# zahmedy/PyTorch-Distributed-Data-Parallel-DDP-Trainer

Hardware: AMD Instinct MI355X
Metric: images/sec MNIST SimpleCNN DDP at 1/2/4/8 MI355X; DDP scaling efficiency (higher is better)
Workload: dtype bf16; 1 GPU; model=SimpleCNN (520,586 params), global_batch=32, per_rank_batch=32, image=1x28x28, parallelism=dp1, engine=fused hipGraph, graph_steps=7, graph_head=0, fuse_level=3, level3=True, params_finite=True, bucket_allreduce=none, params_identical_across_ranks=True, ranks_seen=1, force_allreduce=False, inlaunch_allreduce=False

## Files before the change

csrc/bindings.cpp:

```cpp
#include <torch/extension.h>
#include <c10/hip/HIPStream.h>

#include <optional>

#include "kernels/conv_infer.h"
#include "kernels/launchers.h"
#include "runtime/runtime.h"

namespace py = pybind11;
using at::Tensor;
using namespace ddp_amd;

extern "C" const char ddp_amd_source_hash_str[];

namespace {

hipStream_t cur_stream() { return c10::hip::getCurrentHIPStream().stream(); }

void check_cuda(const Tensor& t, const char* name) {
  TORCH_CHECK(t.is_cuda(), name, " must be a GPU tensor");
  TORCH_CHECK(t.is_contiguous(), name, " must be contiguous");
}
void check(const Tensor& t, const char* name, at::ScalarType st) {
  check_cuda(t, name);
// ... 1118 lines not shown
  m.def("seg_sqnorm", &op_seg_sqnorm, py::arg("p"), py::arg("g"), py::arg("plan"), py::arg("partials"),
        py::arg("ticket"), py::arg("sums"), py::arg("trust"), py::arg("trust_coef"), py::arg("eps"),
        py::arg("gscale") = py::none());
  m.def("lars", &op_lars, py::arg("p"), py::arg("g"), py::arg("mbuf"), py::arg("lr"), py::arg("momentum"),
        py::arg("dampening"), py::arg("nesterov"), py::arg("maximize"), py::arg("first_step"), py::arg("update"),
        py::arg("shadows"), py::arg("plan"), py::arg("trust"), py::arg("gscale") = py::none(),
        py::arg("sched") = py::none());
  m.def("seg_sqnorm_blocks", &seg_sqnorm_blocks);
  m.attr("LARS_ITEM") = LARS_ITEM;
  m.attr("LARS_CHUNK") = LARS_CHUNK;
  m.attr("LARS_MAX_BLOCKS") = LARS_MAX_BLOCKS;
  m.attr("LARS_MAX_SEGS") = LARS_MAX_SEGS;
  m.def("grad_norm_blocks", &grad_norm_blocks);
  m.attr("GRAD_NORM_THREADS") = GN_THREADS;
  m.attr("GRAD_NORM_QUADS") = GN_QUADS;
  m.attr("GRAD_NORM_MAX_BLOCKS") = GN_MAX_BLOCKS;
  m.def("grad_reduce", &op_grad_reduce);
  m.def("scale_copy", &op_scale_copy);
  m.def("_mark_exiting", &ddp_amd::mark_exiting);
  m.def("conv_gemm_fwd", &op_conv_gemm_fwd, py::arg("X"), py::arg("W"), py::arg("bias"), py::arg("Y"),
        py::arg("KH"), py::arg("KW"), py::arg("stride"), py::arg("pad"), py::arg("relu") = false,
        py::arg("stats") = py::none(), py::arg("part") = py::none(), py::arg("bp") = 0, py::arg("bc") = 0,
        py::arg("splits") = 0, py::arg("halo") = -1, py::arg("bn") = py::none());
  m.def("conv_gemm_infer", &op_conv_gemm_infer, py::arg("X"), py::arg("W"), py::arg("sc"), py::arg("sh"),
        py::arg("res"), py::arg("Y"), py::arg("KH"), py::arg("KW"), py::arg("stride"), py::arg("pad"),
        py::arg("relu") = true, py::arg("part") = py::none(), py::arg("bp") = 0, py::arg("bc") = 0,
        py::arg("splits") = 0, py::arg("halo") = -1);
  m.def("bn_fold", &op_bn_fold);
  m.def("resnet_eval_tail", &op_resnet_eval_tail);
  m.def("resnet_eval_totals", &op_resnet_eval_totals);
  m.def("conv_gemm_dgrad", &op_conv_gemm_dgrad, py::arg("dY"), py::arg("W"), py::arg("Xact"), py::arg("dX"),
        py::arg("KH"), py::arg("KW"), py::arg("stride"), py::arg("pad"), py::arg("part") = py::none(),
        py::arg("bp") = 0, py::arg("bc") = 0, py::arg("splits") = 0, py::arg("parity") = -1,
        py::arg("halo") = -1);
  m.def("conv_gemm_wgrad_chunks", &op_conv_gemm_wgrad_chunks);
  m.def("conv_gemm_wgrad_set_halo", &conv_gemm_wgrad_set_halo, py::arg("halo"), py::arg("target") = 256,
        py::arg("cit") = 0,
        "weight-gradient plan override: halo 0 = the per-tap GEMM kernel only, 1 (default) / 2 = "
        "tap-fused halo kernel for every eligible stride-1 3x3 layer; target = blocks per launch; cit = "
        "input channels per halo block (0 auto, 16, 32)");
  m.def("conv_gemm_wgrad_force_tile", &conv_gemm_wgrad_force_tile);
  m.def("conv_gemm_wgrad_tiles", [](const Tensor& X, const Tensor& dY, int KH, int KW, int st, int pd) {
    return conv_gemm_wgrad_tiles(geom_of(X, dY, KH, KW, st, pd));
  });
  m.def("conv_gemm_wgrad_ppc", [](const Tensor& X, const Tensor& dY, int KH, int KW, int st, int pd) {
    return conv_gemm_wgrad_ppc(geom_of(X, dY, KH, KW, st, pd));
  });
  m.def("conv_gemm_wgrad", &op_conv_gemm_wgrad, py::arg("dY"), py::arg("X"), py::arg("out"), py::arg("KH"),
        py::arg("KW"), py::arg("stride"), py::arg("pad"), py::arg("ppc"), py::arg("accum") = false,
        py::arg("ks") = 0, py::arg("bn") = py::none());
  m.def("conv_gemm_wgrad_uses_halo", [](const Tensor& X, const Tensor& dY, int KH, int KW, int stride, int pad,
                                        int ppc) { return conv_gemm_wgrad_uses_halo(geom_of(X, dY, KH, KW, stride, pad), ppc); });
  m.def("conv_gemm_plan", &op_conv_gemm_plan, py::arg("X"), py::arg("Y"), py::arg("KH"), py::arg("KW"),
        py::arg("stride"), py::arg("pad"), py::arg("dgrad") = false, py::arg("bp") = 0, py::arg("bc") = 0,
        py::arg("splits") = 0, py::arg("parity") = -1, py::arg("halo") = -1);
  m.def("bn_finalize", &op_bn_finalize);
  m.def("hip_set_device_flags", [](int dev, unsigned flags) {
    hipError_t e = hipSetDevice(dev);
    if (e == hipSuccess) e = hipSetDeviceFlags(flags);
    return (int)e;
  });
  m.def("bn_apply", &op_bn_apply);
  m.def("bn_finalize_groups", &bn_finalize_groups);
  m.def("bn_bwd_rows", [](long P, int C) { return bn_bwd_rows(P, C, nullptr); });
  m.def("bn_bwd", &op_bn_bwd, py::arg("dout"), py::arg("out"), py::arg("x"), py::arg("mean"),
        py::arg("invstd"), py::arg("gamma"), py::arg("count"), py::arg("ws"), py::arg("sums"),
        py::arg("dgamma"), py::arg("dbeta"), py::arg("accum"), py::arg("dx"), py::arg("dres"),
        py::arg("dout2") = py::none(), py::arg("mask_beta") = py::none());
  m.def("bn_bwd_set_px_per_block", &bn_bwd_set_px_per_block);
  m.def("maxpool_fwd", &op_maxpool_fwd, py::arg("x"), py::arg("y"), py::arg("amax"), py::arg("bn") = py::none());
  m.def("maxpool_bwd", &op_maxpool_bwd, py::arg("dy"), py::arg("amax"), py::arg("dx"),
        py::arg("dy2") = py::none());
  m.def("avgpool_fwd", &op_avgpool_fwd);
  m.def("image_gather_nhwc4", &op_image_gather_nhwc4);
  m.def("image_gather_aug_nhwc4", &op_image_gather_aug_nhwc4);
  m.def("image_gather_mix_nhwc4", &op_image_gather_mix_nhwc4);
  m.def("avgpool_bwd", &op_avgpool_bwd);
  m.def("sgemm", &op_sgemm, py::arg("M"), py::arg("N"), py::arg("K"), py::arg("A"), py::arg("sam"),
        py::arg("sak"), py::arg("B"), py::arg("sbk"), py::arg("sbn"), py::arg("C"), py::arg("bias"),
        py::arg("alpha"), py::arg("accum") = false);
  m.def("transpose_w", &op_transpose_w);
  m.def("rccl_version", []() { int v = 0; ncclGetVersion(&v); return v; });
  m.def("step_head_slots", &conv3x3_step_head_slots);
  m.def("source_hash", []() {
    const std::string s(ddp_amd_source_hash_str);
    const size_t eq = s.find('=');
    return eq == std::string::npos ? s : s.substr(eq + 1);
  });
  m.def("pci_bus_id", [](int dev) {
    char buf[64] = {0};
    if (hipDeviceGetPCIBusId(buf, sizeof(buf) - 1, dev) != hipSuccess)
      throw std::runtime_error("hipDeviceGetPCIBusId failed");
    return std::string(buf);
  });

  py::class_<Comm, std::shared_ptr<Comm>>(m, "Comm")
      .def_static("new_unique_id", []() { return py::bytes(Comm::new_unique_id()); })
      .def(py::init([](py::bytes uid, int rank, int world, int device) {
             return std::make_shared<Comm>(std::string(uid), rank, world, device);
           }))
      .def_property_readonly("rank", &Comm::rank)
      .def_property_readonly("world", &Comm::world)
      .def("all_reduce", [](Comm& c, Tensor& t, int op, uint64_t stream) {
             check_cuda(t, "tensor");
             c.all_reduce(t.data_ptr(), t.numel(), dtype_code(t), op, stream_or_current(stream));
           }, py::arg("tensor"), py::arg("op") = 0, py::arg("stream") = 0)
      .def("all_reduce_premul", [](Comm& c, Tensor& t, double scale, uint64_t stream) {
             check_cuda(t, "tensor");
             TORCH_CHECK(t.scalar_type() == at::kFloat && t.is_contiguous(), "all_reduce_premul: contiguous fp32");
             c.all_reduce_premul(t.data_ptr<float>(), t.numel(), (float)scale, stream_or_current(stream));
           }, py::arg("tensor"), py::arg("scale"), py::arg("stream") = 0)
      .def("broadcast", [](Comm& c, Tensor& t, int root, uint64_t stream) {
             check_cuda(t, "tensor");
             c.broadcast(t.data_ptr(), t.numel(), dtype_code(t), root, stream_or_current(stream));
           }, py::arg("tensor"), py::arg("root") = 0, py::arg("stream") = 0)
      .def("all_gather", [](Comm& c, const Tensor& send, Tensor& recv, uint64_t stream) {
             check_cuda(send, "send"); check_cuda(recv, "recv");
             TORCH_CHECK(recv.numel() == send.numel() * c.world(), "all_gather: recv size");
             c.all_gather(send.data_ptr(), recv.data_ptr(), send.numel(), dtype_code(send),
                          stream_or_current(stream));
           }, py::arg("send"), py::arg("recv"), py::arg("stream") = 0)
      .def("reduce_scatter", [](Comm& c, const Tensor& send, Tensor& recv, int op, uint64_t stream) {
             check_cuda(send, "send"); check_cuda(recv, "recv");
             TORCH_CHECK(send.numel() == recv.numel() * c.world(), "reduce_scatter: send size");
             c.reduce_scatter(send.data_ptr(), recv.data_ptr(), recv.numel(), dtype_code(recv), op,
                              stream_or_current(stream));
           }, py::arg("send"), py::arg("recv"), py::arg("op") = 0, py::arg("stream") = 0);

  py::class_<XgmiComm, std::shared_ptr<XgmiComm>>(m, "XgmiComm")
      .def(py::init<int, int, int>(), py::arg("rank"), py::arg("world"), py::arg("device"))
      .def("add_channel", &XgmiComm::add_channel, py::arg("off"), py::arg("n"), py::arg("oneshot") = false,
           py::arg("grid_cap") = 0)
      .def("blocks", &XgmiComm::blocks)
      .def("bus_id", &XgmiComm::bus_id)
      .def("oneshot", &XgmiComm::oneshot)
      .def_property_readonly("channels", &XgmiComm::channels)
      .def("set_data", [](XgmiComm& x, Tensor& t) {
        check(t, "data", at::kFloat);
        x.set_data(t.data_ptr<float>(), t.numel());
      })
      .def("export_handles", [](const XgmiComm& x) { return py::bytes(x.export_handles()); })
      .def("import_handles", [](XgmiComm& x, const std::vector<py::bytes>& all) {
        std::vector<std::string> v;
        for (const auto& b : all) v.emplace_back(b);
        x.import_handles(v);
      })
      .def("all_reduce", [](XgmiComm& x, int ch, double scale, bool publish, double prescale) {
        x.all_reduce(ch, cur_stream(), (float)scale, publish, (float)prescale);
      }, py::arg("channel"), py::arg("scale") = 1.0, py::arg("publish") = false, py::arg("prescale") = 1.0)
      .def("all_reduce_pair", [](XgmiComm& x, int ch0, int ch1, std::optional<Tensor> params,
                                 std::optional<Tensor> mbuf, double lr, double momentum, double dampening,
                                 double wd, bool nesterov, bool first_step, std::optional<Tensor> step_ctr) {
        SgdArgs sa{(float)lr, (float)momentum, (float)dampening, (float)wd, nesterov ? 1 : 0, 0,
                   first_step ? 1 : 0, params ? 1 : 0};
        float* p = nullptr;
        float* m = nullptr;
        if (params) {
          check(*params, "params", at::kFloat);
          TORCH_CHECK(params->numel() >= x.data_numel(), "all_reduce_pair: params smaller than the data buffer");
          p = params->data_ptr<float>();
          if (momentum != 0.0) {
            TORCH_CHECK(mbuf.has_value(), "all_reduce_pair: momentum buffer required");
            check(*mbuf, "momentum", at::kFloat);
            TORCH_CHECK(mbuf->numel() == params->numel(), "all_reduce_pair: momentum size");
            m = mbuf->data_ptr<float>();
          }
// ... 53 lines not shown
            check(p, "params", at::kFloat);
            TORCH_CHECK(p.numel() >= x.data_numel(r), "xgmi loopback: params smaller than the data buffer");
            TORCH_CHECK(((uintptr_t)p.data_ptr() & 15) == 0, "xgmi loopback: params must be 16-byte aligned");
            rb[r].params = p.data_ptr<float>();
            if (mom) {
              Tensor& mb = (*mbuf)[r];
              check(mb, "momentum", at::kFloat);
              TORCH_CHECK(mb.numel() == p.numel() && ((uintptr_t)mb.data_ptr() & 15) == 0,
                          "xgmi loopback: momentum buffer size / alignment");
              rb[r].mbuf = mb.data_ptr<float>();
            }
            if (shadows) {
              rb[r].sh = make_shadows((*shadows)[r]);
              for (int i = 0; i < rb[r].sh.count; ++i)
                TORCH_CHECK(rb[r].sh.r[i].off >= 0 && rb[r].sh.r[i].off + rb[r].sh.r[i].n <= p.numel(),
                            "shadow out of range");
            }
          }
        } else {
          TORCH_CHECK(!shadows, "xgmi loopback: shadows need params");
        }
        if (step_ctr) {
          TORCH_CHECK((int)step_ctr->size() == W, "xgmi loopback: one step counter per rank");
          for (int r = 0; r < W; ++r) {
            check((*step_ctr)[r], "step_ctr", at::kInt);
            rb[r].step_ctr = (*step_ctr)[r].data_ptr<int>();
          }
        }
        x.all_reduce(ch, cur_stream(), sa, rb, (float)scale, publish, (float)prescale, wt);
      }, py::arg("channel"), py::arg("scale") = 1.0, py::arg("publish") = false, py::arg("prescale") = 1.0,
         py::arg("wt") = false, py::arg("params") = py::none(), py::arg("momentum_buffer") = py::none(),
         py::arg("shadows") = py::none(), py::arg("step_ctr") = py::none(), py::arg("lr") = 0.0,
         py::arg("momentum") = 0.0, py::arg("dampening") = 0.0, py::arg("weight_decay") = 0.0,
         py::arg("nesterov") = false, py::arg("first_step") = false)
      .def("error_flags", &XgmiLoopback::error_flags)
      .def("seq", &XgmiLoopback::seq, py::arg("channel"), py::arg("rank"), py::arg("block"))
      .def("set_timeout", &XgmiLoopback::set_timeout);
  py::class_<Reducer,std::shared_ptr<Reducer>>(m, "Reducer")
      .def(py::init([](std::shared_ptr<Comm> comm, Tensor& flat, std::vector<long> poff,
                       std::vector<long> pnum, std::vector<int> pb, std::vector<long> boff,
                       std::vector<long> bnum, bool prescale) {
             check(flat, "flat_grad", at::kFloat);
             for (size_t i = 0; i < poff.size(); ++i)
               TORCH_CHECK(poff[i] >= 0 && poff[i] + pnum[i] <= flat.numel(), "param slot OOB");
             for (size_t i = 0; i < boff.size(); ++i)
               TORCH_CHECK(boff[i] >= 0 && boff[i] + bnum[i] <= flat.numel(), "bucket OOB");
             return std::make_shared<Reducer>(comm, flat.data_ptr<float>(), poff, pnum, pb, boff,
                                              bnum, prescale);
           }))
      .def("mark_ready", [](Reducer& r, int param, std::optional<Tensor> grad) {
             const float* src = nullptr;
             if (grad) { check(*grad, "grad", at::kFloat); src = grad->data_ptr<float>(); }
             r.mark_ready(param, src, cur_stream());
           })
      .def("finalize", [](Reducer& r) { r.finalize(cur_stream()); })
      .def("set_xgmi", &Reducer::set_xgmi, py::arg("xgmi"), py::arg("channels"))
      .def_property_readonly("world", &Reducer::world)
      .def("reset", &Reducer::reset)
      .def_property_readonly("num_buckets", &Reducer::num_buckets)
      .def_property_readonly("allreduce_calls", &Reducer::allreduce_calls);

  py::class_<SimpleCNNEngine, std::shared_ptr<SimpleCNNEngine>>(m, "SimpleCNNEngine")
      .def(py::init([](py::dict cfgd, py::dict t, py::dict offs, std::shared_ptr<Comm> comm) {
             EngineConfig c{};
             c.max_batch = cfgd["max_batch"].cast<int>();
             c.H = cfgd["H"].cast<int>(); c.W = cfgd["W"].cast<int>();
             c.C1 = cfgd["C1"].cast<int>(); c.C2 = cfgd["C2"].cast<int>(); c.NO = cfgd["NO"].cast<int>();
             c.pxt_fwd = cfgd["pxt_fwd"].cast<int>(); c.pxt_dgrad = cfgd["pxt_dgrad"].cast<int>();
             c.wgrad_rows = cfgd["wgrad_rows"].cast<int>();
             c.world = cfgd["world"].cast<int>(); c.rank = cfgd["rank"].cast<int>();
             c.lr = cfgd["lr"].cast<float>(); c.momentum = cfgd["momentum"].cast<float>();
             c.dampening = cfgd["dampening"].cast<float>();
             c.weight_decay = cfgd["weight_decay"].cast<float>();
             c.nesterov = cfgd["nesterov"].cast<bool>(); c.maximize = cfgd["maximize"].cast<bool>();
             c.force_allreduce = cfgd.contains("force_allreduce") ? cfgd["force_allreduce"].cast<bool>() : false;
             c.fuse_level = cfgd.contains("fuse_level") ? cfgd["fuse_level"].cast<int>() : 0;
             c.fuse_opt = cfgd.contains("fuse_opt") ? (int)cfgd["fuse_opt"].cast<bool>() : 1;
             c.store_a1 = cfgd.contains("store_a1") ? cfgd["store_a1"].cast<int>() : 0;
             c.f32 = cfgd.contains("f32") ? (int)cfgd["f32"].cast<bool>() : 0;
             c.fuse_reduce = cfgd.contains("fuse_reduce") ? cfgd["fuse_reduce"].cast<int>() : 1;
             c.wgrad_split = cfgd.contains("wgrad_split") ? cfgd["wgrad_split"].cast<int>() : 1;
             c.l3_fc_role = cfgd.contains("l3_fc_role") ? cfgd["l3_fc_role"].cast<int>() : 1;
             c.dist_mode = cfgd.contains("dist_mode") ? cfgd["dist_mode"].cast<int>() : 3;
             TORCH_CHECK(c.dist_mode >= 0 && c.dist_mode <= 4, "engine: dist_mode must be 0..4");
             TORCH_CHECK(c.l3_fc_role == 0 || c.l3_fc_role == 1, "engine: l3_fc_role must be 0 or 1");
             TORCH_CHECK(c.wgrad_split == 1 || c.wgrad_split == 2, "engine: wgrad_split must be 1 or 2");
             const int es = c.f32 ? 4 : 2;
             TORCH_CHECK(c.store_a1 >= 0 && c.store_a1 <= 2, "engine: store_a1 must be 0, 1 or 2");
             TORCH_CHECK(c.fuse_level == 0 || c.fuse_level == 1 || c.fuse_level == 3,
                         "engine: fuse_level must be 0, 1 or 3 (level 2 was removed in round 4)");
             TORCH_CHECK(conv3x3_fwd_lds(c.W, c.C1, c.pxt_fwd, c.fuse_level > 0, es) <= 160 * 1024 &&
                             conv3x3_wgrad_lds(c.W, c.C1, c.C2, c.wgrad_rows, c.fuse_level > 0, es) <= 160 * 1024 &&
                             conv3x3_dgrad_lds(c.W, c.C2, c.pxt_dgrad, true, es) <= 160 * 1024,
                         "engine: LDS budget exceeded for this tiling");
             auto T = [&](const char* k) { return t[k].cast<Tensor>(); };
             auto need = [&](const char* k, at::ScalarType st, long n) {
               Tensor x = T(k);
               check(x, k, st);
               TORCH_CHECK(x.numel() >= n, "engine buffer ", k, " too small: ", x.numel(), " < ", n);
               return x;
             };
             const long B = c.max_batch, HW = (long)c.H * c.W;
             EngineBuffers b{};
             Tensor params = need("params", at::kFloat, 1);
             b.params = params.data_ptr<float>();
             b.n_params = params.numel();
             b.grads = need("grads", at::kFloat, b.n_params).data_ptr<float>();
             b.momentum = (c.momentum != 0.f) ? need("momentum", at::kFloat, b.n_params).data_ptr<float>() : nullptr;
             auto O = [&](const char* k) { return offs[k].cast<long>(); };
             b.off_w1 = O("w1"); b.off_b1 = O("b1"); b.off_w2 = O("w2"); b.off_b2 = O("b2");
             b.off_wfc = O("wfc"); b.off_bfc = O("bfc");
             std::vector<EngineBucket> buckets;
             for (auto item : offs["buckets"].cast<py::list>()) {
               auto pr = item.cast<std::pair<long, long>>();
               buckets.push_back(EngineBucket{pr.first, pr.second});
             }
             TORCH_CHECK(b.off_wfc + (long)c.NO * HW * c.C2 <= b.n_params && b.off_w1 + 9L * c.C1 <= b.n_params &&
                         b.off_b2 + c.C2 <= b.n_params && b.off_w2 + 9L * c.C1 * c.C2 <= b.n_params,
                         "engine: parameter offsets out of range");
             TORCH_CHECK(fc_bwd_lds(c.max_batch, c.NO, true, ((long)c.max_batch * HW + 64L * c.pxt_fwd - 1) / (64L * c.pxt_fwd) * 2 * c.NO) <= 160 * 1024,
                         "engine: batch too large for fc_bwd LDS");
             if (c.f32) {
               TORCH_CHECK(c.fuse_level >= 1 && c.store_a1 == 0, "engine: fp32 needs fuse_level 1 or 3 and store_a1 0");
               b.a2_f32 = need("a2", at::kFloat, B * HW * c.C2).data_ptr<float>();
               b.dz2_f32 = need("dz2", at::kFloat, B * HW * c.C2).data_ptr<float>();
               b.w2t_f32 = need("w2t_f32", at::kFloat, 9L * c.C1 * c.C2).data_ptr<float>();
               b.wfc_frag32 = need("wfc_frag32", at::kFloat, (long)c.NO * HW * c.C2).data_ptr<float>();
             } else {
               b.w2_bf16 = bf(need("w2_bf16", at::kBFloat16, 9L * c.C1 * c.C2));
               b.w2t_bf16 = bf(need("w2t_bf16", at::kBFloat16, 9L * c.C1 * c.C2));
               b.wfc_bf16 = bf(need("wfc_bf16", at::kBFloat16, (long)c.NO * HW * c.C2));
               b.wfc_frag = bf(need("wfc_frag", at::kBFloat16, (long)c.NO * HW * c.C2));
               b.a1 = bf(need("a1", at::kBFloat16, B * HW * c.C1));
               b.a2 = bf(need("a2", at::kBFloat16, B * HW * c.C2));
               b.dz2 = bf(need("dz2", at::kBFloat16, B * HW * c.C2));
               b.dz1 = bf(need("dz1", at::kBFloat16, B * HW * c.C1));
             }
             b.fc_part = need("fc_part", at::kFloat, 2L * conv3x3_dgrad_blocks(B, c.H, c.W, c.pxt_fwd) * c.NO).data_ptr<float>();
             b.dlogits = need("dlogits", at::kFloat, B * c.NO).data_ptr<float>();
             b.loss_rows = need("loss_rows", at::kFloat, B).data_ptr<float>();
             b.loss_hist = need("loss_hist", at::kFloat, 1).data_ptr<float>();
             b.w2slab = need("w2slab", at::kFloat, (long)conv3x3_wgrad_blocks(B, c.H, c.wgrad_rows) * (9L * c.C1 * c.C2 + c.C2)).data_ptr<float>();
             b.w1slab = need("w1slab", at::kFloat, (long)conv3x3_dgrad_blocks(B, c.H, c.W, c.pxt_dgrad) * 320).data_ptr<float>();
             b.step_ctr = need("step_ctr", at::kInt, 1).data_ptr<int>();
             b.xb = need("xb", at::kByte, B * HW).data_ptr<unsigned char>();
             b.yb = need("yb", at::kInt, B).data_ptr<int>();
             if (t.contains("sync_flags")) {
               long nfl = L3_HEAD_OFF;
               if (c.fuse_level >= 3) nfl = std::max(nfl, (long)L3_HEAD_OFF + (long)FWD_DZ_CNT_STRIDE * 2);
               b.sync_flags = need("sync_flags", at::kInt, nfl).data_ptr<int>();
               b.sync_err = need("sync_err", at::kInt, 1).data_ptr<int>();
             }
             Tensor images = need("images", at::kByte, HW);
             b.images = images.data_ptr<unsigned char>();
             Tensor labels = need("labels", at::kInt, 1);
             b.labels = labels.data_ptr<int>();
             Tensor idx = need("idx", at::kInt, 1);
             b.idx = idx.data_ptr<int>();
             b.n_idx = (int)idx.numel();
             b.n_rows = (int)std::min<long>(images.numel() / HW, labels.numel());
             if (cfgd.contains("epoch_order") && cfgd["epoch_order"].cast<bool>()) b.idx = nullptr;
             TORCH_CHECK(conv3x3_wgrad_lds(c.W, c.C1, c.C2, c.wgrad_rows, true, es) <= 160 * 1024, "wgrad rows too large");
             return std::make_shared<SimpleCNNEngine>(c, b, comm, buckets);
           }),
           py::arg("config"), py::arg("tensors"), py::arg("offsets"), py::arg("comm") = nullptr)
      .def("step", &SimpleCNNEngine::step, py::arg("batch"), py::arg("batch_stride"))
      .def("refresh_shadows", &SimpleCNNEngine::refresh_shadows)
      .def("set_lr", &SimpleCNNEngine::set_lr)
      .def("capture", &SimpleCNNEngine::capture)
      .def("replay", &SimpleCNNEngine::replay)
      .def("destroy_graph", &SimpleCNNEngine::destroy_graph)
      .def("synchronize", &SimpleCNNEngine::synchronize, py::call_guard<py::gil_scoped_release>())
      .def_property_readonly("last_fused_reduce", &SimpleCNNEngine::last_fused_reduce)
      .def_property_readonly("last_level3", &SimpleCNNEngine::last_level3)
      .def_property_readonly("last_fc_role", &SimpleCNNEngine::last_fc_role)
      .def_property_readonly("last_xar", &SimpleCNNEngine::last_xar)
      .def_property_readonly("last_pair", &SimpleCNNEngine::last_pair)
      .def_property_readonly("last_head", &SimpleCNNEngine::last_head)
      .def_property_readonly("graph_heads", &SimpleCNNEngine::graph_heads)
      .def("overlap_active", &SimpleCNNEngine::overlap_active)
      .def("level3_active", &SimpleCNNEngine::level3_active, py::arg("batch"))
      .def_property_readonly("sync_error", &SimpleCNNEngine::sync_error)
      .def("set_momentum_started", &SimpleCNNEngine::set_momentum_started)
      .def("set_xgmi", &SimpleCNNEngine::set_xgmi, py::arg("xgmi"), py::arg("channels"))
      .def_property_readonly("num_buckets", &SimpleCNNEngine::num_buckets)
      .def("bucket_stage", &SimpleCNNEngine::bucket_stage)
      .def_property_readonly("graph_steps", &SimpleCNNEngine::graph_steps)
      .def_property_readonly("stream", [](SimpleCNNEngine& e) { return (uint64_t)e.stream(); });
}
```

csrc/kernels/common.h:

```cpp
#pragma once
#include <hip/hip_runtime.h>
#include <stdint.h>

#include "kernels/types.h"

namespace ddp_amd {

typedef __attribute__((ext_vector_type(8))) short bf16x8;
typedef __attribute__((ext_vector_type(4))) short bf16x4;
typedef __attribute__((ext_vector_type(4))) float f32x4;
typedef __attribute__((address_space(3))) bf16x4 lds_bf16x4;
typedef __attribute__((address_space(3))) char lds_char;
__device__ __forceinline__ lds_bf16x4* lds_ptr4(lds_char* base, int elem_off) {
  return (lds_bf16x4*)(base + 2 * elem_off);
}
typedef __attribute__((ext_vector_type(2))) __bf16 bf16x2v;

constexpr int WAVE = 64;

__device__ __forceinline__ void lds_barrier() {
  asm volatile("s_waitcnt lgkmcnt(0)\n\ts_barrier" ::: "memory");
}

namespace {
__constant__ unsigned long long* g_stamp_buf = nullptr;
}
#define DDP_STAMP(kid, slot)                                                                 \
  do {                                                                                       \
    unsigned long long* _sb = g_stamp_buf;                                                   \
    if (_sb && threadIdx.x == 0 && blockIdx.y == 0 && blockIdx.x < 4096)                    \
      _sb[(kid) * STAMP_KSTRIDE + blockIdx.x * STAMP_SLOTS + (slot)] = __builtin_amdgcn_s_memrealtime(); \
  } while (0)
#define DDP_STAMPS_SETTER(name)                                                              \
  void name(void* p) { (void)hipMemcpyToSymbol(HIP_SYMBOL(g_stamp_buf), &p, sizeof(p)); }

__device__ __forceinline__ float bf2f(bf16_t b) {
  return __builtin_bit_cast(float, ((unsigned)b) << 16);
}
__device__ __forceinline__ bf16_t f2bf(float f) {
  return __builtin_bit_cast(bf16_t, (__bf16)f);
}
__device__ __forceinline__ float bf16_round(float f) { return bf2f(f2bf(f)); }

__device__ __forceinline__ bf16x8 zero8() {
  bf16x8 z = {0, 0, 0, 0, 0, 0, 0, 0};
  return z;
}
__device__ __forceinline__ bf16x8 ld8(const bf16_t* p) {
  return *reinterpret_cast<const bf16x8*>(p);
}
__device__ __forceinline__ f32x4 mfma16(bf16x8 a, bf16x8 b, f32x4 c) {
  return __builtin_amdgcn_mfma_f32_16x16x32_bf16(a, b, c, 0, 0, 0);
}

__device__ __forceinline__ bf16x8 ld16(const void* p) { return *reinterpret_cast<const bf16x8*>(p); }
__device__ __forceinline__ void st16(void* p, bf16x8 v) { *reinterpret_cast<bf16x8*>(p) = v; }

struct F32Frag {
  f32x4 lo, hi;
};
template <typename T>
struct Prec;
template <>
struct Prec<bf16_t> {
  using Frag = bf16x8;
  static constexpr int CE = 8;
  static constexpr int PAD = 16;
  static __device__ __forceinline__ int kofs(int lane) { return 8 * (lane >> 4); }
  static __device__ __forceinline__ Frag frag(const bf16_t* p) { return *reinterpret_cast<const bf16x8*>(p); }
  static __device__ __forceinline__ Frag zero() { return zero8(); }
  static __device__ __forceinline__ f32x4 mma(const Frag& a, const Frag& b, f32x4 c) { return mfma16(a, b, c); }
};
template <>
struct Prec<float> {
  using Frag = F32Frag;
  static constexpr int CE = 4;
  static constexpr int PAD = 8;
  static __device__ __forceinline__ int kofs(int lane) { return 4 * (lane >> 4); }
  static __device__ __forceinline__ Frag frag(const float* p) {
    return Frag{*reinterpret_cast<const f32x4*>(p), *reinterpret_cast<const f32x4*>(p + 16)};
  }
  static __device__ __forceinline__ Frag zero() { return Frag{{0.f, 0.f, 0.f, 0.f}, {0.f, 0.f, 0.f, 0.f}}; }
  static __device__ __forceinline__ f32x4 mma(const Frag& a, const Frag& b, f32x4 c) {
#pragma unroll
    for (int j = 0; j < 4; ++j) c = __builtin_amdgcn_mfma_f32_16x16x4f32(a.lo[j], b.lo[j], c, 0, 0, 0);
#pragma unroll
    for (int j = 0; j < 4; ++j) c = __builtin_amdgcn_mfma_f32_16x16x4f32(a.hi[j], b.hi[j], c, 0, 0, 0);
    return c;
  }
};
template <typename F>
__device__ __forceinline__ F fsel(bool ok, const F& v, const F& z) {
  return ok ? v : z;
}

__device__ __forceinline__ int xcd_remap(int b, int nb) {
  const int per = nb >> 3, rem = nb & 7, x = b & 7, i = b >> 3;
  return x < rem ? x * (per + 1) + i : rem * (per + 1) + (x - rem) * per + i;
}
__device__ __forceinline__ int3 xcd_block3() {
  const int gx = gridDim.x, gy = gridDim.y;
  const int b = blockIdx.x + gx * (blockIdx.y + gy * blockIdx.z);
  const int l = xcd_remap(b, gx * gy * gridDim.z);
  return make_int3(l % gx, (l / gx) % gy, l / (gx * gy));
}

__device__ __forceinline__ uint2 pack4(float a, float b, float c, float d) {
  uint2 r;
  r.x = (unsigned)f2bf(a) | ((unsigned)f2bf(b) << 16);
  r.y = (unsigned)f2bf(c) | ((unsigned)f2bf(d) << 16);
  return r;
}
__device__ __forceinline__ void unpack4(uint2 v, float* o) {
  o[0] = __builtin_bit_cast(float, v.x << 16);
  o[1] = __builtin_bit_cast(float, v.x & 0xffff0000u);
  o[2] = __builtin_bit_cast(float, v.y << 16);
  o[3] = __builtin_bit_cast(float, v.y & 0xffff0000u);
}

__device__ __forceinline__ bf16x8 mask8(bf16x8 g, bf16x8 y) {
  bf16x8 r;
#pragma unroll
  for (int j = 0; j < 8; ++j) {
    const unsigned short u = (unsigned short)y[j];
    const bool pos = (u & 0x8000u) == 0 && u != 0;
    r[j] = pos ? g[j] : (short)0;
  }
  return r;
}

template <typename T>
__device__ __forceinline__ bf16x8 mask16(bf16x8 g, bf16x8 y);
template <>
__device__ __forceinline__ bf16x8 mask16<bf16_t>(bf16x8 g, bf16x8 y) {
  return mask8(g, y);
}
template <>
__device__ __forceinline__ bf16x8 mask16<float>(bf16x8 g, bf16x8 y) {
  const f32x4 gf = __builtin_bit_cast(f32x4, g), yf = __builtin_bit_cast(f32x4, y);
// ... 142 lines not shown
```

csrc/kernels/conv3x3_body.h:

```cpp
#pragma once
#include <algorithm>
#include <stdexcept>

#include <cstdio>
#include <cstdlib>

#include "kernels/common.h"
#include "kernels/fc_bwd_body.h"
#include "kernels/launchers.h"
#include "kernels/slab_reduce.h"
#include "kernels/xgmi_body.h"

namespace ddp_amd {

template <int INF, int NT = 256, typename S1, typename D1, typename S2, typename D2>
__device__ __forceinline__ void stage2(int n1, S1 src1, D1 dst1, int n2, S2 src2, D2 dst2) {
  const int n = n1 + n2;
  for (int base = threadIdx.x; base < n; base += NT * INF) {
    bf16x8 v[INF];
#pragma unroll
    for (int u = 0; u < INF; ++u) {
      const int i = base + u * NT;
      v[u] = (i < n1) ? src1(i) : ((i < n) ? src2(i - n1) : zero8());
    }
#pragma unroll
    for (int u = 0; u < INF; ++u) {
      const int i = base + u * NT;
      if (i < n1) dst1(i, v[u]);
      else if (i < n) dst2(i - n1, v[u]);
    }
  }
}
template <typename SrcFn, typename DstFn>
__device__ __forceinline__ void stage16(int n, SrcFn src, DstFn dst) {
  stage2<8>(n, src, dst, 0, src, dst);
}

constexpr unsigned long long DZ_WAIT_TICKS = 2000000;

struct BwdReduce {
  SlabSet ss{};
  long nchunks = 0;
  int first_reducer = 0;
  int nconv = 0;
  int* done = nullptr;
  int* err = nullptr;
  int interleave = 0;
  int deep = 0;
};

#define DDP_GEOM_OVERRIDE()                                    \
  if (GH) {                                                    \
    H = GH; W = GW; Cin = GCI; Cout = GCO;                     \
  }


__host__ __device__ inline size_t fwd_stage_lds(int W, int Cin, int pxt, bool a1x, int es = 2) {
  const size_t XR = 64 * pxt + 2 * W + 2;
  const int pad = es == 2 ? 16 : 8;
  const size_t b = (size_t)es * ((size_t)64 * (9 * Cin + pad) + XR * (Cin + pad)) +
                   (a1x ? sizeof(float) * ((XR + 2 * W + 2) + Cin * 10) : 0);
  return (b + 15) & ~(size_t)15;
}
constexpr int FC_MAX_NOF = 16;
__host__ __device__ inline size_t fc_epi_lds(int pxt, int nof) { return sizeof(float) * 4 * pxt * 4 * nof; }

template <typename T, int PXT, bool MASK_DY, bool MASK_X, bool FUSE_W1, bool A1X, int GH, int GW, int GCI,
          int GCO, int WGS = 0>
__device__ __forceinline__ void dgrad_body(
    const T* __restrict__ dY, const T* __restrict__ Yact, const T* __restrict__ WT,
    const T* __restrict__ Xact, T* __restrict__ dX, int B, int H, int W, int Cin, int Cout,
    const void* __restrict__ x0, int x0_u8, BatchIdx bi, float* __restrict__ w1slab, C1Src c1, char* smem, int bx, int by) {
  using P = Prec<T>;
  constexpr bool F32 = sizeof(T) == 4;
  constexpr bool WG = WGS > 0, HALF = WGS == 1;
  static_assert(!WG || (F32 && GCI == 32 && GCO == 64 && FUSE_W1), "weights-from-global dgrad: fp32 SimpleCNN conv2");
  constexpr int CE = P::CE;
  constexpr int NCT = HALF ? 1 : 2;
  DDP_STAMP(STAMP_K_DGRAD, 0);
  DDP_GEOM_OVERRIDE();
  constexpr int CH = 64 * PXT;
  const int lane = threadIdx.x & 63, wave = threadIdx.x >> 6;
  const int HW = H * W;
  const long Ptot = (long)B * HW;
  const int ci_blk = HALF ? by * 16 : by * 32;
  const int KW = 9 * Cout, WS = KW + P::PAD, DS = Cout + P::PAD;
  const int XR = CH + 2 * W + 2;
  T* sWT = reinterpret_cast<T*>(smem);
  T* sDY = sWT + (WG ? 0 : 32 * WS);
  float* sx0 = reinterpret_cast<float*>(sDY + XR * DS);
  float* s_w1 = sx0 + XR;
  unsigned char* s_m1 = reinterpret_cast<unsigned char*>(s_w1 + 4 * 320);
  const long P0 = (long)bx * CH;
  const long Pbase = P0 - W - 1;
  const int mg = HALF ? 2 * by + (wave & 1) : wave;

  auto x0_at = [&](int r) {
    const long P = Pbase + r;
    float v = 0.f;
    if (P >= 0 && P < Ptot) {
      const int n = (int)(P / HW), rm = (int)(P - (long)n * HW);
      if (x0_u8) v = (float)((const unsigned char*)x0)[(long)bi.row(n, bi.base()) * HW + rm] / 255.0f;
      else v = ((const float*)x0)[P];
    }
    return v;
  };
  const float x0_pre = (FUSE_W1 && (int)threadIdx.x < XR) ? x0_at(threadIdx.x) : 0.f;
  Conv1Group cg;
  if (A1X) cg = conv1_group_load(c1.w, c1.b, mg);
  const T* wg = WT + (long)(ci_blk + (lane & 15)) * Cout + P::kofs(lane);
  const long tstr = (long)Cin * Cout;
  typename P::Frag an[WG ? 2 : 1][WG ? NCT : 1];
  if constexpr (WG) {
#pragma unroll
    for (int k = 0; k < 2; ++k)
#pragma unroll
      for (int t = 0; t < NCT; ++t) an[k][t] = P::frag(wg + 16 * t * Cout + 32 * k);
  }
  const int wc = KW / CE, cpc = Cout / CE;
  stage2<F32 ? 32 : 16>(WG ? 0 : 32 * wc,
          [&](int i) {
            const int r = i / wc, rest = (i - r * wc) * CE;
            const int tap = rest / Cout, co = rest - tap * Cout;
            return ld16(WT + ((long)tap * Cin + ci_blk + r) * Cout + co);
          },
          [&](int i, bf16x8 v) { const int r = i / wc, c = (i - r * wc) * CE; st16(sWT + r * WS + c, v); },
          XR * cpc,
          [&](int i) {
            const int r = i / cpc, c = (i - r * cpc) * CE;
            const long Pq = Pbase + r;
            bf16x8 v = zero8();
            if (Pq >= 0 && Pq < Ptot) {
              v = ld16(dY + Pq * Cout + c);
              if (MASK_DY) v = mask16<T>(v, ld16(Yact + Pq * Cout + c));
            }
            return v;
          },
          [&](int i, bf16x8 v) { const int r = i / cpc, c = (i - r * cpc) * CE; st16(sDY + r * DS + c, v); });
  DDP_STAMP(STAMP_K_CONV1, 0);
  if (FUSE_W1) {
    if ((int)threadIdx.x < XR) sx0[threadIdx.x] = x0_pre;
    for (int r = threadIdx.x + 256; r < XR; r += 256) sx0[r] = x0_at(r);
  }
  DDP_STAMP(STAMP_K_CONV1, 1);
  if (A1X) {
    __syncthreads();
    const int g = mg;
    for (int lp = lane + (HALF ? 64 * (wave >> 1) : 0); lp < CH; lp += HALF ? 128 : 64) {
      const long P = P0 + lp;
      unsigned m = 0;
      if (P < Ptot) {
        const int rm = (int)(P % HW);
        const int hh = rm / W, ww = rm - (rm / W) * W;
        float v[9];
#pragma unroll
        for (int k = 0; k < 9; ++k) {
          const int dh = k / 3 - 1, dw = k % 3 - 1;
          const bool ok = (unsigned)(hh + dh) < (unsigned)H && (unsigned)(ww + dw) < (unsigned)W;
          v[k] = ok ? sx0[lp + W + 1 + dh * W + dw] : 0.f;
        }
#pragma unroll
        for (int j = 0; j < 8; ++j) {
          const float a1v = conv1_eval_g(cg, v, j);
          m |= ((F32 ? a1v : bf2f(f2bf(a1v))) > 0.f ? 1u : 0u) << j;
        }
      }
      s_m1[lp * 4 + g] = (unsigned char)m;
    }
    DDP_STAMP(STAMP_K_CONV1, 2);
  }
  const int kofs = P::kofs(lane);
  const int col = lane & 15;
  int h[PXT], w[PXT], rowc[PXT];
  bool valid[PXT];
  long Pp[PXT];
  float xa[PXT][2][4] = {};
#pragma unroll
  for (int pt = 0; pt < PXT; ++pt) {
    const int lp = (wave * PXT + pt) * 16 + col;
    Pp[pt] = P0 + lp;
    valid[pt] = Pp[pt] < Ptot;
    const long Pc = valid[pt] ? Pp[pt] : 0;
    const int n = (int)(Pc / HW);
    const int rm = (int)(Pc - (long)n * HW);
    h[pt] = rm / W;
    w[pt] = rm - h[pt] * W;
    rowc[pt] = lp + W + 1;
    if (MASK_X && !A1X) {
#pragma unroll
      for (int t = 0; t < NCT; ++t) {
        const T* xp = Xact + Pc * Cin + ci_blk + 16 * t + 4 * (lane >> 4);
        if constexpr (F32) {
          const float4 x4 = *reinterpret_cast<const float4*>(xp);
          xa[pt][t][0] = x4.x; xa[pt][t][1] = x4.y; xa[pt][t][2] = x4.z; xa[pt][t][3] = x4.w;
        } else {
          unpack4(*reinterpret_cast<const uint2*>(xp), xa[pt][t]);
        }
      }
    }
  }
  lds_barrier();
  DDP_STAMP(STAMP_K_DGRAD, 1);

  f32x4 acc[PXT][NCT];
#pragma unroll
  for (int pt = 0; pt < PXT; ++pt)
#pragma unroll
    for (int t = 0; t < NCT; ++t) acc[pt][t] = (f32x4){0.f, 0.f, 0.f, 0.f};
  auto kstep = [&](int tap, int co0, const typename P::Frag* a) {
    const int dh = 1 - tap / 3, dw = 1 - tap % 3;
    typename P::Frag b[PXT];
#pragma unroll
    for (int pt = 0; pt < PXT; ++pt) {
      const int hh = h[pt] + dh, ww = w[pt] + dw;
      const bool ok = valid[pt] && (unsigned)hh < (unsigned)H && (unsigned)ww < (unsigned)W;
      const typename P::Frag v = P::frag(sDY + (rowc[pt] + dh * W + dw) * DS + co0 + kofs);
      b[pt] = fsel(ok, v, P::zero());
    }
#pragma unroll
    for (int pt = 0; pt < PXT; ++pt)
#pragma unroll
      for (int t = 0; t < NCT; ++t) acc[pt][t] = P::mma(a[t], b[pt], acc[pt][t]);
  };
  if constexpr (WG) {
#pragma unroll
    for (int tap = 0; tap < 9; ++tap) {
      typename P::Frag ac[2][NCT];
#pragma unroll
      for (int k = 0; k < 2; ++k)
#pragma unroll
        for (int t = 0; t < NCT; ++t) ac[k][t] = an[k][t];
      if (tap + 1 < 9) {
#pragma unroll
        for (int k = 0; k < 2; ++k)
#pragma unroll
          for (int t = 0; t < NCT; ++t) an[k][t] = P::frag(wg + (tap + 1) * tstr + 16 * t * Cout + 32 * k);
      }
      kstep(tap, 0, ac[0]);
      kstep(tap, 32, ac[1]);
    }
  } else {
    const T* wrow = sWT + col * WS + kofs;
#pragma unroll
    for (int tap = 0; tap < 9; ++tap) {
      for (int co0 = 0; co0 < Cout; co0 += 32) {
        const typename P::Frag a[2] = {P::frag(wrow + tap * Cout + co0), P::frag(wrow + 16 * WS + tap * Cout + co0)};
        kstep(tap, co0, a);
      }
    }
  }

  DDP_STAMP(STAMP_K_DGRAD, 2);
  float w1a[FUSE_W1 ? NCT : 1][4][10];
  if (FUSE_W1) {
#pragma unroll
    for (int t = 0; t < NCT; ++t)
#pragma unroll
      for (int j = 0; j < 4; ++j)
#pragma unroll
        for (int k = 0; k < 10; ++k) w1a[t][j][k] = 0.f;
  }
#pragma unroll
  for (int pt = 0; pt < PXT; ++pt) {
    float xv[9];
    if (FUSE_W1) {
#pragma unroll
      for (int k = 0; k < 9; ++k) {
        const int dh = k / 3 - 1, dw = k % 3 - 1;
        const int hh = h[pt] + dh, ww = w[pt] + dw;
        const bool ok = valid[pt] && (unsigned)hh < (unsigned)H && (unsigned)ww < (unsigned)W;
        xv[k] = ok ? sx0[rowc[pt] + dh * W + dw] : 0.f;
      }
    }
#pragma unroll
    for (int t = 0; t < NCT; ++t) {
      const int ci = ci_blk + 16 * t + 4 * (lane >> 4);
      float v[4] = {acc[pt][t][0], acc[pt][t][1], acc[pt][t][2], acc[pt][t][3]};
      if (MASK_X && A1X) {
        const int lp = (wave * PXT + pt) * 16 + col;
        const unsigned m = s_m1[lp * 4 + (ci >> 3)] >> (ci & 7);
#pragma unroll
        for (int j = 0; j < 4; ++j) v[j] = ((m >> j) & 1u) ? v[j] : 0.f;
      } else if (MASK_X) {
#pragma unroll
        for (int j = 0; j < 4; ++j) v[j] = xa[pt][t][j] > 0.f ? v[j] : 0.f;
      }
      float q[4] = {v[0], v[1], v[2], v[3]};
      if constexpr (F32) {
        if (dX && valid[pt]) *reinterpret_cast<float4*>(dX + Pp[pt] * Cin + ci) = make_float4(v[0], v[1], v[2], v[3]);
      } else {
        const uint2 pk = pack4(v[0], v[1], v[2], v[3]);
        if (dX && valid[pt]) *reinterpret_cast<uint2*>(dX + Pp[pt] * Cin + ci) = pk;
        unpack4(pk, q);
      }
      if (FUSE_W1) {
#pragma unroll
        for (int j = 0; j < 4; ++j) {
          const float d = valid[pt] ? q[j] : 0.f;
#pragma unroll
          for (int k = 0; k < 9; ++k) w1a[t][j][k] = fmaf(d, xv[k], w1a[t][j][k]);
          w1a[t][j][9] += d;
        }
      }
    }
  }
  DDP_STAMP(STAMP_K_DGRAD, 3);
  if (FUSE_W1) {
#pragma unroll
    for (int t = 0; t < NCT; ++t)
#pragma unroll
      for (int j = 0; j < 4; ++j)
#pragma unroll
        for (int k = 0; k < 10; ++k) w1a[t][j][k] = sum16(w1a[t][j][k]);
    if (col == 0) {
#pragma unroll
      for (int t = 0; t < NCT; ++t)
#pragma unroll
        for (int j = 0; j < 4; ++j) {
          const int ci = ci_blk + 16 * t + 4 * (lane >> 4) + j;
#pragma unroll
          for (int k = 0; k < 9; ++k) s_w1[wave * 320 + ci * 9 + k] = w1a[t][j][k];
          s_w1[wave * 320 + 288 + ci] = w1a[t][j][9];
        }
    }
    __syncthreads();
    for (int i = threadIdx.x; i < 320; i += 256) {
      if (HALF && ((i < 288 ? i / 9 : i - 288) >> 4) != by) continue;
      st_wt(w1slab + (long)bx * 320 + i, ((s_w1[i] + s_w1[320 + i]) + s_w1[640 + i]) + s_w1[960 + i]);
    }
  }
  DDP_STAMP(STAMP_K_DGRAD, 4);
}

template <typename T, int PXT, bool MASK_DY, bool MASK_X, bool FUSE_W1, bool A1X, int GH, int GW, int GCI,
          int GCO>
__global__ __launch_bounds__(256) void conv3x3_dgrad_kernel(
    const T* __restrict__ dY, const T* __restrict__ Yact, const T* __restrict__ WT,
    const T* __restrict__ Xact, T* __restrict__ dX, int B, int H, int W, int Cin, int Cout,
    const void* __restrict__ x0, int x0_u8, BatchIdx bi, float* __restrict__ w1slab, C1Src c1) {
  extern __shared__ __attribute__((aligned(16))) char smem[];
  dgrad_body<T, PXT, MASK_DY, MASK_X, FUSE_W1, A1X, GH, GW, GCI, GCO>(
      dY, Yact, WT, Xact, dX, B, H, W, Cin, Cout, x0, x0_u8, bi, w1slab, c1, smem, blockIdx.x, blockIdx.y);
}

template <typename T, bool MASK_DY, bool A1X, int GH, int GW, int GCI, int GCO, bool STAGE = false, int CS = 1>
__device__ __forceinline__ void wgrad_body(
    const T* __restrict__ dY, const T* __restrict__ Yact, const T* __restrict__ X,
    float* __restrict__ slab, int B, int H, int W, int Cin, int Cout, int R, C1Src c1, char* smem, int bx, int by) {
  constexpr bool F32 = sizeof(T) == 4;
  constexpr int CE = Prec<T>::CE;
  static_assert(CS == 1 || (CS == 2 && (STAGE || F32) && !(STAGE && F32) && GCI == 32 && GCO == 64),
                "the channel-split wgrad role: bf16 with a staged slab row, or fp32 with direct stores");
  constexpr bool XC = F32 && CS == 2;
  DDP_STAMP(STAMP_K_WGRAD, 0);
  DDP_GEOM_OVERRIDE();
  const int lane = threadIdx.x & 63, wave = threadIdx.x >> 6;
  const int nRC = (H + R - 1) / R;
  int rb = bx, half = 0;
  if constexpr (CS == 2) {
    if (((B * nRC) & 7) == 0) {
      half = (bx >> 3) & 1;
      rb = ((bx >> 4) << 3) | (bx & 7);
    } else {
      half = bx & 1;
      rb = bx >> 1;
    }
  }
  const int n = rb / nRC;
  const int r0 = (rb - n * nRC) * R;
  const int Wp = (W + 7) & ~7;
  const int DS = Cout + 16, XS = XC ? 16 : Cin + 16;
  const int nslot = ((R * Wp + 31) / 32) * 32;
  T* sdY = reinterpret_cast<T*>(smem);
  T* sX = sdY + (long)nslot * DS;
  const int XW = Wp + 2;

  const int c1g = CS == 2 ? 2 * half + (wave & 1) : wave;
  Conv1Group cg;
  if (A1X) cg = conv1_group_load(c1.w, c1.b, c1g);
  const int cxn = CS == 2 ? Cin / 2 : Cin, cx0 = half * cxn;
  const int cpy_dy = Cout / CE, cpy_x = cxn / CE;
  auto dy_src = [&](int i) {
    const int slot = i / cpy_dy, ch = (i - slot * cpy_dy) * CE;
    const int r = slot / Wp, c = slot - (slot / Wp) * Wp;
    const int hh = r0 + r;
    bf16x8 v = zero8();
    if (r < R && hh < H && c < W) {
      const long off = (((long)n * H + hh) * W + c) * Cout + ch;
      v = ld16(dY + off);
      if (MASK_DY) v = mask16<T>(v, ld16(Yact + off));
    }
    return v;
  };
  auto dy_dst = [&](int i, bf16x8 v) {
    const int slot = i / cpy_dy, ch = (i - slot * cpy_dy) * CE;
    st16(sdY + (long)slot * DS + ch, v);
  };
  const int XW2 = Wp + 4, XR2 = R + 4, NXX = XR2 * XW2;
  float* sxx = reinterpret_cast<float*>(sX + (long)(R + 2) * XW * XS);
  const long img = A1X ? (long)c1.bi.row(n, c1.bi.base()) * H * W : 0;
  auto x_inside = [&](int i, int& off) {
    const int rr = i / XW2, cc = i - (i / XW2) * XW2;
    const int hh = r0 - 2 + rr, ww = cc - 2;
    off = hh * W + ww;
    return (unsigned)hh < (unsigned)H && (unsigned)ww < (unsigned)W;
  };
  auto recompute = [&]() {
    conv1_recompute_tile<T>(
        (R + 2) * XW, cg, c1g, CS == 2 ? 64 * (wave >> 1) : 0, CS == 2 ? 128 : 64,
        [&](int pos) {
          const int rr = pos / XW, cc = pos - (pos / XW) * XW;
          return (unsigned)(r0 - 1 + rr) < (unsigned)H && (unsigned)(cc - 1) < (unsigned)W;
        },
        [&](int pos, int k) {
          const int rr = pos / XW, cc = pos - (pos / XW) * XW;
          return sxx[(rr + k / 3) * XW2 + cc + k % 3];
        },
        [&](int pos, int g) { return sX + (long)pos * XS + 8 * (XC ? g - 2 * half : g); });
  };
  const int ndy = nslot * cpy_dy;
  stage2<F32 ? 32 : 16>(ndy, dy_src, dy_dst,
          A1X ? 0 : (R + 2) * XW * cpy_x,
          [&](int i) {
            const int pos = i / cpy_x, ch = cx0 + (i - pos * cpy_x) * CE;
            const int rr = pos / XW, cc = pos - (pos / XW) * XW;
            const int hh = r0 - 1 + rr, ww = cc - 1;
            return ((unsigned)hh < (unsigned)H && (unsigned)ww < (unsigned)W)
                       ? ld16(X + (((long)n * H + hh) * W + ww) * Cin + ch) : zero8();
          },
          [&](int i, bf16x8 v) {
            const int pos = i / cpy_x, ch = cx0 + (i - pos * cpy_x) * CE;
            st16(sX + (long)pos * XS + (XC ? ch - cx0 : ch), v);
          });
  if (A1X) {
    for (int i = threadIdx.x; i < NXX; i += 256) {
      int off = 0;
      sxx[i] = x_inside(i, off) ? (float)c1.x[img + off] / 255.0f : 0.f;
    }
    __syncthreads();
    DDP_STAMP(STAMP_K_WGRAD, 1);
    recompute();
  }
  __syncthreads();
  DDP_STAMP(STAMP_K_WGRAD, 2);

  constexpr int NCT = CS == 2 ? 1 : 2;
  const int nct = Cin / 16;
  const int asg = by * 4 + wave;
  const int coT = CS == 2 ? 16 * wave : (asg / nct) * 32;
  const int ciT = CS == 2 ? 16 * half : (asg - (asg / nct) * nct) * 16;
  const int g = lane >> 4, i16 = lane & 15, q = i16 >> 2, p = i16 & 3;

  f32x4 acc[NCT][9], accb[NCT];
#pragma unroll
  for (int c = 0; c < NCT; ++c) {
    accb[c] = (f32x4){0.f, 0.f, 0.f, 0.f};
#pragma unroll
    for (int k = 0; k < 9; ++k) acc[c][k] = (f32x4){0.f, 0.f, 0.f, 0.f};
  }
  if constexpr (F32) {
    const int ciL = XC ? 0 : ciT;
    const bool bias = CS == 1 || ciT == 0;
#pragma unroll 1
    for (int s0 = 0; s0 < nslot; s0 += 32) {
#pragma unroll
      for (int j = 0; j < 8; ++j) {
        const int sl = s0 + 4 * j + g;
        float a[NCT];
#pragma unroll
        for (int c = 0; c < NCT; ++c) a[c] = sdY[(long)sl * DS + coT + 16 * c + i16];
        const int rs0 = sl / Wp, cs = sl - rs0 * Wp, rs = min(rs0, R - 1);
#pragma unroll
// ... 28 lines not shown
      }
      const int rA0 = sA / Wp, cA = sA - rA0 * Wp, rB0 = sB / Wp, cB = sB - rB0 * Wp;
      const int rA = min(rA0, R - 1), rB = min(rB0, R - 1);
      const int xA = ldsX + (rA * XW + cA) * XS + ciT + 4 * p, xB = ldsX + (rB * XW + cB) * XS + ciT + 4 * p;
#pragma unroll
      for (int tap = 0; tap < 9; ++tap) {
        const int kh = tap / 3, kw = tap % 3;
        const int to = (kh * XW + kw) * XS;
        const bf16x4 lo = __builtin_amdgcn_ds_read_tr16_b64_v4i16(lds_ptr4(lsm, xA + to));
        const bf16x4 hi = __builtin_amdgcn_ds_read_tr16_b64_v4i16(lds_ptr4(lsm, xB + to));
        const bf16x8 b = (bf16x8){lo[0], lo[1], lo[2], lo[3], hi[0], hi[1], hi[2], hi[3]};
#pragma unroll
        for (int c = 0; c < NCT; ++c) acc[c][tap] = mfma16(a[c], b, acc[c][tap]);
      }
      if (CS == 1 || ciT == 0) {
#pragma unroll
        for (int c = 0; c < NCT; ++c) accb[c] = mfma16(a[c], ones, accb[c]);
      }
    }
  }

  DDP_STAMP(STAMP_K_WGRAD, 3);
  const long row = (long)Cout * 9 * Cin + Cout;
  float* out = slab + (long)rb * row;
  if constexpr (STAGE) {
    __syncthreads();
    float* srow = reinterpret_cast<float*>(smem);
    const int wrow = 9 * Cin;
#pragma unroll
    for (int c = 0; c < NCT; ++c)
#pragma unroll
      for (int r = 0; r < 4; ++r) {
        const int co = coT + 16 * c + 4 * g + r;
        const int sk = 16 * (co >> 2);
#pragma unroll
        for (int tap = 0; tap < 9; ++tap) srow[co * wrow + tap * Cin + ciT + i16 + sk] = acc[c][tap][r];
        if (ciT == 0 && i16 == 0) srow[Cout * wrow + 4 * Cout + co] = accb[c][r];
      }
    __syncthreads();
    const __amdgpu_buffer_rsrc_t rs = __builtin_amdgcn_make_buffer_rsrc(out, (short)0, (int)(row * 4), 0x00020000);
    typedef __attribute__((ext_vector_type(4))) int i32x4_t;
    if constexpr (CS == 2) {
      const int nq = Cout * 9 * 4;
      const int nst = nq + (half == 0 ? Cout / 4 : 0);
      for (int i = threadIdx.x; i < nst; i += 256) {
        const int e = i < nq ? (i >> 2) * Cin + 16 * half + 4 * (i & 3) : Cout * wrow + 4 * (i - nq);
        const int pos = e < Cout * wrow ? e + 16 * ((e / wrow) >> 2) : e + 4 * Cout;
        __builtin_amdgcn_raw_buffer_store_b128(__builtin_bit_cast(i32x4_t, *reinterpret_cast<const float4*>(srow + pos)),
                                               rs, e * 4, 0, 16 );
      }
    } else {
      for (int i = threadIdx.x; i < row / 4; i += 256) {
        const int e = 4 * i;
        const int pos = e < Cout * wrow ? e + 16 * ((e / wrow) >> 2) : e + 4 * Cout;
        __builtin_amdgcn_raw_buffer_store_b128(__builtin_bit_cast(i32x4_t, *reinterpret_cast<const float4*>(srow + pos)),
                                               rs, i * 16, 0, 16 );
      }
    }
  } else {
#pragma unroll
    for (int c = 0; c < NCT; ++c)
#pragma unroll
      for (int r = 0; r < 4; ++r) {
        const int co = coT + 16 * c + 4 * g + r;
#pragma unroll
        for (int tap = 0; tap < 9; ++tap) st_wt(out + ((long)co * 9 + tap) * Cin + ciT + i16, acc[c][tap][r]);
        if (ciT == 0 && i16 == 0) st_wt(out + (long)Cout * 9 * Cin + co, accb[c][r]);
      }
  }
  DDP_STAMP(STAMP_K_WGRAD, 4);
}

template <typename T, bool MASK_DY, bool A1X, int GH, int GW, int GCI, int GCO>
__global__ __launch_bounds__(256) void conv3x3_wgrad_kernel(
    const T* __restrict__ dY, const T* __restrict__ Yact, const T* __restrict__ X,
    float* __restrict__ slab, int B, int H, int W, int Cin, int Cout, int R, C1Src c1) {
  extern __shared__ __attribute__((aligned(16))) char smem[];
  wgrad_body<T, MASK_DY, A1X, GH, GW, GCI, GCO>(dY, Yact, X, slab, B, H, W, Cin, Cout, R, c1, smem,
                                              blockIdx.x, blockIdx.y);
}

constexpr int BFC_MAXB = 64;

__device__ __forceinline__ float* fc_role_prologue(const BwdFc& fcr, int B, char* smem, bool first0) {
  float* s_dl = reinterpret_cast<float*>(smem);
  for (int i = threadIdx.x; i < B * 10; i += 256) s_dl[(i / 10) * FCDW_LD + i % 10] = fcr.dl[i];
  __syncthreads();
  if (first0 && threadIdx.x < 64) {
    float* s_dd = s_dl + B * FCDW_LD;
    for (int i = threadIdx.x; i < B * 10; i += 64) s_dd[i] = s_dl[(i / 10) * FCDW_LD + i % 10];
    asm volatile("s_waitcnt lgkmcnt(0)" ::: "memory");
    fc_bwd_bias_loss<false>(fcr.ex, s_dd, nullptr, B, 10, true);
  }
  return s_dl;
}
template <typename T>
__device__ __forceinline__ void fc_role_chunk(const BwdFc& fcr, const float* s_dl, int B, long q) {
  const T* a2 = static_cast<const T*>(fcr.a2);
  if (B <= 32) fc_dw_wave_chunk<32>(s_dl, a2, fcr.dW, fcr.scale, B, fcr.K, fcr.ex, q * 128);
  else fc_dw_wave_chunk<BFC_MAXB>(s_dl, a2, fcr.dW, fcr.scale, B, fcr.K, fcr.ex, q * 128);
}

template <int SLEEP = 2>
__device__ __forceinline__ bool wait_count(const int* cnt, int want, int* err, int code) {
  __shared__ int s_ok;
  if (threadIdx.x < 64) {
    const unsigned long long t0 = __builtin_amdgcn_s_memrealtime();
    bool ok = true;
    while (__hip_atomic_load(cnt, __ATOMIC_RELAXED, __HIP_MEMORY_SCOPE_AGENT) < want) {
      if (__builtin_amdgcn_s_memrealtime() - t0 > DZ_WAIT_TICKS) {
        if (threadIdx.x == 0 && err) __hip_atomic_store(err, code, __ATOMIC_RELAXED, __HIP_MEMORY_SCOPE_AGENT);
        ok = false;
        break;
      }
      __builtin_amdgcn_s_sleep(SLEEP);
    }
    if (threadIdx.x == 0) s_ok = ok ? 1 : 0;
  }
  __syncthreads();
  return s_ok != 0;
}

__device__ __forceinline__ void count_done(int* cnt) {
  asm volatile("s_waitcnt vmcnt(0)" ::: "memory");
  __syncthreads();
  if (threadIdx.x == 0) __hip_atomic_fetch_add(cnt, 1, __ATOMIC_RELAXED, __HIP_MEMORY_SCOPE_AGENT);
}

template <typename T, int PXT, bool DA1X, bool WA1X, int GH, int GW, int GCI, int GCO, bool FRED, int CS = 1,
          bool FCR = false, int DG = 1, bool XAR = false>
__global__ __launch_bounds__(256, (sizeof(T) == 2 || CS == 2) ? 2 : 1) void conv3x3_bwd_kernel(
    const T* __restrict__ dY, const T* __restrict__ WT, T* __restrict__ dX,
    float* __restrict__ w1slab, float* __restrict__ slab, int B, int H, int W, int Cin, int Cout,
    int R, int nd, C1Src c1, const T* __restrict__ Xact, BwdReduce red, BwdFc fcr, BwdXar xar) {
  extern __shared__ __attribute__((aligned(16))) char smem[];
  int cb = (int)blockIdx.x;
  if constexpr (XAR) {
    static_assert(FCR && FRED, "the in-launch all-reduce waits for the fc role and the fused reduction");
    const int nx = xar.nblk0 + xar.nblk1;
    if (cb < nx) {
      unsigned* s_sh = reinterpret_cast<unsigned*>(smem);
      DDP_STAMP(STAMP_K_XGMI, 0);
      const int k = cb < xar.nblk0 ? 0 : 1;
      XgmiArgs* s_xa = reinterpret_cast<XgmiArgs*>(smem + 64);
      {
        const int* src = reinterpret_cast<const int*>(xar.args + k);
        int* dst = reinterpret_cast<int*>(s_xa);
        for (int i = threadIdx.x; i < (int)(sizeof(XgmiArgs) / 4); i += 256) dst[i] = src[i];
      }
      if (k == 0) {
        const bool ok = wait_count(xar.fc_done, xar.fc_expect, xar.err, XAR_ERR);
        DDP_STAMP(STAMP_K_XGMI, 5);
        if (ok) xgmi_allreduce_body(*s_xa, cb, xar.nblk0, s_sh);
      } else {
        const bool ok = wait_count(xar.fc_done, xar.fc_expect, xar.err, XAR_ERR) &&
                        wait_count(xar.red_done, xar.red_expect, xar.err, XAR_ERR);
        DDP_STAMP(STAMP_K_XGMI, 5);
        if (ok) xgmi_allreduce_body(*s_xa, cb - xar.nblk0, xar.nblk1, s_sh);
      }
      asm volatile("s_waitcnt vmcnt(0)" ::: "memory");
      __syncthreads();
      DDP_STAMP(STAMP_K_XGMI, 7);
      if (threadIdx.x == 0) {
        const int old = __hip_atomic_fetch_add(xar.xar_done, 1, __ATOMIC_RELAXED, __HIP_MEMORY_SCOPE_AGENT);
        if (old == nx - 1 && xar.step_ctr) xar.step_ctr[0] += 1;
      }
      return;
    }
    cb -= nx;
  }
  if constexpr (FCR) {
    const int f = cb - fcr.fc0;
    if (f >= 0 && f < fcr.nfc) {
      DDP_STAMP(STAMP_K_FC_BWD, 0);
      __builtin_amdgcn_s_setprio(2);
      const float* s_dl = fc_role_prologue(fcr, B, smem, f == 0);
      DDP_STAMP(STAMP_K_FC_BWD, 1);
      const int nch = (int)((fcr.K + 127) / 128);
      const int q = f * 4 + (threadIdx.x >> 6);
      if (q < nch) fc_role_chunk<T>(fcr, s_dl, B, q);
      DDP_STAMP(STAMP_K_FC_BWD, 4);
      if constexpr (XAR) count_done(xar.fc_done);
      return;
// ... 108 lines not shown
```

csrc/kernels/conv3x3_fwd.h:

```cpp
#pragma once

#include <type_traits>

#include "kernels/conv3x3_body.h"
#include "kernels/xent_body.h"

namespace ddp_amd {

constexpr unsigned long long FWD_DZ_WAIT_TICKS = 2000000;
#ifndef DDP_AMD_F32_FC_PREFETCH
#define DDP_AMD_F32_FC_PREFETCH 0
#endif
constexpr bool F32_FC_PREFETCH = DDP_AMD_F32_FC_PREFETCH;
#ifndef DDP_AMD_FWD_PF_SPLIT
#define DDP_AMD_FWD_PF_SPLIT 1
#endif

struct FwdMerge {
  const XgmiArgs* args = nullptr;
  int nblk0 = 0, nblk1 = 0;
  int* fc_done = nullptr;
  int* conv_done = nullptr;
  int* err = nullptr;
  ShadowSet late{};
};
constexpr int MRG_ERR = 5;

__device__ __forceinline__ bf16x8 ld16_sc1(__amdgpu_buffer_rsrc_t r, int byte_off) {
  typedef __attribute__((ext_vector_type(4))) int i32x4_t;
  return __builtin_bit_cast(bf16x8, __builtin_amdgcn_raw_buffer_load_b128(r, byte_off, 0, 16 ));
}
__device__ __forceinline__ Conv1Group conv1_group_load_sc1(const float* w1, const float* b1, int g) {
  Conv1Group r;
#pragma unroll
  for (int j = 0; j < 8; ++j) {
#pragma unroll
    for (int k = 0; k < 9; ++k)
      r.w[j][k] = __hip_atomic_load(w1 + (8 * g + j) * 9 + k, __ATOMIC_RELAXED, __HIP_MEMORY_SCOPE_AGENT);
    r.b[j] = __hip_atomic_load(b1 + 8 * g + j, __ATOMIC_RELAXED, __HIP_MEMORY_SCOPE_AGENT);
  }
  return r;
}
constexpr int MRG_SLEEP = 16;

__device__ __forceinline__ void merge_allreduce_role(FwdMerge mg, char* smem) {
  const int k = (int)blockIdx.x < mg.nblk1 ? 1 : 0;
  const int rb = k == 1 ? (int)blockIdx.x : (int)blockIdx.x - mg.nblk1;
  __builtin_amdgcn_s_setprio(2);
  unsigned* s_sh = reinterpret_cast<unsigned*>(smem);
  XgmiArgs* s_xa = reinterpret_cast<XgmiArgs*>(smem + 64);
  {
    const int* src = reinterpret_cast<const int*>(mg.args + k);
    int* dst = reinterpret_cast<int*>(s_xa);
    for (int i = threadIdx.x; i < (int)(sizeof(XgmiArgs) / 4); i += (int)blockDim.x) dst[i] = src[i];
  }
  __syncthreads();
  DDP_STAMP(STAMP_K_HEAD, 0);
  xgmi_allreduce_body<true>(*s_xa, rb, k == 0 ? mg.nblk0 : mg.nblk1, s_sh, STAMP_K_HEAD);
  DDP_STAMP(STAMP_K_HEAD, 7);
  count_done(k == 0 ? mg.fc_done : mg.conv_done);
  DDP_STAMP(STAMP_K_HEAD, 6);
  if (k == 1 && mg.late.count) {
    const XgmiArgs& a = *s_xa;
    const ShadowSet late = mg.late;
    const long n = a.n, G = (long)mg.nblk1 * XGMI_THREADS;
    const float* pb = a.params + a.off;
    const __amdgpu_buffer_rsrc_t rp = sys_rsrc(pb);
    for (long q = (long)rb * XGMI_THREADS + threadIdx.x; 4 * q < n; q += G) {
      if (4 * q + 3 < n) {
        shadow_quad<false>(late, a.off + 4 * q, ld4_sys(rp, q));
      } else {
        for (long e = 4 * q; e < n; ++e) shadow_one<false>(late, a.off + e, ld_sys(pb + e));
      }
    }
  }
}

template <typename T, int PXT, int NW, bool RELU, int NOF, bool A1X, int GH, int GW, int GCI, int GCO,
          bool DZ = false, int OCC = 1>
__global__ __launch_bounds__(NW * 64, OCC * NW / 4) void conv3x3_fwd_kernel(
    const T* __restrict__ X, const T* __restrict__ Wt, const float* __restrict__ bias,
    T* __restrict__ Y, int B, int H, int W, int Cin, int Cout,
    const T* __restrict__ wfc, float* __restrict__ fc_part, C1Src c1, FwdDz dzo) {
  constexpr bool MRG = false;
  constexpr bool NOA2 = false;
  const FwdMerge mg{};
  extern __shared__ __attribute__((aligned(16))) char smem[];
  const int bx = (int)blockIdx.x, by = (int)blockIdx.y;
#include "kernels/conv3x3_fwd_body.inc.h"
}

template <typename T, int PXT, int NW, bool RELU, int NOF, bool A1X, int GH, int GW, int GCI, int GCO, bool DZ,
          int OCC, bool MRG>
__device__ __forceinline__ void fwd_body(
    const int bx, const int by, const T* __restrict__ X, const T* __restrict__ Wt, const float* __restrict__ bias,
    T* __restrict__ Y, int B, int H, int W, int Cin, int Cout, const T* __restrict__ wfc,
    float* __restrict__ fc_part, const C1Src& c1, const FwdDz& dzo, const FwdMerge& mg) {
  constexpr bool NOA2 = false;
  extern __shared__ __attribute__((aligned(16))) char smem[];
#include "kernels/conv3x3_fwd_body.inc.h"
}

template <typename T, int PX, int OCC = 1>
static auto fwd_dz_kernel() {
  return conv3x3_fwd_kernel<T, 1, 4 * PX, true, 10, true, 28, 28, 32, 64, true, OCC>;
}

static bool fwd_dz_occ2(unsigned grid) {
  static const int env = [] { const char* e = getenv("DDP_AMD_FWD_OCC2"); return e ? atoi(e) : -1; }();
  if (env >= 0) return env == 1;
  int dev = 0, cus = 0;
  if (hipGetDevice(&dev) != hipSuccess) return false;
  if (hipDeviceGetAttribute(&cus, hipDeviceAttributeMultiprocessorCount, dev) != hipSuccess) return false;
  return cus > 0 && grid > (unsigned)cus;
}

template <typename T>
static bool fwd_dz_fits(int B, int H, int W, int pxt) {
  if (H != 28 || W != 28 || (pxt != 1 && pxt != 2) || B <= 0) return false;
  const long P = (long)B * H * W;
  const int per_blk = 64 * pxt;
  if (per_blk > H * W || P >= (1L << 31)) return false;
  const long grid = (P + per_blk - 1) / per_blk;
  const size_t lds = conv3x3_fwd_lds(W, 32, pxt, true, (int)sizeof(T));
  bool occ2 = false;
  const void* k = pxt == 2 ? reinterpret_cast<const void*>(fwd_dz_kernel<T, 2>())
                           : reinterpret_cast<const void*>(fwd_dz_kernel<T, 1>());
  if constexpr (sizeof(T) == 2) {
    occ2 = pxt == 2 && fwd_dz_occ2((unsigned)grid);
    if (occ2) {
      k = reinterpret_cast<const void*>(fwd_dz_kernel<T, 2, 2>());
      lds_optin(fwd_dz_kernel<T, 2, 2>(), lds);
    }
  }
  if (!occ2) lds_optin(pxt == 2 ? fwd_dz_kernel<T, 2>() : fwd_dz_kernel<T, 1>(), lds);
  int dev = 0, cus = 0, occ = 0;
  if (hipGetDevice(&dev) != hipSuccess) return false;
  if (hipDeviceGetAttribute(&cus, hipDeviceAttributeMultiprocessorCount, dev) != hipSuccess) return false;
  if (hipOccupancyMaxActiveBlocksPerMultiprocessor(&occ, k, occ2 ? 512 : 256 * pxt, lds) != hipSuccess) return false;
  if ((long)occ * cus >= grid) return true;
  return inorder_optin() && (long)occ * cus >= 64;
}
}
```

csrc/kernels/conv3x3_fwd_body.inc.h:

```cpp
  using P = Prec<T>;
  constexpr bool F32 = sizeof(T) == 4;
  static_assert(!DZ || (NOF == 10 && A1X), "level-3 dZ2 needs the fc epilogue and the conv1 recompute");
  static_assert(!MRG || (DZ && !F32), "the merged forward is the bf16 level-3 forward");
  constexpr int CE = P::CE;
  DDP_STAMP(STAMP_K_CONV_FWD, 0);
  DDP_GEOM_OVERRIDE();
  typedef __attribute__((address_space(1))) unsigned long long gran_t;
  constexpr int DZ_SW = (OCC == 2 || F32) ? XENT_MAX_BLK / 2 : XENT_MAX_BLK;
  unsigned dz_epoch = 1u;
  if constexpr (DZ) {
    const unsigned g = *dzo.gen + 1u;
    dz_epoch = g ? g : 1u;
  }
  constexpr int CH = 16 * NW * PXT, NT = NW * 64;
  const int lane = threadIdx.x & 63, wave = threadIdx.x >> 6;
  const int HW = H * W;
  const long Ptot = (long)B * HW;
  const int co0 = by * 64;
  const int KW = 9 * Cin, WS = KW + P::PAD, XS = Cin + P::PAD;
  const int XR = CH + 2 * W + 2;
  T* sW = reinterpret_cast<T*>(smem);
  T* sX = sW + 64 * WS;
  const long P0 = (long)bx * CH;
  const long Pbase = P0 - W - 1;
// ... 280 lines not shown
        if constexpr (NOA2) st_wt(dst, acc_o);
        else *dst = acc_o;
      }
    }
  }
  DDP_STAMP(STAMP_K_CONV_FWD, 4);
  if constexpr (DZ) {
    const int HWi = H * W;
    const int img0 = (int)(P0 / HWi);
    const long plast = (P0 + CH < Ptot ? P0 + CH : Ptot) - 1;
    const int nimg = (int)(plast / HWi) - img0 + 1;
    float* s_lg = s_fc + NW * PXT * 4 * NOF;
    float* s_dl = s_lg + 2 * NOF;
    auto store_a2 = [&]() {
#pragma unroll
      for (int pt = 0; pt < PXT; ++pt)
#pragma unroll
        for (int t = 0; t < 4; ++t) {
          const int co = co0 + 16 * t + 4 * (lane >> 4);
          if (!valid[pt]) continue;
          if constexpr (F32) st_wt(reinterpret_cast<float4*>(Y + Pp[pt] * Cout + co), a2q[pt][t]);
          else st_wt(reinterpret_cast<uint2*>(Y + Pp[pt] * Cout + co), a2pk[pt][t]);
        }
    };
    DDP_STAMP(STAMP_K_FWD_DZ, 0);
    store_a2();
    if (wave == 0) {
      const int slot = lane >= NOF ? 1 : 0, o = lane - slot * NOF;
      const bool act = lane < 2 * NOF && slot < nimg;
      int label = 0;
      float fcb = 0.f;
      if (lane < 2 * NOF) {
        const int im = img0 + slot;
        if (im < B) label = c1.labels[c1.bi.row(im, bi_base)];
        fcb = MRG ? __hip_atomic_load(dzo.fc_bias + o, __ATOMIC_RELAXED, __HIP_MEMORY_SCOPE_AGENT) : dzo.fc_bias[o];
      }
      const int im = img0 + (act ? slot : 0);
      const int nblk = (im * HWi + HWi - 1) / CH - im * HWi / CH + 1;
      const gran_t* gr = (const gran_t*)dzo.gran;
      const unsigned long long t0 = __builtin_amdgcn_s_memrealtime();
      bool dead = false;
      float a = 0.f;
      DDP_STAMP(STAMP_K_FWD_DZ, 1);
      auto sweep = [&](auto j0c) {
        constexpr int J0 = decltype(j0c)::value;
        unsigned long long g[DZ_SW];
#pragma unroll
        for (int k = 0; k < DZ_SW; ++k) g[k] = 0;
        const bool none = J0 > 0 && !__any(act && nblk > J0);
        while (!none) {
          bool ok = true;
          if (act) {
#pragma unroll
            for (int k = 0; k < DZ_SW; ++k)
              g[k] = __hip_atomic_load(gr + xent_logit_idx(im, o, HWi, CH, NOF, J0 + k), __ATOMIC_RELAXED,
                                       __HIP_MEMORY_SCOPE_AGENT);
#pragma unroll
            for (int k = 0; k < DZ_SW; ++k) ok &= (unsigned)(g[k] >> 32) == dz_epoch;
          }
          if (__all(ok) || dead) break;
          if (__builtin_amdgcn_s_memrealtime() - t0 > FWD_DZ_WAIT_TICKS) {
            if (lane == 0 && dzo.err) __hip_atomic_store(dzo.err, 3, __ATOMIC_RELAXED, __HIP_MEMORY_SCOPE_AGENT);
            dead = true;
            break;
          }
          __builtin_amdgcn_s_sleep(1);
        }
        a = xent_logit_acc_range<J0, J0 + DZ_SW>(a, im, o, HWi, CH, NOF, [&](int j, int) {
          return __builtin_bit_cast(float, (unsigned)g[j - J0]);
        });
      };
      sweep(std::integral_constant<int, 0>{});
      if constexpr (DZ_SW < XENT_MAX_BLK) sweep(std::integral_constant<int, DZ_SW>{});
      DDP_STAMP(STAMP_K_FWD_DZ, 2);
      asm volatile("" : "+v"(label));
      if (act) s_lg[lane] = fcb + a;
      DDP_STAMP(STAMP_K_FWD_DZ, 4);
      asm volatile("s_waitcnt lgkmcnt(0)" ::: "memory");
      if (act) {
        float lossv = 0.f;
        const float d = xent_row_dl(s_lg + slot * NOF, NOF, o, label, dzo.gscale, &lossv);
        s_dl[lane] = d;
        if (dzo.dl_out && (slot == 1 || P0 == (long)img0 * HWi)) {
          dzo.dl_out[im * NOF + o] = d;
          if (o == 0) dzo.loss_rows[im] = lossv;
        }
      }
    }
    lds_barrier();
    DDP_STAMP(STAMP_K_FWD_DZ, 3);
#pragma unroll
    for (int pt = 0; pt < PXT; ++pt) {
      const long tp = P0 + (wave * PXT + pt) * 16;
      const float* dl = s_dl + (tp / HWi != img0 ? NOF : 0);
      float d[NOF];
#pragma unroll
      for (int o = 0; o < NOF; ++o) d[o] = dl[o];
#pragma unroll
      for (int t = 0; t < 4; ++t) {
        if constexpr (!PFW && !F32) __builtin_amdgcn_sched_barrier(0);
        float dz[4] = {0.f, 0.f, 0.f, 0.f};
#pragma unroll
        for (int o = 0; o < NOF; ++o) {
          float w4[4];
          if constexpr (F32) {
            const float4 wf = wq[pt][t][o];
            w4[0] = wf.x; w4[1] = wf.y; w4[2] = wf.z; w4[3] = wf.w;
          } else if constexpr (PFW) {
            unpack4(wv[pt][t][o], w4);
          } else {
            unpack4(fcw(pt, t, o), w4);
          }
#pragma unroll
          for (int j = 0; j < 4; ++j) dz[j] = fmaf(d[o], w4[j], dz[j]);
        }
        float q[4];
        if constexpr (F32) {
          q[0] = a2q[pt][t].x; q[1] = a2q[pt][t].y; q[2] = a2q[pt][t].z; q[3] = a2q[pt][t].w;
        } else {
          unpack4(a2pk[pt][t], q);
        }
#pragma unroll
        for (int j = 0; j < 4; ++j) dz[j] = q[j] > 0.f ? dz[j] : 0.f;
        const int co = co0 + 16 * t + 4 * (lane >> 4);
        if constexpr (F32) {
          if (valid[pt]) st_wt(reinterpret_cast<float4*>(dzo.dz2_f32 + Pp[pt] * Cout + co), make_float4(dz[0], dz[1], dz[2], dz[3]));
        } else {
          if (valid[pt]) st_wt(reinterpret_cast<uint2*>(dzo.dz2 + Pp[pt] * Cout + co), pack4(dz[0], dz[1], dz[2], dz[3]));
        }
      }
    }
    DDP_STAMP(STAMP_K_CONV_FWD, 7);
    DDP_STAMP(STAMP_K_FWD_DZ, 5);
  }
```

csrc/kernels/fc_bwd_body.h:

```cpp
#pragma once
#include "kernels/common.h"
#include "kernels/launchers.h"
#include "kernels/xent_body.h"

namespace ddp_amd {

constexpr int FCB_RB = 8;

template <int CPL>
struct ColF {
  float v[CPL];
};
template <int CPL>
__device__ __forceinline__ ColF<CPL> ldc(const bf16_t* p) {
  ColF<CPL> r;
  if constexpr (CPL == 2) {
    const unsigned u = *reinterpret_cast<const unsigned*>(p);
    r.v[0] = __builtin_bit_cast(float, u << 16);
    r.v[1] = __builtin_bit_cast(float, u & 0xffff0000u);
  } else {
    const uint2 u = *reinterpret_cast<const uint2*>(p);
    r.v[0] = __builtin_bit_cast(float, u.x << 16);
    r.v[1] = __builtin_bit_cast(float, u.x & 0xffff0000u);
    r.v[2] = __builtin_bit_cast(float, u.y << 16);
    r.v[3] = __builtin_bit_cast(float, u.y & 0xffff0000u);
  }
  return r;
}
template <int CPL>
__device__ __forceinline__ ColF<CPL> ldc(const float* p) {
  ColF<CPL> r;
  if constexpr (CPL == 2) {
    const float2 a = *reinterpret_cast<const float2*>(p);
    r.v[0] = a.x; r.v[1] = a.y;
  } else {
    const float4 a = *reinterpret_cast<const float4*>(p);
    r.v[0] = a.x; r.v[1] = a.y; r.v[2] = a.z; r.v[3] = a.w;
  }
  return r;
}
template <int CPL>
__device__ __forceinline__ void stc_wt(bf16_t* p, const float* v) {
  const unsigned a = (unsigned)f2bf(v[0]) | ((unsigned)f2bf(v[1]) << 16);
  if constexpr (CPL == 2) {
    st_wt(reinterpret_cast<unsigned*>(p), a);
  } else {
    const unsigned b = (unsigned)f2bf(v[2]) | ((unsigned)f2bf(v[3]) << 16);
    st_wt(reinterpret_cast<uint2*>(p), make_uint2(a, b));
  }
}
template <int CPL>
__device__ __forceinline__ void stc_wt(float* p, const float* v) {
  if constexpr (CPL == 2) st_wt(reinterpret_cast<float2*>(p), make_float2(v[0], v[1]));
  else st_wt(reinterpret_cast<float4*>(p), make_float4(v[0], v[1], v[2], v[3]));
}

template <int WPB, int NOT, int CPL>
__host__ __device__ constexpr int fcb_red_floats() { return WPB * NOT * 64 * CPL; }

__host__ __device__ inline long fcb_lds_floats(int B, int NO, bool xent, long npart, int red) {
  const long head = ((long)(xent ? 2 * B * NO + B : B * NO) + B + 3) & ~3L;
  return head + (red > npart ? red : npart);
}

template <bool XENT>
__device__ __forceinline__ void fc_bwd_bias_loss(const FcBwdExtras& ex, const float* s_dl, const float* s_loss,
                                                 int B, int NO, bool last) {
  const int lane = threadIdx.x & 63;
  if (ex.dbias && lane < NO) {
    float acc = 0.f;
#pragma unroll 16
    for (int b = 0; b < B; ++b) acc += s_dl[b * NO + lane];
    const float g = acc * ex.dbias_scale;
    if (ex.sys_store) st_sys(ex.dbias + lane, g);
    else ex.dbias[lane] = g;
    if (last && ex.p_b && ex.sgd.update) {
      float m = ex.m_b ? ex.m_b[lane] : 0.f;
      const float pn = sgd_one(ex.p_b[lane], 0.f + g, &m, ex.sgd);
      ex.p_b[lane] = pn;
      if (ex.m_b) ex.m_b[lane] = m;
    }
  }
  if ((XENT || ex.loss_rows) && ex.loss_out) {
    const float* lr = XENT ? s_loss : ex.loss_rows;
    const int at = ex.step_ctr ? *ex.step_ctr : 0;
    float acc = 0.f;
    for (int b0 = 0; b0 < B; b0 += 64) {
      const float v = b0 + lane < B ? lr[b0 + lane] : 0.f;
      const int nb = B - b0 < 64 ? B - b0 : 64;
      for (int k = 0; k < nb; ++k)
        acc += __builtin_bit_cast(float, __builtin_amdgcn_readlane(__builtin_bit_cast(int, v), k));
    }
    if (lane == 63) {
      ex.loss_out[at] = acc / (float)B;
      if (last && ex.step_inc) *ex.step_inc = at + 1;
    }
  }
  if (last || !ex.last_ctr) {
    if (ex.zero_i32)
      for (int i = lane; i < ex.n_zero; i += 64) ex.zero_i32[(long)i * ex.zero_stride] = 0;
    if (ex.gen_inc && lane == 0) {
      const unsigned g = *ex.gen_inc + 1u;
      *ex.gen_inc = g == 0xffffffffu ? 0u : g;
    }
  }
}

constexpr int FCDW_LD = 12;
template <int MAXB, typename T>
__device__ __forceinline__ void fc_dw_wave_chunk(const float* s_dl, const T* __restrict__ X,
                                                 float* __restrict__ dW, float scale, int B, long K,
                                                 const FcBwdExtras& ex, long col0) {
  constexpr bool F32 = sizeof(T) == 4;
  constexpr int NO = 10, VW = 8, RPV = (MAXB + VW - 1) / VW;
  const int lane = threadIdx.x & 63;
  const long col = col0 + 2 * lane;
  const bool active = col < K;
  const long cc = active ? col : 0;
  typedef __attribute__((ext_vector_type(2))) int i32x2_t;
  const int vo4 = (int)cc * 4, vo2 = (int)cc * 2;
  float2 pp[NO], mm[NO];
  if (ex.sgd.update) {
    const __amdgpu_buffer_rsrc_t rp = __builtin_amdgcn_make_buffer_rsrc(ex.p_w, (short)0, 0x7fffffff, 0x00020000);
    const __amdgpu_buffer_rsrc_t rm =
        __builtin_amdgcn_make_buffer_rsrc(ex.m_w ? ex.m_w : ex.p_w, (short)0, 0x7fffffff, 0x00020000);
#pragma unroll
    for (int o = 0; o < NO; ++o) {
      pp[o] = __builtin_bit_cast(float2, __builtin_amdgcn_raw_buffer_load_b64(rp, vo4, (int)(o * K * 4), 0));
      mm[o] = ex.m_w ? __builtin_bit_cast(float2, __builtin_amdgcn_raw_buffer_load_b64(rm, vo4, (int)(o * K * 4), 0))
                     : make_float2(0.f, 0.f);
    }
  }
  const __amdgpu_buffer_rsrc_t rx = __builtin_amdgcn_make_buffer_rsrc(const_cast<T*>(X), (short)0, 0x7fffffff,
                                                                      0x00020000);
  unsigned xw[F32 ? 1 : MAXB];
  float2 xf[F32 ? MAXB : 1];
#pragma unroll
  for (int b = 0; b < MAXB; ++b) {
    if constexpr (F32)
      xf[b] = __builtin_bit_cast(float2, __builtin_amdgcn_raw_buffer_load_b64(rx, vo4, (int)((long)min(b, B - 1) * K * 4), 0));
    else
      xw[b] = (unsigned)__builtin_amdgcn_raw_buffer_load_b32(rx, vo2, (int)((long)min(b, B - 1) * K * 2), 0);
  }
  float acc[NO][2];
#pragma unroll
  for (int v = 0; v < VW; ++v) {
    __builtin_amdgcn_sched_barrier(0);
    float p[NO][2];
#pragma unroll
    for (int o = 0; o < NO; ++o) p[o][0] = p[o][1] = 0.f;
#pragma unroll
    for (int u = 0; u < RPV; ++u) {
      const int b = v + VW * u;
      if (b < MAXB && b < B) {
        const float x0 = F32 ? xf[F32 ? b : 0].x : __builtin_bit_cast(float, xw[F32 ? 0 : b] << 16);
        const float x1 = F32 ? xf[F32 ? b : 0].y : __builtin_bit_cast(float, xw[F32 ? 0 : b] & 0xffff0000u);
        const float4 d0 = *reinterpret_cast<const float4*>(s_dl + b * FCDW_LD);
        const float4 d1 = *reinterpret_cast<const float4*>(s_dl + b * FCDW_LD + 4);
        const float2 d2 = *reinterpret_cast<const float2*>(s_dl + b * FCDW_LD + 8);
        const float d[NO] = {d0.x, d0.y, d0.z, d0.w, d1.x, d1.y, d1.z, d1.w, d2.x, d2.y};
#pragma unroll
        for (int o = 0; o < NO; ++o) {
          p[o][0] = fmaf(d[o], x0, p[o][0]);
          p[o][1] = fmaf(d[o], x1, p[o][1]);
        }
      }
    }
#pragma unroll
    for (int o = 0; o < NO; ++o) {
      acc[o][0] = v == 0 ? p[o][0] : acc[o][0] + p[o][0];
      acc[o][1] = v == 0 ? p[o][1] : acc[o][1] + p[o][1];
    }
  }
  __builtin_amdgcn_sched_barrier(0);
  if (!active) return;
  const long frag0 = (ex.sh_frag || ex.sh_frag32) ? fcfrag_index((int)col, ex.frag_HW, ex.frag_C) : 0;
#pragma unroll
  for (int o = 0; o < NO; ++o) {
    const float g0 = acc[o][0] * scale, g1 = acc[o][1] * scale;
    const long idx = (long)o * K + col;
    if (dW) {
      if (ex.sys_store) {
        st_sys(dW + idx, g0);
        st_sys(dW + idx + 1, g1);
      } else {
        *reinterpret_cast<float2*>(dW + idx) = make_float2(g0, g1);
      }
    }
    if (ex.sgd.update) {
      float m0 = mm[o].x, m1 = mm[o].y;
      const float p0 = sgd_one(pp[o].x, g0, &m0, ex.sgd), p1 = sgd_one(pp[o].y, g1, &m1, ex.sgd);
      st_wt(reinterpret_cast<float2*>(ex.p_w + idx), make_float2(p0, p1));
      if (ex.m_w) *reinterpret_cast<float2*>(ex.m_w + idx) = make_float2(m0, m1);
      const unsigned pb = (unsigned)f2bf(p0) | ((unsigned)f2bf(p1) << 16);
      if (ex.sh_plain) st_wt(reinterpret_cast<unsigned*>(ex.sh_plain + idx), pb);
      if (ex.sh_frag) st_wt(reinterpret_cast<unsigned*>(ex.sh_frag + frag0 + (long)o * K), pb);
      if (ex.sh_frag32) st_wt(reinterpret_cast<float2*>(ex.sh_frag32 + frag0 + (long)o * K), make_float2(p0, p1));
    }
  }
}

template <typename T, bool MASK, bool XENT, int NOT, int WPB, int VW, int CPL, bool DXO = true>
__device__ __forceinline__ void fc_bwd_body(const float* __restrict__ dL, const T* __restrict__ X,
                                            const T* __restrict__ Wf, T* __restrict__ dX,
                                            float* __restrict__ dW, float scale, int B, long K, int NO_rt,
                                            const FcBwdExtras& ex, float* smem, int bx, int* ready) {
  static_assert(VW % WPB == 0, "virtual waves must be a multiple of the physical waves");
  constexpr int COLS = 64 * CPL, NT = WPB * 64, KV = VW / WPB;
  DDP_STAMP(STAMP_K_FC_BWD, 0);
  const int NO = NOT == 10 ? 10 : NO_rt;
  const int lane = threadIdx.x & 63, wave = threadIdx.x >> 6;
  float* s_dl = smem;
  float* s_loss = s_dl + B * NO;
  float* s_lg = s_loss + B;
  int* s_lab = reinterpret_cast<int*>(s_lg + B * NO);
  float* s_red = smem + (((XENT ? 2 * B * NO + B : B * NO) + B + 3) & ~3);

  const long col = (long)bx * COLS + CPL * lane;
  const bool active = col < K;
  const long cc = active ? col : 0;
  ColF<CPL> wr[DXO ? NOT : 1];
  if constexpr (DXO) {
#pragma unroll
    for (int o = 0; o < NOT; ++o) {
      if (o < NO) wr[o] = ldc<CPL>(Wf + (long)o * K + cc);
// ... 158 lines not shown
```

csrc/kernels/infer.hip:

```cpp
#include <stdexcept>

#include "kernels/conv3x3_fwd.h"
#include "kernels/xent_body.h"

namespace ddp_amd {

template <typename T, int NW>
__global__ __launch_bounds__(NW * 64, NW / 4) void simplecnn_infer_kernel(
    const T* __restrict__ Wt, const float* __restrict__ bias, const T* __restrict__ wfc,
    const float* __restrict__ fc_bias, int B, float* __restrict__ fc_part, int* __restrict__ img_cnt, C1Src c1,
    InferOut out) {
  constexpr int PXT = 1, NOF = 10, OCC = 1, GH = 28, GW = 28, GCI = 32, GCO = 64;
  constexpr bool RELU = true, A1X = true, DZ = false, MRG = false, NOA2 = true;
  const T* X = nullptr;
  T* Y = nullptr;
  int H = GH, W = GW, Cin = GCI, Cout = GCO;
  const FwdDz dzo{};
  const FwdMerge mg{};
  extern __shared__ __attribute__((aligned(16))) char smem[];
  const int bx = (int)blockIdx.x, by = 0;
#include "kernels/conv3x3_fwd_body.inc.h"
  if (wave != 0) return;
  const int img0 = (int)(P0 / HW);
  const long plast = (P0 + CH < Ptot ? P0 + CH : Ptot) - 1;
  const int nimg = (int)(plast / HW) - img0 + 1;
  float* s_lg = s_fc + NW * PXT * 4 * NOF;
  asm volatile("s_waitcnt vmcnt(0)" ::: "memory");
  bool last = false;
  if (lane < nimg) {
    const int im = img0 + lane;
    const int kb0 = im * HW / CH, kb1 = (im * HW + HW - 1) / CH;
    int* cnt = img_cnt + (long)im * FWD_DZ_CNT_STRIDE;
    const int prev = __hip_atomic_fetch_add(cnt, 1, __ATOMIC_RELAXED, __HIP_MEMORY_SCOPE_AGENT);
    last = prev == kb1 - kb0;
    if (last) __hip_atomic_store(cnt, 0, __ATOMIC_RELAXED, __HIP_MEMORY_SCOPE_AGENT);
  }
  const unsigned long long fin = __ballot(last);
  if (!fin) return;
  const int slot = lane >= NOF ? 1 : 0, o = lane - slot * NOF;
  const bool mine = lane < 2 * NOF && ((fin >> slot) & 1);
  const int im = img0 + slot;
  if (mine) {
    const float a = xent_logit_acc(im, o, HW, CH, NOF, [&](int i) {
      return __hip_atomic_load(fc_part + i, __ATOMIC_RELAXED, __HIP_MEMORY_SCOPE_AGENT);
    });
    const float lg = fc_bias[o] + a;
    s_lg[lane] = lg;
    if (out.logits) out.logits[(long)im * NOF + o] = lg;
  }
  asm volatile("s_waitcnt lgkmcnt(0)" ::: "memory");
  if (mine && o == 0) {
    const float* x = s_lg + slot * NOF;
    const int label = c1.labels[c1.bi.row(im, c1.bi.base())];
    float lossv = 0.f;
    (void)xent_row_dl(x, NOF, 0, label, 1.f, &lossv);
    int best = 0;
    float mx = x[0];
    for (int k = 1; k < NOF; ++k)
      if (x[k] > mx) { mx = x[k]; best = k; }
    out.pred[im] = best;
    out.correct[im] = best == label ? 1 : 0;
    out.loss_rows[im] = lossv;
  }
}

int infer_blocks(int B, int pxt) { return (int)(((long)B * 28 * 28 + 64 * pxt - 1) / (64 * pxt)); }

static size_t infer_lds(int pxt, int es) {
  return std::max(conv3x3_fwd_lds(28, 32, pxt, true, es), (size_t)(80 * 1024 + 16));
}

template <typename T>
static void infer_launch(const T* Wt, const float* bias, const T* wfc, const float* fc_bias, int B, int pxt,
                         const C1Src& c1, float* fc_part, int* img_cnt, const InferOut& out, hipStream_t s) {
  const char* bad = !Wt || !bias ? "the conv2 weight / bias" : !wfc || !fc_bias ? "the fc weight (FCFRAG order) / bias"
                    : !c1.x || !c1.labels || !c1.w || !c1.b ? "the images / labels / conv1 parameters"
                    : !fc_part || !img_cnt ? "its scratch" : !out.pred || !out.correct || !out.loss_rows ? "its outputs"
                    : nullptr;
  if (bad) throw std::runtime_error(std::string("simplecnn_infer: missing ") + bad);
  if (pxt != 1 && pxt != 2) throw std::runtime_error("simplecnn_infer: pxt must be 1 or 2");
  if (B <= 0 || (long)B * 28 * 28 >= (1L << 31)) throw std::runtime_error("simplecnn_infer: need 0 < B * 784 < 2^31");
  const size_t lds = infer_lds(pxt, (int)sizeof(T));
  const dim3 grid((unsigned)infer_blocks(B, pxt));
  if (pxt == 2) {
    auto k = simplecnn_infer_kernel<T, 8>;
    lds_optin(k, lds);
    hipLaunchKernelGGL(k, grid, dim3(512), lds, s, Wt, bias, wfc, fc_bias, B, fc_part, img_cnt, c1, out);
  } else {
    auto k = simplecnn_infer_kernel<T, 4>;
    lds_optin(k, lds);
    hipLaunchKernelGGL(k, grid, dim3(256), lds, s, Wt, bias, wfc, fc_bias, B, fc_part, img_cnt, c1, out);
  }
}

void simplecnn_infer(const bf16_t* Wt, const float* bias, const bf16_t* wfc, const float* fc_bias, int B, int pxt,
                     const C1Src& c1, float* fc_part, int* img_cnt, const InferOut& out, hipStream_t s) {
// ... 46 lines not shown
```

csrc/kernels/launchers.h:

```cpp
#pragma once
#include <hip/hip_runtime.h>
#include <stdint.h>

#include "kernels/types.h"

namespace ddp_amd {

void stamps_set(void* buf);

void conv1_fwd(const void* x, bool x_is_u8, BatchIdx bi, const float* w, const float* b, bf16_t* y,
               int B, int H, int W, int Cout, hipStream_t s);
void conv1_fwd(const void* x, bool x_is_u8, BatchIdx bi, const float* w, const float* b, float* y,
               int B, int H, int W, int Cout, hipStream_t s);
int conv1_wgrad_blocks(int B, int H, int W, int chunk);
void conv1_wgrad(const void* x, bool x_is_u8, BatchIdx bi, const bf16_t* dy, const bf16_t* yact,
                 float* slab, int B, int H, int W, int Cout, int chunk, hipStream_t s);
void conv1_wgrad(const void* x, bool x_is_u8, BatchIdx bi, const float* dy, const float* yact,
                 float* slab, int B, int H, int W, int Cout, int chunk, hipStream_t s);

constexpr int FWD_DZ_CNT_STRIDE = 64;
struct FwdDz {
  bf16_t* dz2 = nullptr;
  float* dz2_f32 = nullptr;
  unsigned long long* gran = nullptr;
// ... 238 lines not shown
void adamw_step(float* p, const float* g, float* mbuf, float* vbuf, long n, const AdamArgs& a,
                const ShadowSet& sh, hipStream_t s, const float* gscale, const float* coef, int n_coef,
                SchedState* sched);
constexpr int LARS_THREADS = 256, LARS_ITEM = 4096, LARS_CHUNK = 64, LARS_MAX_BLOCKS = 2048;
constexpr int LARS_MAX_SEGS = 4095;
int seg_sqnorm_blocks(int n_items);
void seg_sqnorm(const float* w, const float* g, long n, const LarsItem* items, int n_items, const LarsSeg* segs,
                int n_seg, float* partials, int* ticket, float* sums, float* trust, float trust_coef, float eps,
                const float* gscale, hipStream_t s);
void lars_step(float* p, const float* g, float* mbuf, long n, const SgdArgs& a, const ShadowSet& sh,
               const short* cmap, const float* trust, int n_seg, hipStream_t s, const float* gscale = nullptr,
               const float* lr_table = nullptr, int n_table = 0, SchedState* sched = nullptr);
void ema_step(float* e, const float* p, long n, float om, int* num_updates, hipStream_t s,
              const float* table = nullptr, int n_table = 0, SchedState* sched = nullptr);
void ema_swap(float* p, float* e, long n, const ShadowSet& sh, hipStream_t s);
constexpr int GN_THREADS = 256, GN_QUADS = 4, GN_MAX_BLOCKS = 1024;
struct ClipStats {
  float total_norm;
  float coef;
  int steps;
  int clipped;
};
int grad_norm_blocks(long n);
void grad_sqnorm(const float* g, long n, float max_norm, float* partials, int* ticket, ClipStats* out,
                 hipStream_t s);
void grad_reduce(const SlabSet& ss, hipStream_t s);
int grad_reduce_groups(const SlabSet& ss);
void scale_copy(float* dst, const float* src, long n, float scale, hipStream_t s);

constexpr int XGMI_MAX_RANKS = 8, XGMI_THREADS = 256, XGMI_MAX_BLOCKS = 1024;
constexpr int XGMI_GRID_CAP = 256;
constexpr int XGMI_FLAG_OFF = 0;
constexpr int XGMI_SEQ_OFF = XGMI_MAX_BLOCKS * XGMI_MAX_RANKS;
constexpr int XGMI_ERR_OFF = XGMI_SEQ_OFF + XGMI_MAX_BLOCKS;
constexpr int XGMI_SIG_WORDS = XGMI_ERR_OFF + 64;
enum { XGMI_PHASE_B0 = 0, XGMI_PHASE_B1 = 1, XGMI_PHASE_ONESHOT = 2 };
__host__ __device__ constexpr unsigned xgmi_error_code(int block, int peer, int phase) {
  return 0x80000000u | ((unsigned)block << 12) | ((unsigned)(peer & 0xff) << 4) | (unsigned)(phase & 0xf);
}
constexpr double XGMI_DEFAULT_TIMEOUT_S = 30.0;
struct XgmiArgs {
  float* data[XGMI_MAX_RANKS];
  float* stage[XGMI_MAX_RANKS];
  unsigned* sig[XGMI_MAX_RANKS];
  long off, n, slice;
  int oneshot;
  int publish;
  float scale;
  float prescale;
  int rank, world;
  unsigned long long timeout_ticks;
  SgdArgs sgd;
  float* params;
  float* mbuf;
  ShadowSet sh;
  int* step_ctr;
};
long xgmi_slice(long n, int world);
int xgmi_blocks(long n, int world, bool oneshot = false);
long xgmi_stage_floats(long n, int world, bool oneshot);
void xgmi_allreduce(const XgmiArgs& a, int blocks, hipStream_t s);
constexpr int XGMI_GROUP_MAX_BLOCKS = 64;
bool xgmi_allreduce_group(const XgmiArgs* args, int world, int nblk, bool wt, hipStream_t s);

struct BwdXar {
  const XgmiArgs* args = nullptr;
  int nblk0 = 0, nblk1 = 0;
  int* fc_done = nullptr;
  int* red_done = nullptr;
  int* xar_done = nullptr;
  int fc_expect = 0, red_expect = 0;
  int* step_ctr = nullptr;
  int* err = nullptr;
};
constexpr int XAR_ERR = 4;
constexpr int RED_ERR = 2;
constexpr int FWD_DZ_ERR = 3;
constexpr int HEAD_ERR = 5;
void xgmi_allreduce_pair(const BwdXar& x, hipStream_t s);
bool conv3x3_step_head(const BwdXar& x, int* done_fc, int* done_conv, const bf16_t* Wt, const float* bias,
                       bf16_t* Y, int B, const bf16_t* wfc, float* fc_part, const C1Src& c1, const FwdDz& dz,
                       int* err, hipStream_t s, const ShadowSet* late = nullptr);
bool conv3x3_step_head_fits(int nx, int B);
int conv3x3_step_head_slots();

}
```

csrc/kernels/optim.hip:

```cpp
#include "kernels/common.h"
#include "kernels/flat_step.h"
#include "kernels/launchers.h"
#include "kernels/shadow.h"
#include "kernels/slab_reduce.h"

namespace ddp_amd {

struct SgdRule {
  float* mbuf;
  SgdArgs a;
  __device__ __forceinline__ float4 quad(long q, float4 v, float4 d) const {
    float4 m = {0.f, 0.f, 0.f, 0.f};
    if (a.momentum != 0.f) m = reinterpret_cast<const float4*>(mbuf)[q];
    v.x = sgd_one(v.x, d.x, &m.x, a);
    v.y = sgd_one(v.y, d.y, &m.y, a);
    v.z = sgd_one(v.z, d.z, &m.z, a);
    v.w = sgd_one(v.w, d.w, &m.w, a);
    if (a.momentum != 0.f) reinterpret_cast<float4*>(mbuf)[q] = m;
    return v;
  }
  __device__ __forceinline__ float one(long i, float v, float d) const {
    float m = (a.momentum != 0.f) ? mbuf[i] : 0.f;
    v = sgd_one(v, d, &m, a);
    if (a.momentum != 0.f) mbuf[i] = m;
// ... 42 lines not shown

void sgd_step(float* p, const float* g, float* mbuf, long n, const SgdArgs& a, const ShadowSet& sh,
              int* step_ctr, hipStream_t s, const float* gscale, const float* lr_table, int n_table,
              SchedState* sched) {
  const bool dlr = sched != nullptr && lr_table != nullptr && n_table > 0;
  auto kernel = gscale ? (dlr ? sgd_kernel<true, true> : sgd_kernel<true, false>)
                       : (dlr ? sgd_kernel<false, true> : sgd_kernel<false, false>);
  hipLaunchKernelGGL(kernel, dim3(flat_grid(n)), dim3(FLAT_THREADS), 0, s, p, g, mbuf, n, a, sh, step_ctr, gscale,
                     lr_table, n_table, sched);
}

__global__ void noop_kernel(int* __restrict__ sink) {
  if (sink && blockIdx.x == 0 && threadIdx.x == 0) sink[0] = 0;
}

void noop(int blocks, int* sink, hipStream_t s) {
  hipLaunchKernelGGL(noop_kernel, dim3(blocks), dim3(256), 0, s, sink);
}

__global__ __launch_bounds__(256) void slab_reduce_rows_kernel(SlabSeg sg) {
  const long n4 = sg.n >> 2;
  const long stride = (long)gridDim.x * blockDim.x;
  for (long q = (long)blockIdx.x * blockDim.x + threadIdx.x; q < n4; q += stride) {
    const float* src = sg.slab + sg.src_off + 4 * q;
    float4 g[4];
#pragma unroll
    for (int u = 0; u < 4; ++u) g[u] = make_float4(0.f, 0.f, 0.f, 0.f);
    for (int r0 = 0; r0 < sg.rows; r0 += 4) {
#pragma unroll
      for (int u = 0; u < 4; ++u) {
        if (r0 + u < sg.rows) {
          const float4 b = *reinterpret_cast<const float4*>(src + (long)(r0 + u) * sg.row_stride);
          g[u].x += b.x; g[u].y += b.y; g[u].z += b.z; g[u].w += b.w;
        }
      }
    }
    float4 a = g[0];
#pragma unroll
    for (int u = 1; u < 4; ++u) { a.x += g[u].x; a.y += g[u].y; a.z += g[u].z; a.w += g[u].w; }
    float4* d = reinterpret_cast<float4*>(sg.dst + 4 * q);
    if (sg.accum) {
      const float4 o = *d;
      a.x = fmaf(a.x, sg.scale, o.x); a.y = fmaf(a.y, sg.scale, o.y);
      a.z = fmaf(a.z, sg.scale, o.z); a.w = fmaf(a.w, sg.scale, o.w);
    } else {
      a.x *= sg.scale; a.y *= sg.scale; a.z *= sg.scale; a.w *= sg.scale;
    }
    *d = a;
  }
}

int grad_reduce_groups(const SlabSet& ss) {
  int max_rows = 0;
  for (int k = 0; k < ss.count; ++k) max_rows = ss.s[k].rows > max_rows ? ss.s[k].rows : max_rows;
  return max_rows >= 64 ? 16 : 4;
}

void grad_reduce(const SlabSet& ss, hipStream_t s) {
  if (ss.count == 1 && !ss.sgd.update && !ss.sys_store && !ss.step_ctr && ss.s[0].rows <= 16 &&
      ss.s[0].n % 4 == 0 && ss.s[0].row_stride % 4 == 0 && ss.s[0].src_off % 4 == 0 &&
      ((uintptr_t)ss.s[0].slab & 15) == 0 && ((uintptr_t)ss.s[0].dst & 15) == 0) {
    const long b = (ss.s[0].n / 4 + 255) / 256;
    hipLaunchKernelGGL(slab_reduce_rows_kernel, dim3((unsigned)(b < 4096 ? b : 4096)), dim3(256), 0, s, ss.s[0]);
    return;
  }
  const long blocks = slab_chunks(ss);
  if (blocks == 0) return;
  if (grad_reduce_groups(ss) == 16)
    hipLaunchKernelGGL(grad_reduce_kernel<16>, dim3((unsigned)blocks), dim3(1024), 0, s, ss);
  else
    hipLaunchKernelGGL(grad_reduce_kernel<4>, dim3((unsigned)blocks), dim3(256), 0, s, ss);
}

void scale_copy(float* dst, const float* src, long n, float scale, hipStream_t s) {
  const long blocks = (n + 255) / 256;
  const unsigned grid = (unsigned)(blocks < 1024 ? (blocks > 0 ? blocks : 1) : 1024);
  hipLaunchKernelGGL(scale_copy_kernel, dim3(grid), dim3(256), 0, s, dst, src, n, scale);
}

DDP_STAMPS_SETTER(stamps_set_optim)
void stamps_set_conv1(void*);
void stamps_set_conv3x3(void*);
void stamps_set_conv3x3_bwd(void*);
void stamps_set_linear(void*);
void stamps_set_xent(void*);
void stamps_set_allreduce(void*);
void stamps_set_infer(void*);
void stamps_set(void* p) {
  stamps_set_optim(p);
  stamps_set_conv1(p);
  stamps_set_conv3x3(p);
  stamps_set_conv3x3_bwd(p);
  stamps_set_linear(p);
  stamps_set_xent(p);
  stamps_set_allreduce(p);
  stamps_set_infer(p);
}

}
```

csrc/runtime/engine.cpp:

```cpp
#include <algorithm>
#include <cstdio>
#include <cstdlib>
#include <cstring>
#include <type_traits>

#include "runtime/runtime.h"

namespace ddp_amd {

SimpleCNNEngine::SimpleCNNEngine(const EngineConfig& cfg, const EngineBuffers& buf,
                                 std::shared_ptr<Comm> comm, std::vector<EngineBucket> buckets)
    : cfg_(cfg), b_(buf), comm_(std::move(comm)), buckets_(std::move(buckets)) {
  if (cfg_.C1 != 32) throw std::runtime_error("engine: fused conv1 wgrad needs C1 == 32");
  if (cfg_.C2 % 64 != 0) throw std::runtime_error("engine: C2 must be a multiple of 64");
  if ((cfg_.H * cfg_.W) % 16 != 0) throw std::runtime_error("engine: H*W must be a multiple of 16");
  if (cfg_.NO != 10) throw std::runtime_error("engine: the fused fc epilogue is built for 10 classes");
  if (cfg_.f32 && (cfg_.fuse_level < 1 || cfg_.store_a1 != 0))
    throw std::runtime_error("engine: fp32 mode needs fuse_level >= 1 (level 1 or 3) and store_a1 0");
  if (cfg_.f32 && !(b_.a2_f32 && b_.dz2_f32 && b_.w2t_f32 && b_.wfc_frag32))
    throw std::runtime_error("engine: fp32 mode needs the a2 / dz2 / w2t / wfc_frag32 fp32 buffers");
  const long conv0 = std::min(std::min(b_.off_w2, b_.off_b2), std::min(b_.off_w1, b_.off_b1));
  const long fc_hi = std::max(b_.off_wfc + (long)cfg_.NO * cfg_.H * cfg_.W * cfg_.C2, b_.off_bfc + cfg_.NO);
  if (fc_hi > conv0) throw std::runtime_error("engine: fc gradients must precede the conv gradients");
  long prev_end = 0;
  for (const EngineBucket& bk : buckets_) {
    if (bk.n <= 0 || bk.off < prev_end || bk.off + bk.n > b_.n_params)
      throw std::runtime_error("engine: bucket plan out of range / overlapping / unordered");
    prev_end = bk.off + bk.n;
    stage_.push_back(bk.off + bk.n <= conv0 ? 0 : 1);
  }
  last_bucket_ = (int)buckets_.size() - 1;
  for (int s : stage_) stage_used_[s] = true;
  xch_.assign(buckets_.size(), -1);
  DDP_HIP_CHECK(hipStreamCreateWithFlags(&cs_, hipStreamNonBlocking));
  DDP_HIP_CHECK(hipStreamCreateWithFlags(&ms_, hipStreamNonBlocking));
  for (hipEvent_t* e : {&e_b0_, &e_b1_, &e_d0_, &e_d1_, &e_fwd_, &e_fc_})
    DDP_HIP_CHECK(hipEventCreateWithFlags(e, hipEventDisableTiming));
  l3_fits_.assign(cfg_.max_batch + 1, -1);
  if (b_.sync_err) {
    DDP_HIP_CHECK(hipHostMalloc(reinterpret_cast<void**>(&err_host_), sizeof(int),
                                hipHostMallocCoherent | hipHostMallocMapped));
    *err_host_ = 0;
    int* dev = nullptr;
    DDP_HIP_CHECK(hipHostGetDevicePointer(reinterpret_cast<void**>(&dev), err_host_, 0));
    b_.sync_err = dev;
  }
  if (cfg_.fuse_level >= 3 && b_.sync_flags && b_.sync_err) {
    const size_t ng = 2 * (size_t)cfg_.NO * (size_t)conv3x3_dgrad_blocks(cfg_.max_batch, cfg_.H, cfg_.W, 1);
    DDP_HIP_CHECK(hipMalloc(reinterpret_cast<void**>(&gran_), ng * sizeof(unsigned long long)));
    DDP_HIP_CHECK(hipMalloc(reinterpret_cast<void**>(&gen_), 256));
    DDP_HIP_CHECK(hipMemset(gran_, 0, ng * sizeof(unsigned long long)));
    DDP_HIP_CHECK(hipMemset(gen_, 0, 256));
    DDP_HIP_CHECK(hipStreamSynchronize(nullptr));
  }
}

SimpleCNNEngine::~SimpleCNNEngine() {
  if (process_exiting()) return;
  if (cs_) hipStreamSynchronize(cs_);
  destroy_graph();
  for (hipEvent_t e : {e_b0_, e_b1_, e_d0_, e_d1_, e_fwd_, e_fc_}) hipEventDestroy(e);
  for (XarArgs& e : xar_cache_) hipFree(const_cast<XgmiArgs*>(e.dev));
  if (err_host_) hipHostFree(err_host_);
  if (gran_) hipFree(gran_);
  if (gen_) hipFree(gen_);
}

void SimpleCNNEngine::destroy_graph() {
  if (graph_exec_) hipGraphExecDestroy(graph_exec_);
  if (graph_) hipGraphDestroy(graph_);
  graph_exec_ = nullptr;
  graph_ = nullptr;
  graph_steps_ = 0;
}

void SimpleCNNEngine::synchronize() {
  DDP_HIP_CHECK(hipStreamSynchronize(cs_));
  if (const int e = sync_error()) {
    throw std::runtime_error(std::string("engine: an in-launch hand-off wait timed out (") +
                             (e == RED_ERR ? "fused slab reduction" : e == XAR_ERR ? "in-launch all-reduce"
                              : e == HEAD_ERR ? "dist_mode 4 step head: forward waiting for the bucket all-reduce"
                                              : "level-3 forward dZ2") +
                             "); results invalid");
  }
}

bool SimpleCNNEngine::sync_ok_for_xar() const { return b_.sync_flags != nullptr && b_.sync_err != nullptr; }

StepPlan SimpleCNNEngine::plan(int batch) {
  StepFacts f;
  f.xgmi = xgmi_ != nullptr;
  f.xgmi_world = xgmi_ ? xgmi_->world() : 1;
  f.comm = comm_ != nullptr;
  f.comm_world = comm_ ? comm_->world() : 1;
  f.sync_flags = b_.sync_flags != nullptr;
  f.sync_err = b_.sync_err != nullptr;
  if (cfg_.fuse_level >= 3 && batch > 0 && batch <= cfg_.max_batch) {
    signed char& fit = l3_fits_[batch];
    if (fit < 0)
      fit = conv3x3_fwd_dz_fits(batch, cfg_.H, cfg_.W, cfg_.pxt_fwd, cfg_.f32 ? 4 : 2) && cfg_.C1 == 32 &&
                    cfg_.C2 == 64
                ? 1 : 0;
    f.l3_fits = fit == 1;
  }
  f.fc_role_ok = conv3x3_bwd_fc_role_ok(cfg_.H, cfg_.W, cfg_.C1, cfg_.C2, cfg_.pxt_dgrad, cfg_.wgrad_split);
  f.xar_plan_ok = xar_plan_ok_;
  return plan_step(cfg_, f, batch);
}

ShadowSet SimpleCNNEngine::shadow_set(bool plain_fc) const {
  const int HW = cfg_.H * cfg_.W, C1 = cfg_.C1, C2 = cfg_.C2;
  const long n_w2 = (long)C2 * 9 * C1, n_fc = (long)cfg_.NO * HW * C2;
  ShadowSet sh{};
  if (cfg_.f32) {
    sh.r[0] = ShadowRegion{b_.off_w2, n_w2, nullptr, SHADOW_F32_TAPT, C2, 9, C1, b_.w2t_f32};
    sh.r[1] = ShadowRegion{b_.off_wfc, n_fc, nullptr, SHADOW_F32_FCFRAG, HW, C2, 0, b_.wfc_frag32};
    sh.count = 2;
    return sh;
  }
  sh.r[0] = ShadowRegion{b_.off_w2, n_w2, b_.w2_bf16, SHADOW_BF16, 0, 0, 0};
  sh.r[1] = ShadowRegion{b_.off_w2, n_w2, b_.w2t_bf16, SHADOW_BF16_TAPT, C2, 9, C1};
  sh.r[2] = ShadowRegion{b_.off_wfc, n_fc, b_.wfc_frag, SHADOW_BF16_FCFRAG, HW, C2, 0};
  sh.r[3] = ShadowRegion{b_.off_wfc, n_fc, b_.wfc_bf16, SHADOW_BF16, 0, 0, 0};
  sh.count = plain_fc ? 4 : 3;
  return sh;
}

void SimpleCNNEngine::refresh_shadows() {
  const SgdArgs a{0.f, 0.f, 0.f, 0.f, 0, 0, 0, 0};
  sgd_step(b_.params, b_.grads, nullptr, b_.n_params, a, shadow_set(true), nullptr, cs_);
  DDP_HIP_CHECK(hipGetLastError());
}

namespace {

template <typename T>
struct StepOperands {
  const T* w2;
  const T* w2t;
  T* a2;
  T* dz2;
  const T* wfc_frag;
  const T* wfc;
  T* a1;
  ShadowSet sh;
};

template <typename T>
StepOperands<T> step_operands(const EngineBuffers& b, const ShadowSet& sh) {
  if constexpr (std::is_same<T, float>::value)
    return {b.params + b.off_w2, b.w2t_f32, b.a2_f32, b.dz2_f32, b.wfc_frag32, b.params + b.off_wfc, nullptr, sh};
  else
    return {b.w2_bf16, b.w2t_bf16, b.a2, b.dz2, b.wfc_frag, b.wfc_bf16, b.a1, sh};
}

}

void SimpleCNNEngine::launch_step(int B, int stride, bool first_momentum_step, unsigned parts) {
  if (cfg_.f32)
    launch_step_t<float>(B, stride, first_momentum_step, parts);
  else
    launch_step_t<bf16_t>(B, stride, first_momentum_step, parts);
}

C1Src SimpleCNNEngine::make_c1src(int B, int stride, const StepPlan& pl) const {
  C1Src c1;
  c1.x = b_.images;
  c1.bi = BatchIdx{b_.idx, b_.step_ctr, stride, 0};
  c1.bi.n_idx = b_.n_idx;
  c1.bi.n_rows = b_.n_rows;
  c1.w = b_.params + b_.off_w1;
  c1.b = b_.params + b_.off_b1;
  c1.xb_out = b_.xb;
  c1.yb_out = b_.yb;
  c1.labels = b_.labels;
  if (cfg_.store_a1) c1.a1_out = b_.a1;
  if (pl.fred || pl.l3 || pl.pair_mode) {
    const int nfwd = conv3x3_dgrad_blocks(B, cfg_.H, cfg_.W, cfg_.pxt_fwd);
    const int nsync = SYNC_RED_INTS + ((pl.l3 || pl.pair_mode) ? L3_FC_INTS : 0);
    c1.zero_i32 = b_.sync_flags;
    c1.zero_per_block = (nsync + nfwd - 1) / nfwd;
    c1.zero_total = nsync;
  }
  return c1;
}

// ... 50 lines not shown
      ex.zero_i32 = b_.sync_flags + L3_HEAD_OFF;
      ex.n_zero = 2;
      ex.zero_stride = FWD_DZ_CNT_STRIDE;
    }
  }
  if (pl.fc_role) {
    if (pl.fopt) {
      ex.p_b = P + b_.off_bfc;
      ex.m_b = M ? M + b_.off_bfc : nullptr;
    }
    if (pl.fopt || pl.ov) ex.step_inc = b_.step_ctr;
  }
  return ex;
}

SlabSet SimpleCNNEngine::make_slabs(int B, const StepPlan& pl, const SgdArgs& sa) const {
  const int C1 = cfg_.C1, C2 = cfg_.C2, NO = cfg_.NO;
  const long n_w2 = (long)C2 * 9 * C1, w2row = n_w2 + C2;
  const float inv_ws = 1.f / (float)cfg_.world;
  float* G = b_.grads;
  SlabSet ss{};
  const int wblk = conv3x3_wgrad_blocks(B, cfg_.H, cfg_.wgrad_rows);
  ss.s[0] = SlabSeg{b_.w2slab, w2row, 0, n_w2, wblk, G + b_.off_w2, inv_ws};
  ss.s[1] = SlabSeg{b_.w2slab, w2row, n_w2, (long)C2, wblk, G + b_.off_b2, inv_ws};
  const int dblk = conv3x3_dgrad_blocks(B, cfg_.H, cfg_.W, cfg_.pxt_dgrad);
  ss.s[2] = SlabSeg{b_.w1slab, 320, 0, (long)C1 * 9, dblk, G + b_.off_w1, inv_ws};
  ss.s[3] = SlabSeg{b_.w1slab, 320, (long)C1 * 9, (long)C1, dblk, G + b_.off_b1, inv_ws};
  ss.count = 4;
  if (pl.fopt) {
    auto opt = [&](SlabSeg& sg, long off) {
      sg.p = b_.params + off;
      sg.m = b_.momentum ? b_.momentum + off : nullptr;
    };
    opt(ss.s[0], b_.off_w2);
    if (cfg_.f32) {
      ss.s[0].sh_t32 = b_.w2t_f32;
    } else {
      ss.s[0].sh = b_.w2_bf16;
      ss.s[0].sh_t = b_.w2t_bf16;
    }
    ss.s[0].t_co = C2; ss.s[0].t_taps = 9; ss.s[0].t_ci = C1;
    opt(ss.s[1], b_.off_b2);
    opt(ss.s[2], b_.off_w1);
    opt(ss.s[3], b_.off_b1);
    ss.sgd = sa;
    if (!pl.fc_role) {
      ss.s[4] = SlabSeg{G + b_.off_bfc, (long)NO, 0, (long)NO, 1, G + b_.off_bfc, 1.f};
      opt(ss.s[4], b_.off_bfc);
      ss.count = 5;
      ss.step_ctr = b_.step_ctr;
    }
  }
  ss.sys_store = pl.use_x ? 1 : 0;
  return ss;
}

bool SimpleCNNEngine::launch_step_head(int B, const SgdArgs& sa, const ShadowSet& sh, const C1Src& c1,
                                       const FwdDz& dzo) {
  ShadowSet sh_head = sh, late{};
  if (late_shadow_ok(b_.off_w2, (long)cfg_.C2 * 9 * cfg_.C1)) {
    sh_head.r[1] = sh.r[2];
    sh_head.count = 2;
    late.r[0] = sh.r[1];
    late.count = 1;
  }
  BwdXar hx;
  int* mc = b_.sync_flags + L3_HEAD_OFF;
  bool head_used = false;
  if (cfg_.pxt_fwd == 1 && B == cfg_.max_batch) {
    if (!make_xar(hx, sa, b_.momentum, sh_head)) throw std::runtime_error("engine: the step head needs the pair plan");
    hx.step_ctr = nullptr;
    head_used = conv3x3_step_head(hx, mc, mc + FWD_DZ_CNT_STRIDE, b_.w2_bf16, b_.params + b_.off_b2, b_.a2, B,
                                  b_.wfc_frag, b_.fc_part, c1, dzo, b_.sync_err, cs_, &late);
  }
  if (!head_used) {
    if (!make_xar(hx, sa, b_.momentum, sh)) throw std::runtime_error("engine: the step head needs the pair plan");
    hx.step_ctr = nullptr;
    xgmi_allreduce_pair(hx, cs_);
  }
  DDP_HIP_CHECK(hipGetLastError());
  return head_used;
}

template <typename T>
void SimpleCNNEngine::launch_step_t(int B, int stride, bool first_momentum_step, unsigned parts) {
  constexpr bool BF16 = std::is_same<T, bf16_t>::value;
  if (!BF16 && parts != PART_ALL) throw std::runtime_error("engine: the fp32 step runs whole (no step-head merge)");
  const int H = cfg_.H, W = cfg_.W, HW = H * W, C1 = cfg_.C1, C2 = cfg_.C2, NO = cfg_.NO;
  if (B <= 0 || B > cfg_.max_batch) throw std::runtime_error("engine: bad batch size");
  const StepPlan pl = plan(B);
  if ((parts & (PART_HEAD | PART_AR)) && !pl.ov && parts != PART_ALL)
    throw std::runtime_error("engine: a split step needs the dist_mode 4 chain");
  if (BF16 && !pl.l3 && plain_stale_) {
    refresh_shadows();
    plain_stale_ = false;
  }
  const StepOperands<T> op = step_operands<T>(b_, shadow_set(!pl.l3));
  float* P = b_.params;
  float* G = b_.grads;
  float* M = b_.momentum;
  const float inv_ws = 1.f / (float)cfg_.world;
  const SgdArgs sa{cfg_.lr, cfg_.momentum, cfg_.dampening, cfg_.weight_decay, cfg_.nesterov,
                   cfg_.maximize, first_momentum_step ? 1 : 0, 1};

  const C1Src c1 = make_c1src(B, stride, pl);
  const FwdDz dzo = pl.l3 ? make_fwd_dz(B) : FwdDz{};
  bool head_used = false;
  if constexpr (BF16) {
    if (parts & PART_HEAD) {
      if (first_momentum_step) throw std::runtime_error("engine: the step head runs the steady-state SGD only");
      head_used = launch_step_head(B, sa, op.sh, c1, dzo);
    }
  }
  if ((parts & PART_FWD) || ((parts & PART_HEAD) && !head_used)) {
    if constexpr (BF16) {
      if (!pl.f1) conv1_fwd(b_.images, true, c1.bi, P + b_.off_w1, P + b_.off_b1, b_.a1, B, H, W, C1, cs_);
    }
    conv3x3_fwd(pl.f1 ? nullptr : op.a1, op.w2, P + b_.off_b2, op.a2, B, H, W, C1, C2, true, op.wfc_frag,
                b_.fc_part, NO, cfg_.pxt_fwd, cs_, pl.f1 ? &c1 : nullptr, pl.l3 ? &dzo : nullptr);
  }
  if (parts & (PART_FWD | PART_HEAD)) last_head_ = head_used;
  if (head_used && capturing_) graph_heads_ += 1;
  if (!(parts & (PART_BWD | PART_AR))) return;

  if constexpr (BF16) {
    if (!pl.f1)
      xent_rows(b_.fc_part, HW, 64 * cfg_.pxt_fwd, P + b_.off_bfc, NO, B, b_.labels, c1.bi, b_.dlogits,
                b_.loss_rows, 1.f / (float)B, cs_);
  }
  const FcBwdExtras ex = make_fc_extras(B, pl, sa);
  float* dWfc = pl.fopt ? nullptr : G + b_.off_wfc;
  const long K = (long)HW * C2;
  BwdFc fcr;
  std::function<void(hipStream_t)> fc_launch;
  if (pl.fc_role) {
    fcr.a2 = op.a2;
    fcr.dl = b_.dlogits;
    fcr.dW = dWfc;
    fcr.scale = inv_ws;
    fcr.K = K;
    fcr.ex = ex;
  } else {
    fc_launch = [&](hipStream_t s) {
      fc_bwd(b_.dlogits, op.a2, pl.l3 ? nullptr : op.wfc, pl.l3 ? nullptr : op.dz2, dWfc, inv_ws, B, K, NO,
             true, s, ex);
    };
  }
  if (BF16 && pl.l3) plain_stale_ = true;

  const SlabSet ss = make_slabs(B, pl, sa);

  C1Src c1b;
  c1b.x = b_.xb;
  c1b.bi = BatchIdx{nullptr, nullptr, 0, 0};
  c1b.bi.n_rows = B;
  c1b.w = c1.w;
  c1b.b = c1.b;
  bool reduced = false;
  BwdXar xa;
  const bool want_xar = pl.xar_wanted && make_xar(xa, sa, M, op.sh);
  if (pl.use_x && pl.l3 && cfg_.dist_mode == 2 && !want_xar && std::getenv("DDP_AMD_XAR_DEBUG"))
    fprintf(stderr, "[ddp_amd] in-launch all-reduce off: plan_ok %d fc_role %d fred %d buckets %d\n",
            (int)xar_plan_ok_, (int)pl.fc_role, (int)pl.fred, (int)buckets_.size());
  bool xar_used = false, pair_used = false;
  auto conv_launch = [&]() {
    if (!(parts & PART_BWD)) {
    } else if (pl.f1) {
      reduced = conv3x3_bwd(op.dz2, op.w2t, nullptr, b_.w1slab, b_.w2slab, B, H, W, C1, C2, cfg_.pxt_dgrad,
                            cfg_.wgrad_rows, c1b, cfg_.store_a1 ? op.a1 : nullptr, cfg_.store_a1 == 2, cs_,
                            pl.fred ? &ss : nullptr, b_.sync_flags, b_.sync_err, cfg_.wgrad_split,
                            pl.fc_role ? &fcr : nullptr, !pl.dist && cfg_.fuse_reduce == 2,
                            want_xar ? &xa : nullptr, &xar_used);
    } else if constexpr (BF16) {
      conv3x3_dgrad(b_.dz2, nullptr, b_.w2t_bf16, b_.a1, b_.dz1, B, H, W, C1, C2, b_.images, true, c1.bi,
                    b_.w1slab, cfg_.pxt_dgrad, cs_, nullptr);
      conv3x3_wgrad(b_.dz2, nullptr, b_.a1, b_.w2slab, B, H, W, C1, C2, cfg_.wgrad_rows, cs_, nullptr);
    }
    if (!reduced && (parts & PART_BWD)) grad_reduce(ss, cs_);
    if (pl.one_stream && !xar_used && (parts & PART_AR)) {
      BwdXar pr;
      if (cfg_.dist_mode >= 3 && make_xar(pr, sa, M, op.sh)) {
        if (pl.ov) pr.step_ctr = nullptr;
        xgmi_allreduce_pair(pr, cs_);
        pair_used = true;
        DDP_HIP_CHECK(hipGetLastError());
      } else {
        enqueue_buckets(0, pl.use_x, cs_, sa, M, op.sh);
        enqueue_buckets(1, pl.use_x, cs_, sa, M, op.sh);
      }
    }
  };
// ... 218 lines not shown
```

csrc/runtime/runtime.h:

```cpp
#pragma once
#include <hip/hip_runtime.h>
#include <rccl/rccl.h>

#include <functional>
#include <memory>
#include <stdexcept>
#include <string>
#include <vector>

#include "kernels/launchers.h"
#include "runtime/bucket_state.h"
#include "runtime/step_plan.h"

#define DDP_HIP_CHECK(expr)                                                              \
  do {                                                                                   \
    hipError_t _e = (expr);                                                              \
    if (_e != hipSuccess)                                                                \
      throw std::runtime_error(std::string("HIP error ") + hipGetErrorString(_e) + " at " + \
                               __FILE__ + ":" + std::to_string(__LINE__) + ": " #expr);  \
  } while (0)

#define DDP_NCCL_CHECK(expr)                                                             \
  do {                                                                                   \
    ncclResult_t _r = (expr);                                                            \
// ... 142 lines not shown
class Reducer {
 public:
  Reducer(std::shared_ptr<Comm> comm, float* flat_grad, std::vector<long> param_offsets,
          std::vector<long> param_numels, std::vector<int> param_bucket,
          std::vector<long> bucket_offsets, std::vector<long> bucket_numels, bool prescale);
  void set_xgmi(std::shared_ptr<XgmiComm> x, std::vector<int> channels);
  int world() const;
  ~Reducer();
  void mark_ready(int param, const float* grad_src, hipStream_t compute);
  void finalize(hipStream_t compute);
  void reset();
  int num_buckets() const { return (int)bucket_off_.size(); }
  long allreduce_calls() const { return calls_; }

 private:
  void launch_bucket(int b, hipStream_t compute);
  std::shared_ptr<Comm> comm_;
  std::shared_ptr<XgmiComm> xgmi_;
  std::vector<int> xch_;
  float* flat_;
  std::vector<long> poff_, pnum_;
  std::vector<int> pbucket_;
  std::vector<long> bucket_off_, bucket_num_;
  BucketState state_;
  std::vector<hipEvent_t> ready_, done_;
  hipStream_t comm_stream_ = nullptr;
  bool prescale_;
  long calls_ = 0;
};

struct EngineBuffers {
  float* params;
  float* grads;
  float* momentum;
  long n_params;
  long off_w1, off_b1, off_w2, off_b2, off_wfc, off_bfc;
  bf16_t *w2_bf16, *w2t_bf16, *wfc_bf16, *wfc_frag;
  float *a2_f32 = nullptr, *dz2_f32 = nullptr, *w2t_f32 = nullptr;
  float* wfc_frag32 = nullptr;
  bf16_t *a1, *a2, *dz2, *dz1;
  float *fc_part, *dlogits, *loss_rows, *loss_hist, *w2slab, *w1slab;
  int* step_ctr;
  unsigned char* xb;
  int* yb;
  int* sync_flags = nullptr;
  int* sync_err = nullptr;
  const unsigned char* images;
  const int* labels;
  const int* idx;
  int n_idx, n_rows;
};

constexpr int L3_FC_INTS = 32;
constexpr int L3_HEAD_OFF = SYNC_RED_INTS + L3_FC_INTS;

struct EngineBucket {
  long off, n;
};

class SimpleCNNEngine {
 public:
  SimpleCNNEngine(const EngineConfig& cfg, const EngineBuffers& buf, std::shared_ptr<Comm> comm,
                  std::vector<EngineBucket> buckets);
  ~SimpleCNNEngine();
  void step(int batch, int batch_stride);
  void refresh_shadows();
  void set_lr(float lr) { cfg_.lr = lr; }
  void capture(int nsteps);
  void replay();
  bool has_graph() const { return graph_exec_ != nullptr; }
  int graph_steps() const { return graph_steps_; }
  void destroy_graph();
  hipStream_t stream() const { return cs_; }
  void synchronize();
  int sync_error() const { return err_host_ ? __atomic_load_n(err_host_, __ATOMIC_ACQUIRE) : 0; }
  bool level3_active(int batch) { return plan(batch).l3; }
  bool overlap_active() { return plan(cfg_.max_batch).ov && pair_plan_ok_ && cfg_.pxt_fwd == 1; }
  bool last_fused_reduce() const { return last_fused_reduce_; }
  bool last_level3() const { return last_level3_; }
  bool last_fc_role() const { return last_fc_role_; }
  bool last_xar() const { return last_xar_; }
  bool last_pair() const { return last_pair_; }
  bool last_head() const { return last_head_; }
  int graph_heads() const { return graph_heads_; }
  void set_momentum_started(bool v) { momentum_started_ = v; }
  void set_xgmi(std::shared_ptr<XgmiComm> x, std::vector<int> channels);
  int num_buckets() const { return (int)buckets_.size(); }
  int bucket_stage(int b) const { return stage_.at(b); }

 private:
  enum : unsigned { PART_FWD = 1, PART_BWD = 2, PART_AR = 4, PART_HEAD = 8, PART_ALL = 7 };
  void launch_step(int batch, int batch_stride, bool first_momentum_step, unsigned parts = PART_ALL);
  template <typename T>
  void launch_step_t(int batch, int batch_stride, bool first_momentum_step, unsigned parts);
  StepPlan plan(int batch);
  ShadowSet shadow_set(bool plain_fc) const;
  C1Src make_c1src(int B, int stride, const StepPlan& pl) const;
  FwdDz make_fwd_dz(int B) const;
  FcBwdExtras make_fc_extras(int B, const StepPlan& pl, const SgdArgs& sa) const;
  SlabSet make_slabs(int B, const StepPlan& pl, const SgdArgs& sa) const;
  bool launch_step_head(int B, const SgdArgs& sa, const ShadowSet& sh, const C1Src& c1, const FwdDz& dzo);
  void launch_buckets(int stage, bool use_x, const SgdArgs& sa, float* M, const ShadowSet& sh);
  void join_buckets();
  void enqueue_buckets(int stage, bool use_x, hipStream_t s, const SgdArgs& sa, float* M, const ShadowSet& sh);
  void schedule_backward(bool dist, bool fork, bool use_x, const std::function<void(hipStream_t)>& fc,
                         const std::function<void()>& conv, const SgdArgs& sa, float* M, const ShadowSet& sh);
  bool late_shadow_ok(long off, long n) const;
  bool make_xar(BwdXar& xa, const SgdArgs& sa, float* M, const ShadowSet& sh);
  bool sync_ok_for_xar() const;
  EngineConfig cfg_;
  EngineBuffers b_;
  std::shared_ptr<Comm> comm_;
  std::shared_ptr<XgmiComm> xgmi_;
  std::vector<EngineBucket> buckets_;
  std::vector<int> stage_;
  std::vector<int> xch_;
  int last_bucket_ = -1;
  bool stage_used_[2] = {false, false};
  hipStream_t cs_ = nullptr, ms_ = nullptr;
  hipEvent_t e_b0_, e_b1_, e_d0_, e_d1_, e_fwd_, e_fc_;
  std::vector<signed char> l3_fits_;
  hipGraph_t graph_ = nullptr;
  hipGraphExec_t graph_exec_ = nullptr;
  int graph_steps_ = 0;
  bool momentum_started_ = false;
  bool last_fused_reduce_ = false;
  bool last_level3_ = false;
  bool last_fc_role_ = false;
  bool last_xar_ = false;
  bool last_pair_ = false;
  bool last_head_ = false;
  bool capturing_ = false;
  int graph_heads_ = 0;
  bool xar_plan_ok_ = false;
  bool pair_plan_ok_ = false;
  struct XarArgs {
    XgmiArgs host[2];
    const XgmiArgs* dev = nullptr;
  };
  std::vector<XarArgs> xar_cache_;
  hipStream_t xs_ = nullptr;
  bool plain_stale_ = false;
  int* err_host_ = nullptr;
  unsigned long long* gran_ = nullptr;
  unsigned* gen_ = nullptr;
};

}
```

csrc/runtime/step_plan.h:

```cpp
#pragma once

namespace ddp_amd {

struct EngineConfig {
  int max_batch, H, W, C1, C2, NO;
  int pxt_fwd, pxt_dgrad, wgrad_rows;
  int world, rank;
  float lr, momentum, dampening, weight_decay;
  int nesterov, maximize;
  int force_allreduce;
  int fuse_level = 0;
  int l3_fc_role = 1;
  int fuse_opt = 1;
  int store_a1 = 0;
  int f32 = 0;
  int fuse_reduce = 1;
  int wgrad_split = 1;
  int dist_mode = 3;
};

struct StepFacts {
  bool xgmi = false;
  int xgmi_world = 1;
  bool comm = false;
  int comm_world = 1;
  bool sync_flags = false, sync_err = false;
  bool l3_fits = false;
  bool fc_role_ok = false;
  bool xar_plan_ok = false;
};

struct StepPlan {
  bool use_x;
  bool dist;
  bool f1;
  bool l3;
  bool fred;
  bool pair_mode;
  bool xar_mode;
  bool one_stream;
  bool fc_role;
  bool ov;
  bool fopt;
  bool fork;
  bool xar_wanted;
};

inline StepPlan plan_step(const EngineConfig& c, const StepFacts& f, int B) {
  StepPlan p{};
  p.use_x = f.xgmi && (f.xgmi_world > 1 || c.force_allreduce);
  p.dist = p.use_x || (f.comm && (f.comm_world > 1 || c.force_allreduce));
  p.f1 = c.fuse_level >= 1;
  p.l3 = c.fuse_level >= 3 && f.sync_flags && f.sync_err && B > 0 && B <= c.max_batch && f.l3_fits;
  p.fred = p.f1 && c.fuse_reduce && f.sync_flags;
  p.pair_mode = p.dist && p.use_x && p.f1 && c.dist_mode >= 3 && f.sync_flags && f.sync_err;
  p.xar_mode = p.dist && p.use_x && p.l3 && ((c.dist_mode == 2 && f.xar_plan_ok) || c.dist_mode >= 3);
  p.one_stream = p.xar_mode || p.pair_mode;
  p.fc_role = p.l3 && (!p.dist || p.xar_mode) && c.l3_fc_role && f.fc_role_ok;
  p.ov = !c.f32 && p.dist && p.use_x && p.l3 && p.fc_role && c.dist_mode == 4;
  p.fopt = !p.dist && c.fuse_opt;
  p.fork = p.dist && p.l3 && c.dist_mode == 1;
  p.xar_wanted = p.xar_mode && c.dist_mode == 2 && p.fc_role && p.fred;
  return p;
}

}
```

pytorch-distributed-data-parallel-ddp-trainer_amd/_build.py:

```python
from __future__ import annotations

import concurrent.futures as _cf
import glob
import hashlib
import json
import mmap
import os
import shutil
import subprocess
import sys
import sysconfig

PKG_DIR = os.path.dirname(os.path.abspath(__file__))
REPO_DIR = os.path.dirname(PKG_DIR)
CSRC = os.path.join(REPO_DIR, "csrc")
BUILD_DIR = os.path.join(REPO_DIR, "build", "native")
SO_PATH = os.path.join(PKG_DIR, "_C.so")
ARCH = os.environ.get("DDP_AMD_ARCH", "gfx950")


def _torch_dirs():
    import torch

    tdir = os.path.dirname(torch.__file__)
    return tdir, os.path.join(tdir, "include"), os.path.join(tdir, "lib")


def _hipcc() -> str:
    for cand in (os.environ.get("HIPCC"), shutil.which("hipcc"), "/opt/rocm/bin/hipcc"):
        if cand and os.path.exists(cand):
            return cand
    raise RuntimeError("hipcc not found (ROCm toolchain required to build ddp_amd._C)")


def _headers_mtime() -> float:
    hs = glob.glob(os.path.join(CSRC, "**", "*.h"), recursive=True)
    hs += glob.glob(os.path.join(CSRC, "**", "*.cuh"), recursive=True)
    return max((os.path.getmtime(h) for h in hs), default=0.0)


def _deps(obj: str):
    try:
        with open(obj + ".d") as f:
            text = f.read().replace("\\\n", " ")
    except OSError:
        return None
    files = text.split(":", 1)[1].split() if ":" in text else []
    return [f for f in files if os.path.abspath(f).startswith(CSRC + os.sep)]


def _needs(obj: str, src: str, hdr_mtime: float, cmd=None) -> bool:
    if not os.path.exists(obj):
        return True
    if cmd is not None:
        try:
            with open(obj + ".cmd") as f:
                if f.read() != " ".join(cmd):
                    return True
        except OSError:
            return True
    t = os.path.getmtime(obj)
    deps = _deps(obj)
    if deps is not None:
        return any(not os.path.exists(d) or os.path.getmtime(d) > t for d in [src, *deps])
    return os.path.getmtime(src) > t or hdr_mtime > t


KERNEL_FLAGS = {"conv3x3.hip": ["-fno-slp-vectorize"], "conv3x3_bwd.hip": ["-fno-slp-vectorize"],
                "infer.hip": ["-fno-slp-vectorize"]}
COMMON_FLAGS = ["-O3", "-fPIC", "-std=c++17", "-D__HIP_PLATFORM_AMD__"]
DEVICE_FLAGS = ["-munsafe-fp-atomics"]
BIND_FLAGS = ["-O2", "-DUSE_ROCM", "-DTORCH_EXTENSION_NAME=_C", "-DTORCH_API_INCLUDE_EXTENSION_H"]
SOURCE_EXTS = (".hip", ".cpp", ".h", ".cuh", ".hpp")
HASH_MARKER = b"DDP_AMD_SRC_HASH="
HASH_LEN = 40


def source_hash(csrc: str = CSRC) -> str:
    h = hashlib.sha256()
    files = sorted(p for p in glob.glob(os.path.join(csrc, "**", "*"), recursive=True)
                   if os.path.isfile(p) and p.endswith(SOURCE_EXTS))
    for p in files:
        h.update(os.path.relpath(p, csrc).replace(os.sep, "/").encode() + b"\0")
        with open(p, "rb") as f:
            h.update(f.read())
        h.update(b"\0")
    sig = dict(arch=ARCH, common=COMMON_FLAGS, device=DEVICE_FLAGS, kernel=KERNEL_FLAGS, bind=BIND_FLAGS)
    h.update(json.dumps(sig, sort_keys=True).encode())
    return h.hexdigest()[:HASH_LEN]


def binary_hash(so_path: str = SO_PATH) -> str | None:
    try:
        with open(so_path, "rb") as f, mmap.mmap(f.fileno(), 0, access=mmap.ACCESS_READ) as mm:
            i = mm.find(HASH_MARKER)
            if i < 0:
                return None
            return mm[i + len(HASH_MARKER):i + len(HASH_MARKER) + HASH_LEN].decode("ascii", "replace")
    except (OSError, ValueError):
        return None


def _hash_source_file() -> str:
    path = os.path.join(BUILD_DIR, "source_hash.cpp")
    text = ("// generated by _build.py: the sources this binary was built from\n"
            f'extern "C" const char ddp_amd_source_hash_str[] = "{HASH_MARKER.decode()}{source_hash()}";\n')
    try:
        with open(path) as f:
            if f.read() == text:
                return path
    except OSError:
        pass
    with open(path, "w") as f:
        f.write(text)
    return path


def _compile_cmds():
    hipcc = _hipcc()
    _, tinc, _ = _torch_dirs()
    rocm_inc = os.path.join(os.environ.get("ROCM_PATH", "/opt/rocm"), "include")
    common = [*COMMON_FLAGS, "-I", rocm_inc, "-I", CSRC]
    cmds = []
    for src in sorted(glob.glob(os.path.join(CSRC, "kernels", "*.hip"))):
        obj = os.path.join(BUILD_DIR, "k_" + os.path.basename(src) + ".o")
        cmds.append((src, obj, [hipcc, f"--offload-arch={ARCH}", *common, *KERNEL_FLAGS.get(os.path.basename(src), []),
                                *DEVICE_FLAGS, "-MD", "-MF", obj + ".d", "-c", src, "-o", obj]))
    for src in sorted(glob.glob(os.path.join(CSRC, "runtime", "*.cpp"))):
        obj = os.path.join(BUILD_DIR, "r_" + os.path.basename(src) + ".o")
        cmds.append((src, obj, [hipcc, *common, "-x", "c++", "-MD", "-MF", obj + ".d", "-c", src, "-o", obj]))
    bsrc = os.path.join(CSRC, "bindings.cpp")
    bobj = os.path.join(BUILD_DIR, "bindings.o")
    hsrc = _hash_source_file()
    cmds.append((hsrc, os.path.join(BUILD_DIR, "source_hash.o"), ["g++", "-fPIC", "-c", hsrc, "-o",
                                                                  os.path.join(BUILD_DIR, "source_hash.o")]))
    cmds.append((bsrc, bobj, [
        hipcc, *common[:-2], "-x", "c++", "-I", CSRC, *BIND_FLAGS,
        f"-D_GLIBCXX_USE_CXX11_ABI={int(_cxx11_abi())}",
        "-I", tinc, "-I", os.path.join(tinc, "torch", "csrc", "api", "include"),
        "-I", sysconfig.get_paths()["include"], "-w", "-MD", "-MF", bobj + ".d", "-c", bsrc, "-o", bobj]))
    return cmds


def _cxx11_abi() -> bool:
    import torch

    return bool(torch._C._GLIBCXX_USE_CXX11_ABI)


def build(verbose: bool = False, jobs: int | None = None, force: bool = False) -> str:
    os.makedirs(BUILD_DIR, exist_ok=True)
    hdr = _headers_mtime()
# ... 41 lines not shown
```

pytorch-distributed-data-parallel-ddp-trainer_amd/engine/fused_step.py:

```python
from __future__ import annotations

import dataclasses
import os
import math

import torch

from .. import native
from ..data.loader import DeviceMNIST
from ..data.sampler import ShardedSampler
from ..models.layers import flat_space
from ..ops.functional import wgrad_rows
from ..parallel.ddp import bucket_plan, bucket_ranges

from ..parallel.bucket_model import ONESHOT_MAX_ELEMS

BF16 = torch.bfloat16


@dataclasses.dataclass
class EngineOptions:
    graph_steps: int = 100
    use_graph: bool = True
    pxt_fwd: int | None = None
    pxt_dgrad: int = 2
    wgrad_rows: int | None = None
    bucket_cap_mb: float = 25.0
    first_bucket_mb: float = 1.0
    bucket_plan: str = "model"
    force_allreduce: bool = False
    fuse_level: int = 3
    l3_fc_role: int = 1
    fuse_opt: bool = True
    fuse_reduce: int | None = None
    store_a1: int | None = None
    comm: str = "auto"
    epoch_order: bool = True
    dtype: str = "bf16"
    wgrad_split: int = 2
    dist_mode: int = 4
    xar_blocks: int = 96
    plan_world: int | None = None
    cost_fit: dict | None = None


def agree(store, key: str, rank: int, world: int, ok: bool) -> bool:
    if store is None or world <= 1:
        return bool(ok)
    store.set(f"{key}/{rank}", b"1" if ok else b"0")
    return all(store.get(f"{key}/{r}") == b"1" for r in range(world))



def gather_rank_sum(local: torch.Tensor, world: int) -> torch.Tensor:
    import torch.distributed as dist

    src = local.detach().float().contiguous()
    if world <= 1 or not dist.is_initialized():
        return src.cpu().clone()
    if dist.get_backend() == "gloo":
        src = src.cpu()
    parts = [torch.empty_like(src) for _ in range(world)]
    dist.all_gather(parts, src)
    acc = parts[0].cpu().clone()
    for p in parts[1:]:
        acc += p.cpu()
    return acc


def oracle_mismatches(reduced: torch.Tensor, oracle: torch.Tensor, ranges) -> int:
    r = reduced.detach().float().cpu().contiguous()
    o = oracle.detach().float().cpu().contiguous()
    bad = 0
    for off, n in ranges:
        bad += int((r[off:off + n].view(torch.int32) != o[off:off + n].view(torch.int32)).sum())
    return bad


PLACEMENT_NAMES = {0: "serial", 1: "fork", 3: "pair", 4: "step head"}


def placement_candidates(comm_kind: str, dtype: str = "bf16") -> tuple:
    if comm_kind.startswith("xgmi"):
        return (4, 3, 0, 1) if dtype == "bf16" else (3, 0, 1)
    if comm_kind.startswith("rccl"):
        return (0, 1)
    return ()


def choose_placement(all_times) -> tuple:
    modes = sorted(set().union(*[set(t) for t in all_times]))
    worst = {}
    for m in modes:
        vals = [t.get(m) for t in all_times]
        worst[m] = None if any(v is None for v in vals) else max(vals)
    ok = {m: v for m, v in worst.items() if v is not None}
    if not ok:
        return None, worst
    return min(ok, key=lambda m: (ok[m], m)), worst


def agree_placement(store, key: str, rank: int, world: int, mine: dict) -> tuple:
    import json

    if store is None or world <= 1:
        return choose_placement([mine])
    store.set(f"{key}/{rank}", json.dumps({str(k): v for k, v in mine.items()}).encode())
    allt = [{int(k): v for k, v in json.loads(store.get(f"{key}/{r}").decode()).items()} for r in range(world)]
    return choose_placement(allt)


def chain_decision(same_all: bool, xgmi_ok_all: bool, oracle_ok_all: bool, have_rccl: bool) -> str:
    if not xgmi_ok_all or not oracle_ok_all:
        return "rccl" if have_rccl else "fail"
    return "keep" if same_all else "conservative"
# ... 8 lines not shown
        self.B = int(batch_size)
        pf1 = self.opts.dtype == "bf16" and bool(self.C.conv3x3_fwd_dz_fits(self.B, 28, 28, 1))
        if self.opts.pxt_fwd is None:
            self.opts.pxt_fwd = 1 if pf1 else 2
        if self.opts.dist_mode == 4 and pf1 and (world_size > 1 or self.opts.force_allreduce):
            self.opts.pxt_fwd = 1
        self.world_size, self.rank = world_size, rank
        self.fs = fs = flat_space(model)
        dev = fs.params.device
        if dev.type != "cuda":
            raise RuntimeError("the fused engine runs on a HIP device")
        names = {"w1": "net.0.weight", "b1": "net.0.bias", "w2": "net.2.weight",
                 "b2": "net.2.bias", "wfc": "fl.weight", "bfc": "fl.bias"}
        from ..parallel.bucket_model import XgmiCost, engine_plan

        pw = self.opts.plan_world or world_size
        if self.opts.cost_fit is not None:
            self.cost = XgmiCost.from_fit(pw, self.opts.cost_fit,
                                          source=f"fit:{self.opts.cost_fit.get('topology', 'job')}")
        else:
            self.cost = XgmiCost.calibrated(pw)
        if self.opts.bucket_plan == "model":
            self.buckets, self.pred_comm_us = engine_plan(fs, pw, self.cost)
        elif self.opts.bucket_plan == "torch":
            self.buckets, self.pred_comm_us = bucket_plan(fs, self.opts.bucket_cap_mb, self.opts.first_bucket_mb), None
        else:
            raise ValueError(f"bucket_plan must be model|torch, got {self.opts.bucket_plan!r}")
        ranges = bucket_ranges(fs, self.buckets)
        offs = {k: fs.offsets[v] for k, v in names.items()}
        offs["buckets"] = [(int(o), int(n)) for o, n in ranges]
        self.sampler = ShardedSampler(len(data), world_size, rank, shuffle=True, seed=seed)
        n_rank = len(self.sampler)
        B, HW = self.B, 28 * 28
        if self.opts.dtype not in ("bf16", "fp32"):
            raise ValueError(f"engine dtype must be bf16 or fp32, got {self.opts.dtype!r}")
        f32 = self.opts.dtype == "fp32"
        self.store_a1 = self.opts.store_a1 if self.opts.store_a1 is not None else (0 if f32 else 1)
        if f32 and (self.opts.fuse_level < 1 or self.store_a1 != 0):
            raise ValueError("the fp32 engine runs the level-1 or level-3 chain (fuse_level >= 1, store_a1 0)")
        R = self.wgrad_rows = self.opts.wgrad_rows or wgrad_rows(28, B, torch.float32 if f32 else BF16)
        g = self.opt.param_groups[0]
        if g["momentum"] != 0 and self.opt.momentum_buffer is None:
            self.opt.momentum_buffer = torch.zeros_like(fs.params)
        e = lambda *s, dt=torch.float32: torch.empty(*s, dtype=dt, device=dev)
        self.steps_per_epoch = math.ceil(n_rank / B)
        if f32:
            act = dict(a2=e(B * HW * 64), dz2=e(B * HW * 64), w2t_f32=e(64 * 9 * 32),
                       wfc_frag32=e(10 * HW * 64))
        else:
            act = dict(w2_bf16=e(64 * 9 * 32, dt=BF16), w2t_bf16=e(64 * 9 * 32, dt=BF16),
                       wfc_bf16=e(10 * HW * 64, dt=BF16), wfc_frag=e(10 * HW * 64, dt=BF16),
                       a1=e(B * HW * 32, dt=BF16), a2=e(B * HW * 64, dt=BF16),
                       dz2=e(B * HW * 64, dt=BF16), dz1=e(B * HW * 32, dt=BF16))
        self.t = dict(
            params=fs.params, grads=fs.grads,
            momentum=self.opt.momentum_buffer if self.opt.momentum_buffer is not None else e(1),
            **act,
            fc_part=e(2 * self.C.conv3x3_dgrad_blocks(B, 28, 28, self.opts.pxt_fwd) * 10),
            dlogits=e(B * 10), loss_rows=e(B),
            loss_hist=torch.zeros(self.steps_per_epoch + 1, device=dev),
            w2slab=e(self.C.conv3x3_wgrad_blocks(B, 28, R) * (64 * 9 * 32 + 64)),
            w1slab=e(self.C.conv3x3_dgrad_blocks(B, 28, 28, self.opts.pxt_dgrad) * 320),
            step_ctr=torch.zeros(1, dtype=torch.int32, device=dev),
            xb=torch.empty(B * HW, dtype=torch.uint8, device=dev),
            yb=torch.empty(B, dtype=torch.int32, device=dev),
            images=(torch.empty(n_rank * HW, dtype=torch.uint8, device=dev) if self.opts.epoch_order
                    else data.images_u8.view(-1)),
            labels=(torch.empty(n_rank, dtype=torch.int32, device=dev) if self.opts.epoch_order
                    else data.labels_i32),
            idx=torch.zeros(n_rank, dtype=torch.int32, device=dev),
        )
        nfl = 256 + 32 + 64 * 2
        self.t["sync_flags"] = torch.zeros(nfl, dtype=torch.int32, device=dev)
        self.t["sync_err"] = torch.zeros(1, dtype=torch.int32, device=dev)
        cfg = dict(max_batch=B, H=28, W=28, C1=32, C2=64, NO=10, pxt_fwd=self.opts.pxt_fwd,
                   pxt_dgrad=self.opts.pxt_dgrad, wgrad_rows=R, world=world_size, rank=rank,
                   lr=float(g["lr"]), momentum=float(g["momentum"]),
                   dampening=float(g["dampening"]), weight_decay=float(g["weight_decay"]),
                   nesterov=bool(g["nesterov"]), maximize=bool(g["maximize"]),
                   force_allreduce=bool(self.opts.force_allreduce),
                   fuse_level=self._fuse_level_ok(world_size), fuse_opt=bool(self.opts.fuse_opt),
                   store_a1=int(self.store_a1), f32=f32, fuse_reduce=self._fuse_reduce_ok(world_size),
                   epoch_order=bool(self.opts.epoch_order), wgrad_split=int(self.opts.wgrad_split),
                   l3_fc_role=int(self.opts.l3_fc_role), dist_mode=int(self.opts.dist_mode))
        self.dtype = "fp32" if f32 else "bf16"
        use_comm = world_size > 1 or self.opts.force_allreduce
        self.xgmi = None
        self.xgmi_plan = None
        self.allreduce_us = None
        xch = list(range(len(ranges)))
        if use_comm and self.opts.comm in ("auto", "tune", "xgmi", "xgmi1", "xgmi2"):
            from ..parallel.xgmi import channel_plan, create_xgmi, pick_data_plane

            lim = self.cost.oneshot_cap_elems()
            oneshot = tuple(b for b, (_, n) in enumerate(ranges) if n <= lim)
            from ..parallel.xgmi import ENGINE_GRID_CAP

            cap = int(self.opts.xar_blocks) if self.opts.dist_mode == 2 else ENGINE_GRID_CAP
            self.xgmi = create_xgmi(fs.grads, ranges, rank, world_size, oneshot=oneshot, grid_cap=cap)
            if self.xgmi is not None and self.opts.comm in ("xgmi1", "xgmi2"):
                plan = "xgmi1" if self.opts.comm == "xgmi1" else "xgmi"
            elif self.xgmi is not None and self.opts.comm in ("auto", "xgmi"):
                plan = "xgmi1" if oneshot else "xgmi"
            elif self.xgmi is not None:
                from ..parallel.xgmi import rccl_candidate_comms

                variants = rccl_candidate_comms(rank, world_size) if comm is not None else {}
                plan, self.allreduce_us, chosen = pick_data_plane(
                    self.xgmi, comm, fs.grads, ranges, rank, oneshot=oneshot, rccl_variants=variants)
                if plan.startswith("rccl"):
                    comm = chosen
                variants = {k: c for k, c in variants.items() if c is comm}
                del variants
            if self.xgmi is not None:
                self.xgmi_plan = plan
                if plan.startswith("rccl"):
                    self.xgmi = None
                else:
                    cp = channel_plan(len(ranges), oneshot)
                    xch = [cp[(b, plan == "xgmi1" and b in oneshot)] for b in range(len(ranges))]
        if use_comm and self.xgmi is None and comm is None:
            raise RuntimeError("world size > 1 needs an RCCL communicator or the xGMI path")
        self.comm_kind = ((self.xgmi_plan or "xgmi") if self.xgmi is not None
                          else ((self.xgmi_plan if (self.xgmi_plan or "").startswith("rccl") else "rccl")
                                if use_comm else "none"))
        self.ranges, self.xch, self.comm = ranges, xch, (comm if use_comm else None)
        self.cfg, self.offs = cfg, offs
        self.chain_check = None
        self.eng = self.C.SimpleCNNEngine(cfg, self.t, offs, comm if use_comm else None)
        if self.xgmi is not None:
            self.eng.set_xgmi(self.xgmi, xch)
        if self.opt.momentum_buffer is not None and self.opt.steps > 0:
            self.eng.set_momentum_started(True)
        self.stream = torch.cuda.ExternalStream(self.eng.stream, device=dev)
        self.level3 = bool(self.eng.level3_active(B))
        self._captured = 0
        self.steps_done = 0
        self._need_barrier = world_size > 1
        self._evaluators = {}

    def conservative_cfg(self) -> dict | None:
        ref = dict(self.cfg, fuse_level=min(int(self.cfg["fuse_level"]), 1), fuse_reduce=0)
        return None if ref == self.cfg else ref

    def verify_chain(self, nsteps: int = 2, store=None, _corrupt_rank: int | None = None,
                     _corrupt_oracle_rank: int | None = None) -> bool:
        ref_cfg = self.conservative_cfg()
        if ref_cfg is None and self.xgmi is None:
            self.chain_check = {"ran": False, "reason": "production chain is the conservative one"}
            return True
        if ref_cfg is None:
            ref_cfg = dict(self.cfg)
        import torch.distributed as dist

        if store is None and dist.is_initialized() and self.world_size > 1:
            store = dist.distributed_c10d._get_default_store()
        t = self.t
        keys = ("params", "momentum", "step_ctr", "loss_hist")
        self.synchronize()
        torch.cuda.synchronize()
        snap = {k: t[k].clone() for k in keys}
        started = self.opt.momentum_buffer is not None and self.opt.steps > 0
        B = self.B

        def restore(e):
            with torch.cuda.stream(self.stream):
                for k in keys:
                    t[k].copy_(snap[k])
            torch.cuda.synchronize()
            e.set_momentum_started(started)
            e.refresh_shadows()
            torch.cuda.synchronize()

        head = bool(self.eng.overlap_active())
        if head:
            nsteps = max(nsteps, 3)

        def run(e, graph=False):
            self.start_epoch(0)
            restore(e)
            try:
                if graph:
                    left = nsteps
                    if self.opt.momentum_buffer is not None and not started:
                        e.step(B, B)
                        left -= 1
                    e.capture(left)
                    e.replay()
                else:
                    for _ in range(nsteps):
                        e.step(B, B)
                e.synchronize()
            except RuntimeError as ex:
                return None, f"in-launch wait: {ex}"
            if self.xgmi is not None and self.xgmi.error_flags():
                from ..parallel.xgmi import describe_xgmi_error

                return None, "xgmi: " + describe_xgmi_error(self.xgmi.error_flags())
            torch.cuda.synchronize()
            return [t[k].clone() for k in ("params", "momentum")] + [t["loss_hist"][:nsteps].clone()], None

        ref = self.C.SimpleCNNEngine(ref_cfg, t, self.offs, self.comm)
        if self.xgmi is not None:
            ref.set_xgmi(self.xgmi, self.xch)
        got, err_p = run(self.eng, graph=head)
        heads_checked = int(self.eng.graph_heads) if head else 0
        if head:
            self.eng.destroy_graph()
            self._captured = 0
        if got is not None and _corrupt_rank == self.rank:
            got[0][0] = torch.nextafter(got[0][0], torch.tensor(float("inf"), device=got[0].device))
        pair_ran = bool(self.eng.last_pair)
        want, err_r = run(ref)
        same = got is not None and want is not None and all(torch.equal(a, b) for a, b in zip(got, want))
        xgmi_bad = (err_p or "").startswith("xgmi") or (err_r or "").startswith("xgmi")
        oracle = {"ran": False}
        oracle_ok = True
        if self.xgmi is not None and not xgmi_bad:
# ... 308 lines not shown
```

Measured before the change: 1.007 million images/sec.

## Fuse forward and backward of the single-GPU training step into one persistent launch

Adds a step_one kernel that runs the level-3 forward, loss, FC backward, conv backward and fused reduction/optimizer in a single launch. In-kernel atomic counters hand data from the forward to the backward, and cross-block data is read with cache-bypassing buffer loads and written with write-through stores. It is enabled by default for non-distributed bf16 runs when the resident grid fits. The aim is to remove a kernel launch boundary and its idle gap at batch 32. In exchange it relies on spin-waits with timeouts and on all blocks being co-resident, which risks stalls or error fallbacks.

Measured after the change: 936,100 images/sec. -7.0%, worse.

```diff
diff --git a/csrc/bindings.cpp b/csrc/bindings.cpp
--- a/csrc/bindings.cpp
+++ b/csrc/bindings.cpp
@@ -1224,6 +1224,7 @@
   m.def("transpose_w", &op_transpose_w);
   m.def("rccl_version", []() { int v = 0; ncclGetVersion(&v); return v; });
   m.def("step_head_slots", &conv3x3_step_head_slots);
+  m.def("step_one_fits", &conv3x3_step_one_fits);
   m.def("source_hash", []() {
     const std::string s(ddp_amd_source_hash_str);
     const size_t eq = s.find('=');
@@ -1443,6 +1444,8 @@
              c.wgrad_split = cfgd.contains("wgrad_split") ? cfgd["wgrad_split"].cast<int>() : 1;
              c.l3_fc_role = cfgd.contains("l3_fc_role") ? cfgd["l3_fc_role"].cast<int>() : 1;
              c.dist_mode = cfgd.contains("dist_mode") ? cfgd["dist_mode"].cast<int>() : 3;
+             c.one_launch = cfgd.contains("one_launch") ? cfgd["one_launch"].cast<int>() : 1;
+             TORCH_CHECK(c.one_launch == 0 || c.one_launch == 1, "engine: one_launch must be 0 or 1");
              TORCH_CHECK(c.dist_mode >= 0 && c.dist_mode <= 4, "engine: dist_mode must be 0..4");
              TORCH_CHECK(c.l3_fc_role == 0 || c.l3_fc_role == 1, "engine: l3_fc_role must be 0 or 1");
              TORCH_CHECK(c.wgrad_split == 1 || c.wgrad_split == 2, "engine: wgrad_split must be 1 or 2");
@@ -1539,6 +1542,9 @@
       .def_property_readonly("last_pair", &SimpleCNNEngine::last_pair)
       .def_property_readonly("last_head", &SimpleCNNEngine::last_head)
       .def_property_readonly("graph_heads", &SimpleCNNEngine::graph_heads)
+      .def_property_readonly("last_one", &SimpleCNNEngine::last_one)
+      .def_property_readonly("one_refused", &SimpleCNNEngine::one_refused)
+      .def("one_active", &SimpleCNNEngine::one_active)
       .def("overlap_active", &SimpleCNNEngine::overlap_active)
       .def("level3_active", &SimpleCNNEngine::level3_active, py::arg("batch"))
       .def_property_readonly("sync_error", &SimpleCNNEngine::sync_error)
diff --git a/csrc/kernels/common.h b/csrc/kernels/common.h
--- a/csrc/kernels/common.h
+++ b/csrc/kernels/common.h
@@ -55,6 +55,12 @@
 
 __device__ __forceinline__ bf16x8 ld16(const void* p) { return *reinterpret_cast<const bf16x8*>(p); }
 __device__ __forceinline__ void st16(void* p, bf16x8 v) { *reinterpret_cast<bf16x8*>(p) = v; }
+__device__ __forceinline__ bf16x8 ld16_sc1(__amdgpu_buffer_rsrc_t r, int byte_off) {
+  return __builtin_bit_cast(bf16x8, __builtin_amdgcn_raw_buffer_load_b128(r, byte_off, 0, 16 ));
+}
+__device__ __forceinline__ __amdgpu_buffer_rsrc_t whole_rsrc(const void* p) {
+  return __builtin_amdgcn_make_buffer_rsrc(const_cast<void*>(p), (short)0, 0x7fffffff, 0x00020000);
+}
 
 struct F32Frag {
   f32x4 lo, hi;
diff --git a/csrc/kernels/conv3x3_body.h b/csrc/kernels/conv3x3_body.h
--- a/csrc/kernels/conv3x3_body.h
+++ b/csrc/kernels/conv3x3_body.h
@@ -66,7 +66,7 @@
 __host__ __device__ inline size_t fc_epi_lds(int pxt, int nof) { return sizeof(float) * 4 * pxt * 4 * nof; }
 
 template <typename T, int PXT, bool MASK_DY, bool MASK_X, bool FUSE_W1, bool A1X, int GH, int GW, int GCI,
-          int GCO, int WGS = 0>
+          int GCO, int WGS = 0, bool SC1 = false>
 __device__ __forceinline__ void dgrad_body(
     const T* __restrict__ dY, const T* __restrict__ Yact, const T* __restrict__ WT,
     const T* __restrict__ Xact, T* __restrict__ dX, int B, int H, int W, int Cin, int Cout,
@@ -131,7 +131,8 @@
             const long Pq = Pbase + r;
             bf16x8 v = zero8();
             if (Pq >= 0 && Pq < Ptot) {
-              v = ld16(dY + Pq * Cout + c);
+              if constexpr (SC1) v = ld16_sc1(whole_rsrc(dY), (int)((Pq * Cout + c) * (long)sizeof(T)));
+              else v = ld16(dY + Pq * Cout + c);
               if (MASK_DY) v = mask16<T>(v, ld16(Yact + Pq * Cout + c));
             }
             return v;
@@ -193,6 +194,10 @@
         if constexpr (F32) {
           const float4 x4 = *reinterpret_cast<const float4*>(xp);
           xa[pt][t][0] = x4.x; xa[pt][t][1] = x4.y; xa[pt][t][2] = x4.z; xa[pt][t][3] = x4.w;
+        } else if constexpr (SC1) {
+          unpack4(__builtin_bit_cast(uint2, __builtin_amdgcn_raw_buffer_load_b64(
+                      whole_rsrc(Xact), (int)((Pc * Cin + ci_blk + 16 * t + 4 * (lane >> 4)) * (long)sizeof(T)), 0, 16)),
+                  xa[pt][t]);
         } else {
           unpack4(*reinterpret_cast<const uint2*>(xp), xa[pt][t]);
         }
@@ -343,7 +348,8 @@
       dY, Yact, WT, Xact, dX, B, H, W, Cin, Cout, x0, x0_u8, bi, w1slab, c1, smem, blockIdx.x, blockIdx.y);
 }
 
-template <typename T, bool MASK_DY, bool A1X, int GH, int GW, int GCI, int GCO, bool STAGE = false, int CS = 1>
+template <typename T, bool MASK_DY, bool A1X, int GH, int GW, int GCI, int GCO, bool STAGE = false, int CS = 1,
+          bool SC1 = false>
 __device__ __forceinline__ void wgrad_body(
     const T* __restrict__ dY, const T* __restrict__ Yact, const T* __restrict__ X,
     float* __restrict__ slab, int B, int H, int W, int Cin, int Cout, int R, C1Src c1, char* smem, int bx, int by) {
@@ -387,7 +393,8 @@
     bf16x8 v = zero8();
     if (r < R && hh < H && c < W) {
       const long off = (((long)n * H + hh) * W + c) * Cout + ch;
-      v = ld16(dY + off);
+      if constexpr (SC1) v = ld16_sc1(whole_rsrc(dY), (int)(off * (long)sizeof(T)));
+      else v = ld16(dY + off);
       if (MASK_DY) v = mask16<T>(v, ld16(Yact + off));
     }
     return v;
@@ -582,23 +589,38 @@
 
 constexpr int BFC_MAXB = 64;
 
+template <bool SC1 = false>
 __device__ __forceinline__ float* fc_role_prologue(const BwdFc& fcr, int B, char* smem, bool first0) {
   float* s_dl = reinterpret_cast<float*>(smem);
-  for (int i = threadIdx.x; i < B * 10; i += 256) s_dl[(i / 10) * FCDW_LD + i % 10] = fcr.dl[i];
+  for (int i = threadIdx.x; i < B * 10; i += 256) {
+    if constexpr (SC1)
+      s_dl[(i / 10) * FCDW_LD + i % 10] =
+          __builtin_bit_cast(float, __builtin_amdgcn_raw_buffer_load_b32(whole_rsrc(fcr.dl), i * 4, 0, 16 ));
+    else
+      s_dl[(i / 10) * FCDW_LD + i % 10] = fcr.dl[i];
+  }
   __syncthreads();
   if (first0 && threadIdx.x < 64) {
     float* s_dd = s_dl + B * FCDW_LD;
     for (int i = threadIdx.x; i < B * 10; i += 64) s_dd[i] = s_dl[(i / 10) * FCDW_LD + i % 10];
+    const float* s_ls = nullptr;
+    if constexpr (SC1) {
+      float* ls = s_dd + B * 10;
+      for (int i = threadIdx.x; i < B; i += 64)
+        ls[i] = __builtin_bit_cast(float, __builtin_amdgcn_raw_buffer_load_b32(whole_rsrc(fcr.ex.loss_rows), i * 4, 0, 16));
+      s_ls = ls;
+    }
+    if constexpr (SC1) asm volatile("s_waitcnt vmcnt(0)" ::: "memory");
     asm volatile("s_waitcnt lgkmcnt(0)" ::: "memory");
-    fc_bwd_bias_loss<false>(fcr.ex, s_dd, nullptr, B, 10, true);
+    fc_bwd_bias_loss<false>(fcr.ex, s_dd, nullptr, B, 10, true, s_ls);
   }
   return s_dl;
 }
-template <typename T>
+template <typename T, bool SC1 = false>
 __device__ __forceinline__ void fc_role_chunk(const BwdFc& fcr, const float* s_dl, int B, long q) {
   const T* a2 = static_cast<const T*>(fcr.a2);
-  if (B <= 32) fc_dw_wave_chunk<32>(s_dl, a2, fcr.dW, fcr.scale, B, fcr.K, fcr.ex, q * 128);
-  else fc_dw_wave_chunk<BFC_MAXB>(s_dl, a2, fcr.dW, fcr.scale, B, fcr.K, fcr.ex, q * 128);
+  if (B <= 32) fc_dw_wave_chunk<32, T, SC1>(s_dl, a2, fcr.dW, fcr.scale, B, fcr.K, fcr.ex, q * 128);
+  else fc_dw_wave_chunk<BFC_MAXB, T, SC1>(s_dl, a2, fcr.dW, fcr.scale, B, fcr.K, fcr.ex, q * 128);
 }
 
 template <int SLEEP = 2>
diff --git a/csrc/kernels/conv3x3_fwd.h b/csrc/kernels/conv3x3_fwd.h
--- a/csrc/kernels/conv3x3_fwd.h
+++ b/csrc/kernels/conv3x3_fwd.h
@@ -26,10 +26,6 @@
 };
 constexpr int MRG_ERR = 5;
 
-__device__ __forceinline__ bf16x8 ld16_sc1(__amdgpu_buffer_rsrc_t r, int byte_off) {
-  typedef __attribute__((ext_vector_type(4))) int i32x4_t;
-  return __builtin_bit_cast(bf16x8, __builtin_amdgcn_raw_buffer_load_b128(r, byte_off, 0, 16 ));
-}
 __device__ __forceinline__ Conv1Group conv1_group_load_sc1(const float* w1, const float* b1, int g) {
   Conv1Group r;
 #pragma unroll
@@ -83,7 +79,7 @@
     T* __restrict__ Y, int B, int H, int W, int Cin, int Cout,
     const T* __restrict__ wfc, float* __restrict__ fc_part, C1Src c1, FwdDz dzo) {
   constexpr bool MRG = false;
-  constexpr bool NOA2 = false;
+  constexpr bool NOA2 = false, WTL = false;
   const FwdMerge mg{};
   extern __shared__ __attribute__((aligned(16))) char smem[];
   const int bx = (int)blockIdx.x, by = (int)blockIdx.y;
@@ -91,7 +87,7 @@
 }
 
 template <typename T, int PXT, int NW, bool RELU, int NOF, bool A1X, int GH, int GW, int GCI, int GCO, bool DZ,
-          int OCC, bool MRG>
+          int OCC, bool MRG, bool WTL = false>
 __device__ __forceinline__ void fwd_body(
     const int bx, const int by, const T* __restrict__ X, const T* __restrict__ Wt, const float* __restrict__ bias,
     T* __restrict__ Y, int B, int H, int W, int Cin, int Cout, const T* __restrict__ wfc,
diff --git a/csrc/kernels/conv3x3_fwd_body.inc.h b/csrc/kernels/conv3x3_fwd_body.inc.h
--- a/csrc/kernels/conv3x3_fwd_body.inc.h
+++ b/csrc/kernels/conv3x3_fwd_body.inc.h
@@ -386,8 +386,13 @@
         const float d = xent_row_dl(s_lg + slot * NOF, NOF, o, label, dzo.gscale, &lossv);
         s_dl[lane] = d;
         if (dzo.dl_out && (slot == 1 || P0 == (long)img0 * HWi)) {
-          dzo.dl_out[im * NOF + o] = d;
-          if (o == 0) dzo.loss_rows[im] = lossv;
+          if constexpr (WTL) {
+            st_wt(dzo.dl_out + im * NOF + o, d);
+            if (o == 0) st_wt(dzo.loss_rows + im, lossv);
+          } else {
+            dzo.dl_out[im * NOF + o] = d;
+            if (o == 0) dzo.loss_rows[im] = lossv;
+          }
         }
       }
     }
diff --git a/csrc/kernels/fc_bwd_body.h b/csrc/kernels/fc_bwd_body.h
--- a/csrc/kernels/fc_bwd_body.h
+++ b/csrc/kernels/fc_bwd_body.h
@@ -65,7 +65,7 @@
 
 template <bool XENT>
 __device__ __forceinline__ void fc_bwd_bias_loss(const FcBwdExtras& ex, const float* s_dl, const float* s_loss,
-                                                 int B, int NO, bool last) {
+                                                 int B, int NO, bool last, const float* lds_rows = nullptr) {
   const int lane = threadIdx.x & 63;
   if (ex.dbias && lane < NO) {
     float acc = 0.f;
@@ -82,7 +82,7 @@
     }
   }
   if ((XENT || ex.loss_rows) && ex.loss_out) {
-    const float* lr = XENT ? s_loss : ex.loss_rows;
+    const float* lr = XENT ? s_loss : lds_rows ? lds_rows : ex.loss_rows;
     const int at = ex.step_ctr ? *ex.step_ctr : 0;
     float acc = 0.f;
     for (int b0 = 0; b0 < B; b0 += 64) {
@@ -107,7 +107,7 @@
 }
 
 constexpr int FCDW_LD = 12;
-template <int MAXB, typename T>
+template <int MAXB, typename T, bool SC1 = false>
 __device__ __forceinline__ void fc_dw_wave_chunk(const float* s_dl, const T* __restrict__ X,
                                                  float* __restrict__ dW, float scale, int B, long K,
                                                  const FcBwdExtras& ex, long col0) {
@@ -138,9 +138,9 @@
 #pragma unroll
   for (int b = 0; b < MAXB; ++b) {
     if constexpr (F32)
-      xf[b] = __builtin_bit_cast(float2, __builtin_amdgcn_raw_buffer_load_b64(rx, vo4, (int)((long)min(b, B - 1) * K * 4), 0));
+      xf[b] = __builtin_bit_cast(float2, __builtin_amdgcn_raw_buffer_load_b64(rx, vo4, (int)((long)min(b, B - 1) * K * 4), SC1 ? 16 : 0));
     else
-      xw[b] = (unsigned)__builtin_amdgcn_raw_buffer_load_b32(rx, vo2, (int)((long)min(b, B - 1) * K * 2), 0);
+      xw[b] = (unsigned)__builtin_amdgcn_raw_buffer_load_b32(rx, vo2, (int)((long)min(b, B - 1) * K * 2), SC1 ? 16 : 0);
   }
   float acc[NO][2];
 #pragma unroll
diff --git a/csrc/kernels/infer.hip b/csrc/kernels/infer.hip
--- a/csrc/kernels/infer.hip
+++ b/csrc/kernels/infer.hip
@@ -11,7 +11,7 @@
     const float* __restrict__ fc_bias, int B, float* __restrict__ fc_part, int* __restrict__ img_cnt, C1Src c1,
     InferOut out) {
   constexpr int PXT = 1, NOF = 10, OCC = 1, GH = 28, GW = 28, GCI = 32, GCO = 64;
-  constexpr bool RELU = true, A1X = true, DZ = false, MRG = false, NOA2 = true;
+  constexpr bool RELU = true, A1X = true, DZ = false, MRG = false, NOA2 = true, WTL = false;
   const T* X = nullptr;
   T* Y = nullptr;
   int H = GH, W = GW, Cin = GCI, Cout = GCO;
diff --git a/csrc/kernels/launchers.h b/csrc/kernels/launchers.h
--- a/csrc/kernels/launchers.h
+++ b/csrc/kernels/launchers.h
@@ -344,6 +344,31 @@
                        bf16_t* Y, int B, const bf16_t* wfc, float* fc_part, const C1Src& c1, const FwdDz& dz,
                        int* err, hipStream_t s, const ShadowSet* late = nullptr);
 bool conv3x3_step_head_fits(int nx, int B);
+
+constexpr int ONE_MAX_B = 32;
+constexpr int ONE_FCIN_OFF = SYNC_RED_INTS;
+constexpr int ONE_IMG_OFF = SYNC_RED_INTS + 32;
+constexpr int ONE_IMG_STRIDE = 32;
+constexpr int ONE_BANK_INTS = ONE_IMG_OFF + ONE_IMG_STRIDE * ONE_MAX_B;
+constexpr int ONE_ERR = 6;
+struct StepOne {
+  const bf16_t* Wt = nullptr;
+  const float* bias = nullptr;
+  bf16_t* Y = nullptr;
+  const bf16_t* wfc = nullptr;
+  float* fc_part = nullptr;
+  C1Src c1{};
+  FwdDz dzo{};
+  int* sync = nullptr;
+  int* sel = nullptr;
+  int* step_ctr = nullptr;
+  unsigned* gen = nullptr;
+  int* err = nullptr;
+  int nf = 0, nfcb = 0, nitems = 0;
+};
+bool conv3x3_step_one_fits(int B, int R, bool stored_a1 = false);
+bool conv3x3_step_one(const bf16_t* WT, float* w1slab, float* slab, int B, int R, const SlabSet& fused, int* red_err,
+                      const BwdFc& fc, const StepOne& one, hipStream_t s);
 int conv3x3_step_head_slots();
 
 }
diff --git a/csrc/kernels/optim.hip b/csrc/kernels/optim.hip
--- a/csrc/kernels/optim.hip
+++ b/csrc/kernels/optim.hip
@@ -148,6 +148,7 @@
 void stamps_set_conv1(void*);
 void stamps_set_conv3x3(void*);
 void stamps_set_conv3x3_bwd(void*);
+void stamps_set_step_one(void*);
 void stamps_set_linear(void*);
 void stamps_set_xent(void*);
 void stamps_set_allreduce(void*);
@@ -157,6 +158,7 @@
   stamps_set_conv1(p);
   stamps_set_conv3x3(p);
   stamps_set_conv3x3_bwd(p);
+  stamps_set_step_one(p);
   stamps_set_linear(p);
   stamps_set_xent(p);
   stamps_set_allreduce(p);
diff --git a/csrc/kernels/step_one.hip b/csrc/kernels/step_one.hip
--- /dev/null
+++ b/csrc/kernels/step_one.hip
@@ -0,0 +1,278 @@
+#include <algorithm>
+#include <stdexcept>
+
+#include <cstdio>
+#include <cstdlib>
+
+#include "kernels/conv3x3_fwd.h"
+
+namespace ddp_amd {
+
+__device__ __forceinline__ int one_img_blocks(int im) {
+  return (im * 784 + 783) / 64 - im * 784 / 64 + 1;
+}
+
+__device__ __forceinline__ void one_wait_images(const int* cnt, int lo, int hi, int* err) {
+  if (threadIdx.x < 64) {
+    const int im = lo + (int)threadIdx.x;
+    const bool act = im <= hi;
+    const int want = act ? one_img_blocks(im) : 0;
+    const unsigned long long t0 = __builtin_amdgcn_s_memrealtime();
+    while (true) {
+      const int v = act ? __hip_atomic_load(cnt + ONE_IMG_STRIDE * im, __ATOMIC_RELAXED, __HIP_MEMORY_SCOPE_AGENT) : 0;
+      if (__all(v >= want)) break;
+      if (__builtin_amdgcn_s_memrealtime() - t0 > DZ_WAIT_TICKS) {
+        if (threadIdx.x == 0 && err) __hip_atomic_store(err, ONE_ERR, __ATOMIC_RELAXED, __HIP_MEMORY_SCOPE_AGENT);
+        break;
+      }
+      __builtin_amdgcn_s_sleep(2);
+    }
+  }
+  __syncthreads();
+}
+
+__device__ __forceinline__ void one_wait_arrivals(const int* done, int nblk, int* err, int code) {
+  if (threadIdx.x < 64) {
+    const int lane = threadIdx.x;
+    const unsigned long long t0 = __builtin_amdgcn_s_memrealtime();
+    while (true) {
+      const int v = lane < 8 ? __hip_atomic_load(done + 32 * lane, __ATOMIC_RELAXED, __HIP_MEMORY_SCOPE_AGENT) : 0;
+      int tot = 0;
+#pragma unroll
+      for (int l = 0; l < 8; ++l) tot += __builtin_amdgcn_readlane(v, l);
+      if (tot >= nblk) break;
+      if (__builtin_amdgcn_s_memrealtime() - t0 > DZ_WAIT_TICKS) {
+        if (lane == 0 && err) __hip_atomic_store(err, code, __ATOMIC_RELAXED, __HIP_MEMORY_SCOPE_AGENT);
+        break;
+      }
+      __builtin_amdgcn_s_sleep(2);
+    }
+  }
+  __syncthreads();
+}
+
+template <typename T, bool DA>
+__global__ __launch_bounds__(256, 2) void step_one_kernel(
+    const T* __restrict__ WT, float* __restrict__ w1slab, float* __restrict__ slab, int B, int R, int nd,
+    BwdReduce red, BwdFc fcr, StepOne one) {
+  extern __shared__ __attribute__((aligned(16))) char smem[];
+  const int cb = (int)blockIdx.x;
+  const int nconv = red.nconv;
+  const int sel = __builtin_amdgcn_readfirstlane(
+                      __hip_atomic_load(one.sel, __ATOMIC_RELAXED, __HIP_MEMORY_SCOPE_AGENT)) & 1;
+  int* const bank = one.sync + sel * ONE_BANK_INTS;
+  {
+    int* const other = one.sync + (sel ^ 1) * ONE_BANK_INTS;
+    for (int i = cb * 256 + (int)threadIdx.x; i < ONE_BANK_INTS; i += (int)gridDim.x * 256) other[i] = 0;
+  }
+  int* const img_cnt = bank + ONE_IMG_OFF;
+  const T* const dY = one.dzo.dz2;
+
+  if (cb >= nconv) {
+    const int f = cb - nconv;
+    if (f > 0 && threadIdx.x == 0)
+      __hip_atomic_fetch_add(bank + ONE_FCIN_OFF, 1, __ATOMIC_RELAXED, __HIP_MEMORY_SCOPE_AGENT);
+    DDP_STAMP(STAMP_K_FC_BWD, 0);
+    __builtin_amdgcn_s_setprio(2);
+    one_wait_images(img_cnt, 0, B - 1, one.err);
+    DDP_STAMP(STAMP_K_FC_BWD, 5);
+    const float* s_dl = fc_role_prologue<true>(fcr, B, smem, f == 0);
+    DDP_STAMP(STAMP_K_FC_BWD, 1);
+    const int nch = (int)((fcr.K + 127) / 128);
+    const int q0 = f * 4 + (int)(threadIdx.x >> 6);
+    if (q0 < nch) fc_role_chunk<T, true>(fcr, s_dl, B, q0);
+    __builtin_amdgcn_sched_barrier(0);
+    const int q1 = (f + one.nfcb) * 4 + (int)(threadIdx.x >> 6);
+    if (f + one.nfcb < one.nitems && q1 < nch) fc_role_chunk<T, true>(fcr, s_dl, B, q1);
+    DDP_STAMP(STAMP_K_FC_BWD, 4);
+    if (f == 0) {
+      one_wait_arrivals(bank, nconv, one.err, ONE_ERR);
+      wait_count(bank + ONE_FCIN_OFF, one.nfcb - 1, one.err, ONE_ERR);
+      if (threadIdx.x == 0) {
+        one.step_ctr[0] += 1;
+        const unsigned g = *one.gen + 1u;
+        *one.gen = g == 0xffffffffu ? 0u : g;
+        __hip_atomic_store(one.sel, sel ^ 1, __ATOMIC_RELAXED, __HIP_MEMORY_SCOPE_AGENT);
+      }
+    }
+    return;
+  }
+
+  C1Src c1r = one.c1;
+  c1r.bi.offset = one.c1.bi.base();
+  c1r.bi.step_ctr = nullptr;
+  c1r.xb_out = nullptr;
+  c1r.yb_out = nullptr;
+  constexpr int HW = 28 * 28;
+  const long Ptot = (long)B * HW;
+
+  if (cb < one.nf) {
+    fwd_body<T, 1, 4, true, 10, true, 28, 28, 32, 64, true, 1, false, true>(
+        cb, 0, static_cast<const T*>(nullptr), one.Wt, one.bias, one.Y, B, 28, 28, 32, 64, one.wfc, one.fc_part,
+        one.c1, one.dzo, FwdMerge{});
+    asm volatile("s_waitcnt vmcnt(0)" ::: "memory");
+    __syncthreads();
+    if (threadIdx.x == 0) {
+      const long P0 = (long)cb * 64;
+      const int i0 = (int)(P0 / HW), i1 = (int)(((P0 + 64 < Ptot ? P0 + 64 : Ptot) - 1) / HW);
+      __hip_atomic_fetch_add(img_cnt + ONE_IMG_STRIDE * i0, 1, __ATOMIC_RELAXED, __HIP_MEMORY_SCOPE_AGENT);
+      if (i1 != i0)
+        __hip_atomic_fetch_add(img_cnt + ONE_IMG_STRIDE * i1, 1, __ATOMIC_RELAXED, __HIP_MEMORY_SCOPE_AGENT);
+    }
+  }
+
+  const int nw = nconv - nd;
+  int rd = cb;
+  if (red.interleave) {
+    const int m = nd < nw ? nd : nw;
+    if (cb < 2 * m) rd = (cb & 1) ? nd + (cb >> 1) : (cb >> 1);
+    else rd = nd > nw ? cb - m : nd + (cb - m);
+  }
+  if (rd < nd) {
+    const long p_lo = (long)rd * 128 - 29, p_hi = (long)rd * 128 + 128 + 28;
+    const int lo = (int)((p_lo < 0 ? 0 : p_lo) / HW), hi = (int)((p_hi >= Ptot ? Ptot - 1 : p_hi) / HW);
+    DDP_STAMP(STAMP_K_DGRAD, 5);
+    one_wait_images(img_cnt, lo, hi, one.err);
+    DDP_STAMP(STAMP_K_DGRAD, 6);
+    dgrad_body<T, 2, false, true, true, DA, 28, 28, 32, 64, 0, true>(
+        dY, nullptr, WT, DA ? nullptr : reinterpret_cast<const T*>(one.c1.a1_out), nullptr, B, 28, 28, 32, 64, c1r.x, 1,
+        c1r.bi, w1slab, c1r, smem, rd, 0);
+  } else {
+    const int bx = rd - nd, nRC = (28 + R - 1) / R;
+    const int rb = (((B * nRC) & 7) == 0) ? (((bx >> 4) << 3) | (bx & 7)) : (bx >> 1);
+    const int n = rb / nRC;
+    DDP_STAMP(STAMP_K_WGRAD, 5);
+    one_wait_images(img_cnt, n, n, one.err);
+    DDP_STAMP(STAMP_K_WGRAD, 6);
+    wgrad_body<T, false, true, 28, 28, 32, 64, true, 2, true>(dY, nullptr, nullptr, slab, B, 28, 28, 32, 64, R, c1r,
+                                                             smem, bx, 0);
+  }
+
+  asm volatile("s_waitcnt vmcnt(0)" ::: "memory");
+  __syncthreads();
+  if (threadIdx.x == 0)
+    __hip_atomic_fetch_add(bank + 32 * (blockIdx.x & 7), 1, __ATOMIC_RELAXED, __HIP_MEMORY_SCOPE_AGENT);
+  if (cb < red.first_reducer) return;
+  const int w = cb - red.first_reducer, nr = nconv - red.first_reducer;
+  float* part = reinterpret_cast<float*>(smem);
+  if (red.deep) {
+    constexpr int J = 2;
+    SlabFusedPlan<J> pl;
+    slab_fused_plan<J>(red.ss, w, nr, red.nchunks, pl);
+    DDP_STAMP(STAMP_K_GRAD_REDUCE, 0);
+    one_wait_arrivals(bank, nconv, red.err, RED_ERR);
+    DDP_STAMP(STAMP_K_GRAD_REDUCE, 1);
+    slab_fused_run16<J>(red.ss, pl, part);
+    for (long q0 = w + (long)J * nr; q0 < red.nchunks; q0 += (long)J * nr) {
+      slab_fused_plan<J>(red.ss, q0, nr, red.nchunks, pl);
+      slab_fused_run16<J>(red.ss, pl, part);
+    }
+  } else {
+    constexpr int J = 3;
+    SlabFusedPlan<J> pl;
+    slab_fused_plan<J>(red.ss, w, nr, red.nchunks, pl);
+    DDP_STAMP(STAMP_K_GRAD_REDUCE, 0);
+    one_wait_arrivals(bank, nconv, red.err, RED_ERR);
+    DDP_STAMP(STAMP_K_GRAD_REDUCE, 1);
+    slab_fused_run<J>(red.ss, pl, part);
+    for (long q0 = w + (long)J * nr; q0 < red.nchunks; q0 += (long)J * nr) {
+      slab_fused_plan<J>(red.ss, q0, nr, red.nchunks, pl);
+      slab_fused_run<J>(red.ss, pl, part);
+    }
+  }
+  DDP_STAMP(STAMP_K_GRAD_REDUCE, 2);
+}
+
+namespace {
+
+struct OneGrid {
+  int nf = 0, nd = 0, nrows = 0, nw = 0, nitems = 0, nfcb = 0;
+  size_t lds = 0;
+  bool fits = false;
+};
+
+OneGrid one_grid(int B, int R, bool da) {
+  OneGrid g;
+  if (B <= 0 || B > ONE_MAX_B || R <= 0) return g;
+  g.nf = conv3x3_dgrad_blocks(B, 28, 28, 1);
+  g.nd = conv3x3_dgrad_blocks(B, 28, 28, 2);
+  g.nrows = conv3x3_wgrad_blocks(B, 28, R);
+  g.nw = 2 * g.nrows;
+  g.nitems = (int)(((long)28 * 28 * 64 + 127) / 128 + 3) / 4;
+  g.lds = std::max(conv3x3_bwd_lds(28, 32, 64, 2, R, 2, 2), conv3x3_fwd_lds(28, 32, 1, true, 2));
+  auto k = da ? step_one_kernel<bf16_t, true> : step_one_kernel<bf16_t, false>;
+  lds_optin(k, g.lds);
+  int dev = 0, cus = 0, occ = 0;
+  if (hipGetDevice(&dev) != hipSuccess) return g;
+  if (hipDeviceGetAttribute(&cus, hipDeviceAttributeMultiprocessorCount, dev) != hipSuccess) return g;
+  if (hipOccupancyMaxActiveBlocksPerMultiprocessor(&occ, reinterpret_cast<const void*>(k), 256, g.lds) != hipSuccess)
+    return g;
+  const long cap = (long)occ * cus;
+  const int nconv = g.nd + g.nw;
+  g.nfcb = (int)std::min<long>(g.nitems, cap - nconv);
+  g.fits = g.nf <= nconv && g.nfcb >= 1 && 2 * g.nfcb >= g.nitems && g.nrows <= cap / 2 && nconv + g.nfcb <= cap;
+  return g;
+}
+
+}
+
+bool conv3x3_step_one_fits(int B, int R, bool stored_a1) { return one_grid(B, R, !stored_a1).fits; }
+
+bool conv3x3_step_one(const bf16_t* WT, float* w1slab, float* slab, int B, int R, const SlabSet& fused,
+                      int* red_err, const BwdFc& fc, const StepOne& one_in, hipStream_t s) {
+  const char* bad = !one_in.sync || !one_in.sel || !one_in.step_ctr || !one_in.gen ? "the hand-off words"
+                    : !one_in.dzo.dz2 || !one_in.dzo.gran || !one_in.dzo.gen || !one_in.dzo.fc_bias ||
+                              !one_in.dzo.dl_out || !one_in.dzo.loss_rows
+                        ? "the level-3 forward's outputs"
+                    : !one_in.wfc || !one_in.Wt || !one_in.c1.x || !one_in.c1.bi.step_ctr ? "the forward's operands"
+                    : !fc.dl || !fc.a2 || fc.K != (long)28 * 28 * 64 || fc.ex.last_ctr ? "the fc role's operands" : nullptr;
+  if (bad) throw std::runtime_error(std::string("conv3x3_step_one: missing ") + bad);
+  if (one_in.c1.zero_i32 || fc.ex.step_inc || fc.ex.gen_inc || fused.step_ctr)
+    throw std::runtime_error("conv3x3_step_one: fc block 0 advances the step's words itself; the forward zeroes none");
+  if ((reinterpret_cast<uintptr_t>(slab) & 15) != 0)
+    throw std::runtime_error("conv3x3_step_one: slab rows must start 16-byte aligned");
+  const bool da = one_in.c1.a1_out == nullptr;
+  const OneGrid g = one_grid(B, R, da);
+  if (!g.fits) return false;
+  if (grad_reduce_groups(fused) != 16) return false;
+  for (int k = 0; k < fused.count; ++k)
+    if (fused.s[k].n < 4) return false;
+  const int nconv = g.nd + g.nw;
+  BwdReduce red;
+  red.nconv = nconv;
+  {
+    const char* e = std::getenv("DDP_AMD_BWD_INTERLEAVE");
+    red.interleave = e && e[0] ? (e[0] == '1') : 1;
+  }
+  red.first_reducer = nconv - g.nrows;
+  red.ss = fused;
+  red.nchunks = slab_chunks(fused);
+  {
+    int kmax = 0;
+    for (int k = 1; k < fused.count; ++k)
+      if (fused.s[k].n > fused.s[kmax].n) kmax = k;
+    const int rows = fused.s[kmax].rows;
+    const char* e = std::getenv("DDP_AMD_RED_DEEP");
+    red.deep = (rows > 128 && rows <= 256 && !(e && e[0] == '0')) ? 1 : 0;
+  }
+  red.err = red_err;
+  BwdFc fcr = fc;
+  fcr.nconv = nconv;
+  fcr.fc0 = nconv;
+  fcr.nfc = g.nitems;
+  if ((size_t)B * (FCDW_LD + 10 + 1) * sizeof(float) > g.lds || g.lds < sizeof(float) * 3 * 16 * 64)
+    throw std::runtime_error("conv3x3_step_one: LDS too small for the fc role / the reducer");
+  StepOne one = one_in;
+  one.nf = g.nf;
+  one.nfcb = g.nfcb;
+  one.nitems = g.nitems;
+  auto k = da ? step_one_kernel<bf16_t, true> : step_one_kernel<bf16_t, false>;
+  lds_optin(k, g.lds);
+  hipLaunchKernelGGL(k, dim3((unsigned)(nconv + g.nfcb)), dim3(256), g.lds, s, WT, w1slab, slab, B, R, g.nd, red, fcr,
+                     one);
+  return true;
+}
+
+DDP_STAMPS_SETTER(stamps_set_step_one)
+
+}
diff --git a/csrc/runtime/engine.cpp b/csrc/runtime/engine.cpp
--- a/csrc/runtime/engine.cpp
+++ b/csrc/runtime/engine.cpp
@@ -37,6 +37,9 @@
   for (hipEvent_t* e : {&e_b0_, &e_b1_, &e_d0_, &e_d1_, &e_fwd_, &e_fc_})
     DDP_HIP_CHECK(hipEventCreateWithFlags(e, hipEventDisableTiming));
   l3_fits_.assign(cfg_.max_batch + 1, -1);
+  one_fits_.assign(cfg_.max_batch + 1, -1);
+  if (const char* e = std::getenv("DDP_AMD_ONE_LAUNCH"))
+    if (e[0] == '0' || e[0] == '1') cfg_.one_launch = e[0] == '1';
   if (b_.sync_err) {
     DDP_HIP_CHECK(hipHostMalloc(reinterpret_cast<void**>(&err_host_), sizeof(int),
                                 hipHostMallocCoherent | hipHostMallocMapped));
@@ -51,6 +54,9 @@
     DDP_HIP_CHECK(hipMalloc(reinterpret_cast<void**>(&gen_), 256));
     DDP_HIP_CHECK(hipMemset(gran_, 0, ng * sizeof(unsigned long long)));
     DDP_HIP_CHECK(hipMemset(gen_, 0, 256));
+    const size_t nb = (2 * (size_t)ONE_BANK_INTS + 64) * sizeof(int);
+    DDP_HIP_CHECK(hipMalloc(reinterpret_cast<void**>(&one_sync_), nb));
+    DDP_HIP_CHECK(hipMemset(one_sync_, 0, nb));
     DDP_HIP_CHECK(hipStreamSynchronize(nullptr));
   }
 }
@@ -64,6 +70,7 @@
   if (err_host_) hipHostFree(err_host_);
   if (gran_) hipFree(gran_);
   if (gen_) hipFree(gen_);
+  if (one_sync_) hipFree(one_sync_);
 }
 
 void SimpleCNNEngine::destroy_graph() {
@@ -80,6 +87,7 @@
     throw std::runtime_error(std::string("engine: an in-launch hand-off wait timed out (") +
                              (e == RED_ERR ? "fused slab reduction" : e == XAR_ERR ? "in-launch all-reduce"
                               : e == HEAD_ERR ? "dist_mode 4 step head: forward waiting for the bucket all-reduce"
+                              : e == ONE_ERR ? "one-launch step: backward waiting for the forward"
                                               : "level-3 forward dZ2") +
                              "); results invalid");
   }
@@ -102,6 +110,11 @@
                     cfg_.C2 == 64
                 ? 1 : 0;
     f.l3_fits = fit == 1;
+  }
+  if (cfg_.one_launch && f.l3_fits && one_sync_ && !cfg_.f32 && cfg_.pxt_fwd == 1 && batch <= ONE_MAX_B) {
+    signed char& fit = one_fits_[batch];
+    if (fit < 0) fit = conv3x3_step_one_fits(batch, cfg_.wgrad_rows, cfg_.store_a1 != 0) ? 1 : 0;
+    f.one_fits = fit == 1;
   }
   f.fc_role_ok = conv3x3_bwd_fc_role_ok(cfg_.H, cfg_.W, cfg_.C1, cfg_.C2, cfg_.pxt_dgrad, cfg_.wgrad_split);
   f.xar_plan_ok = xar_plan_ok_;
@@ -318,6 +331,39 @@
   return head_used;
 }
 
+bool SimpleCNNEngine::launch_step_one(int B, const StepPlan& pl, const SgdArgs& sa, const C1Src& c1,
+                                      const FwdDz& dzo) {
+  const long K = (long)cfg_.H * cfg_.W * cfg_.C2;
+  BwdFc fcr;
+  fcr.a2 = b_.a2;
+  fcr.dl = b_.dlogits;
+  fcr.dW = nullptr;
+  fcr.scale = 1.f / (float)cfg_.world;
+  fcr.K = K;
+  fcr.ex = make_fc_extras(B, pl, sa);
+  fcr.ex.step_inc = nullptr;
+  fcr.ex.gen_inc = nullptr;
+  const SlabSet ss = make_slabs(B, pl, sa);
+  StepOne one;
+  one.Wt = b_.w2_bf16;
+  one.bias = b_.params + b_.off_b2;
+  one.Y = b_.a2;
+  one.wfc = b_.wfc_frag;
+  one.fc_part = b_.fc_part;
+  one.c1 = c1;
+  one.c1.zero_i32 = nullptr;
+  one.dzo = dzo;
+  one.sync = one_sync_;
+  one.sel = one_sync_ + 2 * ONE_BANK_INTS;
+  one.step_ctr = b_.step_ctr;
+  one.gen = gen_;
+  one.err = b_.sync_err;
+  const bool ok = conv3x3_step_one(b_.w2t_bf16, b_.w1slab, b_.w2slab, B, cfg_.wgrad_rows, ss, b_.sync_err, fcr, one,
+                                   cs_);
+  if (ok) DDP_HIP_CHECK(hipGetLastError());
+  return ok;
+}
+
 template <typename T>
 void SimpleCNNEngine::launch_step_t(int B, int stride, bool first_momentum_step, unsigned parts) {
   constexpr bool BF16 = std::is_same<T, bf16_t>::value;
@@ -342,7 +388,18 @@
   const C1Src c1 = make_c1src(B, stride, pl);
   const FwdDz dzo = pl.l3 ? make_fwd_dz(B) : FwdDz{};
   bool head_used = false;
+  last_one_ = false;
   if constexpr (BF16) {
+    if (pl.one && parts == PART_ALL) {
+      if (launch_step_one(B, pl, sa, c1, dzo)) {
+        if (capturing_) graph_heads_ += 1;
+        plain_stale_ = true;
+        last_one_ = last_fused_reduce_ = last_level3_ = last_fc_role_ = true;
+        last_xar_ = last_pair_ = last_head_ = false;
+        return;
+      }
+      one_refused_ += 1;
+    }
     if (parts & PART_HEAD) {
       if (first_momentum_step) throw std::runtime_error("engine: the step head runs the steady-state SGD only");
       head_used = launch_step_head(B, sa, op.sh, c1, dzo);
diff --git a/csrc/runtime/runtime.h b/csrc/runtime/runtime.h
--- a/csrc/runtime/runtime.h
+++ b/csrc/runtime/runtime.h
@@ -248,6 +248,9 @@
   bool last_xar() const { return last_xar_; }
   bool last_pair() const { return last_pair_; }
   bool last_head() const { return last_head_; }
+  bool last_one() const { return last_one_; }
+  bool one_active(int batch) { return plan(batch).one; }
+  int one_refused() const { return one_refused_; }
   int graph_heads() const { return graph_heads_; }
   void set_momentum_started(bool v) { momentum_started_ = v; }
   void set_xgmi(std::shared_ptr<XgmiComm> x, std::vector<int> channels);
@@ -266,6 +269,7 @@
   FcBwdExtras make_fc_extras(int B, const StepPlan& pl, const SgdArgs& sa) const;
   SlabSet make_slabs(int B, const StepPlan& pl, const SgdArgs& sa) const;
   bool launch_step_head(int B, const SgdArgs& sa, const ShadowSet& sh, const C1Src& c1, const FwdDz& dzo);
+  bool launch_step_one(int B, const StepPlan& pl, const SgdArgs& sa, const C1Src& c1, const FwdDz& dzo);
   void launch_buckets(int stage, bool use_x, const SgdArgs& sa, float* M, const ShadowSet& sh);
   void join_buckets();
   void enqueue_buckets(int stage, bool use_x, hipStream_t s, const SgdArgs& sa, float* M, const ShadowSet& sh);
@@ -286,6 +290,7 @@
   hipStream_t cs_ = nullptr, ms_ = nullptr;
   hipEvent_t e_b0_, e_b1_, e_d0_, e_d1_, e_fwd_, e_fc_;
   std::vector<signed char> l3_fits_;
+  std::vector<signed char> one_fits_;
   hipGraph_t graph_ = nullptr;
   hipGraphExec_t graph_exec_ = nullptr;
   int graph_steps_ = 0;
@@ -296,6 +301,8 @@
   bool last_xar_ = false;
   bool last_pair_ = false;
   bool last_head_ = false;
+  bool last_one_ = false;
+  int one_refused_ = 0;
   bool capturing_ = false;
   int graph_heads_ = 0;
   bool xar_plan_ok_ = false;
@@ -310,6 +317,7 @@
   int* err_host_ = nullptr;
   unsigned long long* gran_ = nullptr;
   unsigned* gen_ = nullptr;
+  int* one_sync_ = nullptr;
 };
 
 }
diff --git a/csrc/runtime/step_plan.h b/csrc/runtime/step_plan.h
--- a/csrc/runtime/step_plan.h
+++ b/csrc/runtime/step_plan.h
@@ -17,6 +17,7 @@
   int fuse_reduce = 1;
   int wgrad_split = 1;
   int dist_mode = 3;
+  int one_launch = 1;
 };
 
 struct StepFacts {
@@ -28,6 +29,7 @@
   bool l3_fits = false;
   bool fc_role_ok = false;
   bool xar_plan_ok = false;
+  bool one_fits = false;
 };
 
 struct StepPlan {
@@ -44,6 +46,7 @@
   bool fopt;
   bool fork;
   bool xar_wanted;
+  bool one;
 };
 
 inline StepPlan plan_step(const EngineConfig& c, const StepFacts& f, int B) {
@@ -61,6 +64,8 @@
   p.fopt = !p.dist && c.fuse_opt;
   p.fork = p.dist && p.l3 && c.dist_mode == 1;
   p.xar_wanted = p.xar_mode && c.dist_mode == 2 && p.fc_role && p.fred;
+  p.one = c.one_launch && !c.f32 && p.l3 && p.fc_role && p.fred && !p.dist && p.fopt && c.pxt_fwd == 1 &&
+          c.store_a1 <= 1 && f.one_fits;
   return p;
 }
 
diff --git a/pytorch-distributed-data-parallel-ddp-trainer_amd/_build.py b/pytorch-distributed-data-parallel-ddp-trainer_amd/_build.py
--- a/pytorch-distributed-data-parallel-ddp-trainer_amd/_build.py
+++ b/pytorch-distributed-data-parallel-ddp-trainer_amd/_build.py
@@ -67,7 +67,8 @@
 
 
 KERNEL_FLAGS = {"conv3x3.hip": ["-fno-slp-vectorize"], "conv3x3_bwd.hip": ["-fno-slp-vectorize"],
-                "infer.hip": ["-fno-slp-vectorize"]}
+                "infer.hip": ["-fno-slp-vectorize"],
+                "step_one.hip": ["-fno-slp-vectorize"]}
 COMMON_FLAGS = ["-O3", "-fPIC", "-std=c++17", "-D__HIP_PLATFORM_AMD__"]
 DEVICE_FLAGS = ["-munsafe-fp-atomics"]
 BIND_FLAGS = ["-O2", "-DUSE_ROCM", "-DTORCH_EXTENSION_NAME=_C", "-DTORCH_API_INCLUDE_EXTENSION_H"]
diff --git a/pytorch-distributed-data-parallel-ddp-trainer_amd/engine/fused_step.py b/pytorch-distributed-data-parallel-ddp-trainer_amd/engine/fused_step.py
--- a/pytorch-distributed-data-parallel-ddp-trainer_amd/engine/fused_step.py
+++ b/pytorch-distributed-data-parallel-ddp-trainer_amd/engine/fused_step.py
@@ -31,6 +31,7 @@
     force_allreduce: bool = False
     fuse_level: int = 3
     l3_fc_role: int = 1
+    one_launch: int = 1
     fuse_opt: bool = True
     fuse_reduce: int | None = None
     store_a1: int | None = None
@@ -205,7 +206,8 @@
                    fuse_level=self._fuse_level_ok(world_size), fuse_opt=bool(self.opts.fuse_opt),
                    store_a1=int(self.store_a1), f32=f32, fuse_reduce=self._fuse_reduce_ok(world_size),
                    epoch_order=bool(self.opts.epoch_order), wgrad_split=int(self.opts.wgrad_split),
-                   l3_fc_role=int(self.opts.l3_fc_role), dist_mode=int(self.opts.dist_mode))
+                   l3_fc_role=int(self.opts.l3_fc_role), dist_mode=int(self.opts.dist_mode),
+                   one_launch=int(self.opts.one_launch))
         self.dtype = "fp32" if f32 else "bf16"
         use_comm = world_size > 1 or self.opts.force_allreduce
         self.xgmi = None
@@ -257,6 +259,11 @@
             self.eng.set_momentum_started(True)
         self.stream = torch.cuda.ExternalStream(self.eng.stream, device=dev)
         self.level3 = bool(self.eng.level3_active(B))
+        self.one_launch = bool(self.eng.one_active(B))
+        if (self.opts.one_launch and not self.one_launch and self.level3 and not use_comm
+                and self.opts.dtype != "fp32"):
+            self._log_downgrade("one-launch step -> forward and backward as two launches "
+                                f"(batch {B}: the chain's conditions or its resident grid do not hold)")
         self._captured = 0
         self.steps_done = 0
         self._need_barrier = world_size > 1
```
